# rvl-lab-utoronto/video_similarity_search

Hardware: NVIDIA B200
Metric: finch_full_hierarchy_embeddings_per_s (higher is better)
Workload: dtype f16 screen (f32 accumulate) + f32/f64 exact re-rank

## Files before the change

### include/slic_b200.h

```cpp
#ifndef SLIC_B200_H
#define SLIC_B200_H

#include <stddef.h>
#include <stdint.h>

#ifdef __cplusplus
extern "C" {
#endif

#define SLIC_ABI_VERSION 1

#define SLIC_F32 0
#define SLIC_F64 1

#define SLIC_METRIC_COSINE 0
#define SLIC_METRIC_EUCLIDEAN 1

typedef enum slic_status {
    SLIC_OK = 0,
    SLIC_ERR_INVALID_ARG = -1,
    SLIC_ERR_CUDA = -2,
    SLIC_ERR_UNSUPPORTED = -3,
    SLIC_ERR_NO_DEVICE = -4,
    SLIC_ERR_OVERFLOW = -5
} slic_status;

typedef void* slic_stream_t;

int slic_abi_version(void);
const char* slic_last_error(void);
int slic_require_device(void);
int64_t slic_launch_count(void);
int slic_profile_screen(int32_t enable);
int slic_last_screen_time(float* ms_out, double* flop_out);
int slic_last_screen_exec_flop(double* flop_out);

int slic_screen_trace(int32_t enable, uint64_t* counters_out_host);

int slic_normalize_rows(const void* x_dev, int64_t n, int32_t d, int32_t dtype,
                        void* unit_dev, void* norms_dev,
                        uint16_t* unit_f16_dev, int32_t d_pad, slic_stream_t stream);

int slic_center_columns(const float* x_dev, int64_t n, int32_t d, float* out_dev, float* means_out_dev,
                        slic_stream_t stream);

int slic_nn_exact_top1(const void* q_unit_dev, const int32_t* q_rows_dev, int64_t nq,
                       const void* x_unit_dev, int64_t n, int32_t d, int32_t dtype,
                       int64_t self_offset, int32_t* idx_out_dev, void* dist_out_dev,
                       slic_stream_t stream);

int slic_nn_top1(const void* q_unit_dev, const uint16_t* q_f16_dev, int64_t nq,
                 const void* x_unit_dev, const uint16_t* x_f16_dev, int64_t n,
                 int32_t d, int32_t d_pad, int32_t dtype, int64_t self_offset, float eps,
                 int32_t* idx_out_dev, void* dist_out_dev, int32_t* stats_out_dev ,
                 slic_stream_t stream);

int slic_sym_row_bests(const float* unit_dev, const uint16_t* unit_f16_dev, int64_t n, int32_t d, int32_t d_pad,
                       int32_t part, int32_t parts, int32_t* bests_out_dev, slic_stream_t stream);
int slic_nn_top1_sym_part(const float* unit_dev, const uint16_t* unit_f16_dev, int64_t n, int32_t d,
                          int32_t d_pad, int32_t part, int32_t parts, const int32_t* row_bests_dev, float eps,
                          uint64_t* keys_out_dev, int32_t* stats_out_dev ,
                          slic_stream_t stream);
int slic_unpack_neighbor_keys(const uint64_t* keys_dev, int64_t n, int32_t* idx_out_dev,
                              float* dist_out_dev, int32_t* status_out_dev, slic_stream_t stream);

int slic_debug_sym_plan(int64_t n, int32_t part, int32_t parts, int32_t mode, int32_t gated_chunks,
                        int32_t* units_out_host, int64_t capacity, int64_t* num_units_out_host);

int slic_screen_scores_debug(const uint16_t* q_f16_dev, int64_t nq, const uint16_t* x_f16_dev,
                             int64_t n, int32_t d_pad, float* out_dev, slic_stream_t stream);

int slic_distance_matrix(const void* q_dev, int64_t nq, const void* x_dev, int64_t n,
                         int32_t d, int32_t dtype, int32_t metric, int32_t same_matrix,
                         void* out_dev, int64_t ld_out, slic_stream_t stream);

int slic_rows_topk(const void* dist_dev, int64_t nq, int64_t n, int64_t ld, int32_t dtype,
                   int32_t k, int32_t* idx_out_dev, void* val_out_dev, slic_stream_t stream);

int slic_topk_cosine(const void* q_unit_dev, int64_t nq, const void* x_unit_dev, int64_t n,
                     int32_t d, int32_t dtype, int32_t k, int64_t self_offset,
                     int32_t* idx_out_dev, void* dist_out_dev, slic_stream_t stream);

int slic_topk_cosine_tc(const void* q_unit_dev, const uint16_t* q_f16_dev, int64_t nq,
                        const void* x_unit_dev, const uint16_t* x_f16_dev, int64_t n,
                        int32_t d, int32_t d_pad, int32_t dtype, int32_t k, int64_t self_offset,
                        float eps, int32_t* idx_out_dev, void* dist_out_dev,
                        int32_t* stats_out_dev, slic_stream_t stream);

int slic_hit_at_k(const int32_t* topk_idx_dev, int64_t nq, int32_t k_stride,
                  const int64_t* q_labels_dev, const int64_t* x_labels_dev,
                  const int32_t* ks_dev, int32_t num_ks, int32_t* hits_out_dev,
                  slic_stream_t stream);

int slic_finch_components(const int32_t* nn_dev, int64_t n, int32_t use_filter, double min_sim,
                          const void* unit_dev, int32_t d, int32_t dtype, const void* dist_nn_dev,
                          int32_t* labels_out_dev, int32_t* num_clust_out_dev,
                          slic_stream_t stream);

int slic_finch_min_sim(const int32_t* nn_dev, int64_t n, const void* unit_dev, int32_t d,
                       int32_t dtype, const void* dist_nn_dev, float* min_sim_out_dev,
                       slic_stream_t stream);

int slic_finch_closest_link(const int32_t* nn_dev, int64_t n, const void* unit_dev, int32_t d,
                            int32_t dtype, const void* dist_nn_dev, int32_t* pair_out_dev,
                            slic_stream_t stream);

int slic_compose_labels(const int32_t* prev_dev, const int32_t* u_dev, int64_t n,
                        int32_t* out_dev, slic_stream_t stream);

int slic_segmented_mean(const float* data_dev, const int32_t* labels_dev, int64_t n, int32_t d,
                        int32_t num_clust, double* out_dev, slic_stream_t stream);

int slic_cluster_sums(const float* data_dev, const int32_t* labels_dev, int64_t n, int32_t d,
                      int32_t num_clust, double* sums_out_dev, int32_t* counts_out_dev,
                      double* means_out_dev, slic_stream_t stream);
int slic_merge_cluster_sums(const double* sums_prev_dev, const int32_t* counts_prev_dev,
                            const int32_t* labels_dev, int64_t n_prev, int32_t d, int32_t num_clust,
                            double* sums_out_dev, int32_t* counts_out_dev, double* means_out_dev,
                            slic_stream_t stream);

int slic_kmeans_plusplus(const float* unit_dev, int64_t n, int32_t d, int32_t k, int64_t first_id,
                         const double* uniforms_host, int32_t L, int32_t* seeds_out_dev, slic_stream_t stream);
int slic_spherical_kmeans(const float* x_dev, int64_t n, int32_t d, int32_t k, const float* init_dev,
                          const int64_t* first_ids_host, const double* uniforms_host, int32_t L, int32_t n_init,
                          int32_t max_iter, double tol, int32_t* labels_out_dev, float* centers_out_dev,
                          double* inertia_out_host, int32_t* n_iter_out_host, int64_t* stats_out_host,
                          slic_stream_t stream);

int slic_label_mask_u8(const int64_t* a_dev, int64_t na, const int64_t* b_dev, int64_t nb,
                       int32_t prepend_ones, int32_t negate, uint8_t* out_dev,
                       slic_stream_t stream);
int slic_label_mask_bits(const int64_t* a_dev, int64_t na, const int64_t* b_dev, int64_t nb,
                         int32_t negate, uint32_t* out_dev, slic_stream_t stream);

int slic_scatter_last_wins(const int32_t* values_dev, const int64_t* positions_dev, int64_t n,
                           int64_t n_out, int32_t fill, int32_t* out_dev, int32_t* out_of_range_dev,
                           slic_stream_t stream);

int slic_dense_labels(const int32_t* labels_dev, int64_t n, int32_t* dense_out_dev, int32_t* uniq_out_dev,
                      int32_t* num_out_dev, slic_stream_t stream);

int slic_cluster_metrics(const int32_t* labels_true_dev, const int32_t* labels_pred_dev, int64_t n,
                         int32_t num_true, int32_t num_pred, int32_t want_emi, double* out_dev,
                         slic_stream_t stream);

int slic_group_by_label(const int32_t* labels_dev, int64_t n, int32_t num_labels,
                        int32_t* order_out_dev, int32_t* offsets_out_dev, slic_stream_t stream);

int slic_set_flann_threshold(int64_t rows);

int slic_finch(const float* data_dev, int64_t n, int32_t d,
               const int32_t* nn0_dev, const float* dist0_dev, const float* unit0_dev,
               int32_t level0_dense, int32_t ensure_early_exit, int32_t capacity,
               int32_t* labels_out_dev, int32_t* num_clust_out_host, int32_t* num_levels_out_host,
               float* min_sim_out_host , int32_t* has_min_sim_out_host ,
               slic_stream_t stream);

int slic_first_neighbors_host(const void* x_host, int64_t n, int32_t d, int32_t dtype,
                              int32_t* nn_out_host, void* dist_out_host);


int slic_finch_host(const float* x_host, int64_t n, int32_t d, const int64_t* initial_rank_host,
                    int32_t ensure_early_exit, int32_t capacity, int32_t* labels_out_host,
                    int32_t* num_clust_out_host, int32_t* num_levels_out_host,
                    float* min_sim_out_host , int32_t* has_min_sim_out_host );

int slic_copy_to_device(void* dst_dev, const void* src_host, int64_t bytes, slic_stream_t stream);

int slic_set_upload_overlap(int32_t enable);

typedef struct slic_comm slic_comm_t;
#define SLIC_COMM_HANDLE_BYTES 64

int slic_comm_create(const int32_t* devices, int32_t num_devices, int64_t max_rows, slic_comm_t** comm_out);
int slic_finch_multi(slic_comm_t* comm, const float* x_host, int64_t n, int32_t d, const int64_t* initial_rank_host,
                     int32_t ensure_early_exit, int32_t capacity, int32_t* labels_out_host,
                     int32_t* num_clust_out_host, int32_t* num_levels_out_host,
                     float* min_sim_out_host , int32_t* has_min_sim_out_host );
int slic_comm_last_timeline(slic_comm_t* comm, float* ms_out_host);
int slic_comm_destroy(slic_comm_t* comm);

int slic_comm_window_create(int64_t max_rows, slic_comm_t** comm_out, void* ipc_handle_out );
int slic_comm_connect(slic_comm_t* comm, int32_t rank, int32_t world, const void* all_handles);
int slic_comm_nn_top1(slic_comm_t* comm, const float* unit_dev, const uint16_t* f16_dev, int64_t n, int32_t d,
                      int32_t d_pad, int32_t* idx_out_dev, float* dist_out_dev, int32_t* status_out_dev,
                      slic_stream_t stream);

int slic_comm_finch(slic_comm_t* comm, const float* data_dev, int64_t n, int32_t d, int32_t ensure_early_exit,
                    int32_t capacity, int32_t* labels_out_dev, int32_t* num_clust_out_host,
                    int32_t* num_levels_out_host, float* min_sim_out_host ,
                    int32_t* has_min_sim_out_host , slic_stream_t stream);

int slic_host_trace(int32_t enable, float* ms_out_host);

#ifdef __cplusplus
}
#endif
#endif
```

### video_similarity_search_b200/_lib.py

```python
import ctypes
import os

from . import build as _build

_c = ctypes
_i32, _i64, _f32, _f64 = _c.c_int32, _c.c_int64, _c.c_float, _c.c_double
_ptr = _c.c_void_p

SIGNATURES = {
    "slic_abi_version": [],
    "slic_last_error": [],
    "slic_require_device": [],
    "slic_launch_count": [],
    "slic_profile_screen": [_i32],
    "slic_last_screen_time": [_ptr, _ptr],
    "slic_last_screen_exec_flop": [_ptr],
    "slic_screen_trace": [_i32, _ptr],
    "slic_normalize_rows": [_ptr, _i64, _i32, _i32, _ptr, _ptr, _ptr, _i32, _ptr],
    "slic_center_columns": [_ptr, _i64, _i32, _ptr, _ptr, _ptr],
    "slic_nn_exact_top1": [_ptr, _ptr, _i64, _ptr, _i64, _i32, _i32, _i64, _ptr, _ptr, _ptr],
    "slic_nn_top1": [_ptr, _ptr, _i64, _ptr, _ptr, _i64, _i32, _i32, _i32, _i64, _f32, _ptr, _ptr, _ptr, _ptr],
    "slic_sym_row_bests": [_ptr, _ptr, _i64, _i32, _i32, _i32, _i32, _ptr, _ptr],
    "slic_nn_top1_sym_part": [_ptr, _ptr, _i64, _i32, _i32, _i32, _i32, _ptr, _f32, _ptr, _ptr, _ptr],
    "slic_debug_sym_plan": [_i64, _i32, _i32, _i32, _i32, _ptr, _i64, _ptr],
    "slic_unpack_neighbor_keys": [_ptr, _i64, _ptr, _ptr, _ptr, _ptr],
    "slic_screen_scores_debug": [_ptr, _i64, _ptr, _i64, _i32, _ptr, _ptr],
    "slic_distance_matrix": [_ptr, _i64, _ptr, _i64, _i32, _i32, _i32, _i32, _ptr, _i64, _ptr],
    "slic_rows_topk": [_ptr, _i64, _i64, _i64, _i32, _i32, _ptr, _ptr, _ptr],
    "slic_topk_cosine": [_ptr, _i64, _ptr, _i64, _i32, _i32, _i32, _i64, _ptr, _ptr, _ptr],
    "slic_topk_cosine_tc": [_ptr, _ptr, _i64, _ptr, _ptr, _i64, _i32, _i32, _i32, _i32, _i64, _f32, _ptr, _ptr, _ptr, _ptr],
    "slic_hit_at_k": [_ptr, _i64, _i32, _ptr, _ptr, _ptr, _i32, _ptr, _ptr],
    "slic_finch_components": [_ptr, _i64, _i32, _f64, _ptr, _i32, _i32, _ptr, _ptr, _ptr, _ptr],
    "slic_finch_min_sim": [_ptr, _i64, _ptr, _i32, _i32, _ptr, _ptr, _ptr],
    "slic_finch_closest_link": [_ptr, _i64, _ptr, _i32, _i32, _ptr, _ptr, _ptr],
    "slic_compose_labels": [_ptr, _ptr, _i64, _ptr, _ptr],
    "slic_segmented_mean": [_ptr, _ptr, _i64, _i32, _i32, _ptr, _ptr],
    "slic_cluster_sums": [_ptr, _ptr, _i64, _i32, _i32, _ptr, _ptr, _ptr, _ptr],
    "slic_merge_cluster_sums": [_ptr, _ptr, _ptr, _i64, _i32, _i32, _ptr, _ptr, _ptr, _ptr],
    "slic_label_mask_u8": [_ptr, _i64, _ptr, _i64, _i32, _i32, _ptr, _ptr],
    "slic_label_mask_bits": [_ptr, _i64, _ptr, _i64, _i32, _ptr, _ptr],
    "slic_dense_labels": [_ptr, _i64, _ptr, _ptr, _ptr, _ptr],
    "slic_scatter_last_wins": [_ptr, _ptr, _i64, _i64, _i32, _ptr, _ptr, _ptr],
    "slic_cluster_metrics": [_ptr, _ptr, _i64, _i32, _i32, _i32, _ptr, _ptr],
    "slic_group_by_label": [_ptr, _i64, _i32, _ptr, _ptr, _ptr],
    "slic_first_neighbors_host": [_ptr, _i64, _i32, _i32, _ptr, _ptr],
    "slic_set_flann_threshold": [_i64],
    "slic_host_trace": [_i32, _ptr],
    "slic_set_upload_overlap": [_i32],
    "slic_copy_to_device": [_ptr, _ptr, _i64, _ptr],
    "slic_comm_create": [_ptr, _i32, _i64, _ptr],
    "slic_finch_multi": [_ptr, _ptr, _i64, _i32, _ptr, _i32, _i32, _ptr, _ptr, _ptr, _ptr, _ptr],
    "slic_comm_last_timeline": [_ptr, _ptr],
    "slic_comm_destroy": [_ptr],
    "slic_comm_window_create": [_i64, _ptr, _ptr],
    "slic_comm_connect": [_ptr, _i32, _i32, _ptr],
    "slic_comm_nn_top1": [_ptr, _ptr, _ptr, _i64, _i32, _i32, _ptr, _ptr, _ptr, _ptr],
    "slic_comm_finch": [_ptr, _ptr, _i64, _i32, _i32, _i32, _ptr, _ptr, _ptr, _ptr, _ptr, _ptr],
    "slic_finch": [_ptr, _i64, _i32, _ptr, _ptr, _ptr, _i32, _i32, _i32, _ptr, _ptr, _ptr, _ptr, _ptr, _ptr],
    "slic_finch_host": [_ptr, _i64, _i32, _ptr, _i32, _i32, _ptr, _ptr, _ptr, _ptr, _ptr],
    "slic_kmeans_plusplus": [_ptr, _i64, _i32, _i32, _i64, _ptr, _i32, _ptr, _ptr],
    "slic_spherical_kmeans": [_ptr, _i64, _i32, _i32, _ptr, _ptr, _ptr, _i32, _i32, _i32, _f64, _ptr, _ptr, _ptr, _ptr,
                              _ptr, _ptr],
}
_RESTYPES = {"slic_last_error": _c.c_char_p, "slic_launch_count": _c.c_int64}

SLIC_F32, SLIC_F64 = 0, 1
SLIC_METRIC_COSINE, SLIC_METRIC_EUCLIDEAN = 0, 1

_lib = None


class SlicError(RuntimeError):
    """A C-ABI call returned a negative status."""


def library_path():
    return _build.LIB_PATH


def load(build_if_missing=True):
    global _lib
    if _lib is not None:
        return _lib
    path = library_path()
    if not os.path.exists(path):
        if not build_if_missing:
            raise ImportError("libslic_b200.so is missing; run `python -m video_similarity_search_b200.build`")
        _build.build()
    lib = ctypes.CDLL(path)
    for name, argtypes in SIGNATURES.items():
        fn = getattr(lib, name)
        fn.argtypes = argtypes
        fn.restype = _RESTYPES.get(name, _c.c_int)
    if lib.slic_abi_version() != 1:
        raise ImportError("libslic_b200.so ABI version mismatch")
    _lib = lib
    return lib


def check(status, what):
    if status != 0:
        msg = load().slic_last_error()
        raise SlicError("%s failed with status %d: %s" % (what, status, msg.decode() if msg else "?"))


def call(name, *args):
    lib = load()
    check(getattr(lib, name)(*args), name)
```

### video_similarity_search_b200/csrc/nn_screen_tc.cu

```cuda
#include <cuda.h>
#include <cuda_fp16.h>
#include <math.h>
#include <stdlib.h>
#include <string.h>
#include <math_constants.h>

#include <algorithm>
#include <type_traits>
#include <vector>

#include "common.cuh"

namespace slic {

constexpr int TC_BM = 128, TC_BK = 64, TC_UMMA_K = 16;
constexpr int TC_BN = 256;
constexpr int TC_ARES_SPS = 2;
constexpr int TC_ROW_UNIT = 256;
static_assert(TC_ROW_UNIT == TC_BN, "a row unit's diagonal block is one column tile");
constexpr uint32_t TC_A_BYTES = TC_BM * TC_BK * 2;
constexpr int TC_ARES_MAX_SLABS = 8;
constexpr uint32_t TC_BAR_BYTES = 384;
constexpr int TC_UQ_DEPTH = 4;
constexpr int TC_TMEM_COLS = 512;
constexpr int TC_ACCS = TC_TMEM_COLS / TC_BN;
template <bool ARES, bool TOPK> struct TcCfg {
    static constexpr uint32_t B_ROWS = TC_BN / 2;
    static constexpr uint32_t B_BYTES = B_ROWS * TC_BK * 2;
    static constexpr uint32_t A_RES_BYTES = ARES ? TC_ARES_MAX_SLABS * TC_A_BYTES : 0;
    static constexpr int SPS = ARES ? TC_ARES_SPS : 2;
    static constexpr uint32_t SLAB_BYTES = ARES ? B_BYTES : TC_A_BYTES + B_BYTES;
    static constexpr uint32_t STAGE_BYTES = SPS * SLAB_BYTES;
    static constexpr int STAGES = ARES ? (TOPK ? 64 : 96) * 1024 / (int)STAGE_BYTES : 3;
    static_assert(STAGES >= 2 && STAGES <= 6, "ring depth");
    static constexpr uint32_t OPERAND_BYTES = A_RES_BYTES + STAGES * STAGE_BYTES;
    static constexpr uint32_t SMEM_BYTES = OPERAND_BYTES + TC_BAR_BYTES  + 960  +
                                           (TOPK ? 32768u : 0u) ;
    static constexpr uint32_t SYM_THR_BYTES = 2 * 2 * 128 * 2;
    static constexpr uint32_t SYM_SMEM_BYTES = OPERAND_BYTES + TC_BAR_BYTES + SYM_THR_BYTES + (ARES ? 640u : 960u);
    static constexpr uint32_t CORESIDENT_MAX_BYTES = 233472 - 2 * 1024;
    static_assert(TOPK || SYM_SMEM_BYTES <= CORESIDENT_MAX_BYTES,
                  "symmetric variant leaves no shared memory for a co-resident CTA of the upload stream");
    static_assert(TOPK || SMEM_BYTES <= CORESIDENT_MAX_BYTES,
                  "top-1 variant (gated launches) leaves no shared memory for a co-resident CTA of the upload stream");
    static_assert(SMEM_BYTES <= 232448, "exceeds the 227 KB of shared memory a CTA may use");
};
constexpr int TC_MAX_STAGES = 6;
constexpr int TC_EPI_WARPS = 8;
constexpr int TC_THREADS = 64 + 32 * TC_EPI_WARPS;
constexpr int TC_THREADS_SYM = TC_THREADS + 32;
constexpr float TC_DEFAULT_EPS = 0.001953125f + 0.0009765625f + 0.0000152587890625f;
constexpr int TC_TOPK_MAX = 64;
constexpr int TC_HIST_BINS = 128;
constexpr int TC_HIST_STRIDE = 2 * TC_BM;
constexpr uint32_t TC_TOPK_SMEM = TC_HIST_BINS * TC_HIST_STRIDE;
static_assert(TC_TOPK_SMEM == 32768, "TcCfg::SMEM_BYTES assumes 32 KB of histograms");

struct ScreenParams {
    int64_t nq, n;
    int num_k_slabs;
    int64_t self_offset;
    float eps;
    int cap;
    int splits;
    int tiles_per_split;
    int64_t num_units;
    int* cand_idx;
    float* cand_score;
    int* cand_cnt;
    int* cand_flags;
    int topk;
    float* cand_kth;
    int* cand_tb;
    float* dump;
    int* error_flag;
    unsigned long long* trace;
    const int4* unit_table;
    const int* gates;
    unsigned int* best_enc;
    int* log_q;
    int log_region;
    int* sync_counter;
    const int* sync_targets;
    int* queue;
    int num_peers;
    unsigned int* peer_best[SLIC_MAX_PEERS];
    int* peer_sync[SLIC_MAX_PEERS];
};

struct UnitInfo {
    int64_t row_unit;
    int64_t ct0;
    int count, stride;
    int gate;
    int stream;
    bool coldir;
};
__device__ __forceinline__ UnitInfo unit_info(const ScreenParams& p, int64_t u, int64_t n_col_tiles) {
    UnitInfo ui;
    if (p.unit_table) {
        const int4 e = __ldg(p.unit_table + u);
        ui.row_unit = e.x;
        ui.ct0 = e.y;
        ui.count = e.z & 0xffff;
        ui.stride = (int)((unsigned)e.z >> 16);
        ui.gate = (e.w & 0xfff) - 1;
        ui.stream = (e.w >> 12) & 0xffff;
        ui.coldir = ((e.w >> 28) & 1) != 0;
    } else {
        const int64_t row_units = p.num_units / p.splits;
        const int split = (int)(u / row_units);
        ui.row_unit = u % row_units;
        ui.ct0 = (int64_t)split * p.tiles_per_split;
        const int64_t left = n_col_tiles - ui.ct0;
        ui.count = (int)(left < p.tiles_per_split ? (left > 0 ? left : 0) : p.tiles_per_split);
        ui.stride = 1;
        ui.gate = -1;
        ui.stream = split;
        ui.coldir = false;
    }
    return ui;
}

__device__ __forceinline__ unsigned enc_score(float f) {
    const unsigned u = __float_as_uint(f);
    return (u & 0x80000000u) ? ~u : (u | 0x80000000u);
}
__device__ __forceinline__ float dec_score(unsigned e) {
    return __uint_as_float((e & 0x80000000u) ? (e & 0x7fffffffu) : ~e);
}
constexpr unsigned ENC_NEG_INF = 0x007fffffu;

__device__ __forceinline__ uint32_t smem_u32(const void* p) { return (uint32_t)__cvta_generic_to_shared(p); }

__device__ __forceinline__ void mbar_init(uint32_t bar, uint32_t count) {
    asm volatile("mbarrier.init.shared::cta.b64 [%0], %1;" ::"r"(bar), "r"(count));
}
__device__ __forceinline__ void mbar_arrive(uint32_t bar) {
    asm volatile("mbarrier.arrive.shared::cta.b64 _, [%0];" ::"r"(bar) : "memory");
}
__device__ __forceinline__ void mbar_expect_tx(uint32_t bar, uint32_t bytes) {
    asm volatile("mbarrier.arrive.expect_tx.shared::cta.b64 _, [%0], %1;" ::"r"(bar), "r"(bytes) : "memory");
}
__device__ int* g_timeout_record = nullptr;
__device__ int g_timeout_lock = 0;
__device__ __noinline__ void record_timeout(int site, int a, int b) {
    int* r = g_timeout_record;
    if (r && atomicCAS(&g_timeout_lock, 0, 1) == 0) {
        volatile int* v = r;
        v[1] = (int)blockIdx.x;
        v[2] = (int)threadIdx.x;
        v[3] = a;
        v[4] = b;
        v[0] = site;
        __threadfence_system();
    }
}

__device__ __forceinline__ void mbar_wait(uint32_t bar, uint32_t parity, int* error_flag) {
    uint32_t done = 0;
    long long t0 = 0;
    uint32_t polls = 0;
    while (true) {
        asm volatile(
            "{\n\t.reg .pred p;\n\t"
            "mbarrier.try_wait.parity.shared::cta.b64 p, [%1], %2;\n\t"
            "selp.u32 %0, 1, 0, p;\n\t}"
            : "=r"(done)
            : "r"(bar), "r"(parity)
            : "memory");
        if (done) return;
        if ((++polls & 0x3ff) == 0) {
            long long now = clock64();
            if (t0 == 0) t0 = now;
            else if (now - t0 > 8000000000ll) {
                if (error_flag) atomicExch(error_flag, 1);
                record_timeout(1, (int)bar, (int)parity);
                __trap();
            }
        }
    }
}
__device__ __forceinline__ void mbar_wait_traced(uint32_t bar, uint32_t parity, int* error_flag, unsigned long long& acc,
                                                 bool tracing) {
    if (!tracing) {
        mbar_wait(bar, parity, error_flag);
        return;
    }
    const long long t0 = clock64();
    mbar_wait(bar, parity, error_flag);
    acc += (unsigned long long)(clock64() - t0);
}
__device__ __forceinline__ bool mbar_test(uint32_t bar, uint32_t parity) {
    uint32_t done;
    asm volatile(
        "{\n\t.reg .pred p;\n\t"
        "mbarrier.test_wait.parity.shared::cta.b64 p, [%1], %2;\n\t"
        "selp.u32 %0, 1, 0, p;\n\t}"
        : "=r"(done)
        : "r"(bar), "r"(parity)
        : "memory");
    return done != 0;
}
constexpr int SCREEN_ERR_GATE = 3;
__device__ __forceinline__ void gate_wait(const int* gate, int* error_flag) {
    long long t0 = 0;
    uint32_t polls = 0;
    while (true) {
        int v;
        asm volatile("ld.acquire.gpu.global.b32 %0, [%1];" : "=r"(v) : "l"(gate) : "memory");
        if (v != 0) break;
        __nanosleep(256);
        if ((++polls & 0xff) == 0) {
            if (error_flag && *reinterpret_cast<volatile int*>(error_flag) == SCREEN_ERR_GATE) break;
            long long now = clock64();
            if (t0 == 0) t0 = now;
            else if (now - t0 > 4000000000ll) {
                if (error_flag) atomicCAS(error_flag, 0, SCREEN_ERR_GATE);
                record_timeout(2, (int)(reinterpret_cast<uintptr_t>(gate) & 0xffff), v);
                break;
            }
        }
    }
    asm volatile("fence.proxy.async.global;" ::: "memory");
}
__device__ __forceinline__ void counter_wait(const int* counter, int target, int* error_flag) {
    long long t0 = 0;
    uint32_t polls = 0;
    while (true) {
        int v;
        asm volatile("ld.acquire.sys.global.b32 %0, [%1];" : "=r"(v) : "l"(counter) : "memory");
        if (v >= target) break;
        __nanosleep(128);
        if ((++polls & 0xff) == 0) {
            if (error_flag && *reinterpret_cast<volatile int*>(error_flag) == SCREEN_ERR_GATE) break;
            long long now = clock64();
            if (t0 == 0) t0 = now;
            else if (now - t0 > 4000000000ll) {
                if (error_flag) atomicCAS(error_flag, 0, SCREEN_ERR_GATE);
                record_timeout(3, v, target);
                break;
            }
        }
    }
}
constexpr uint32_t TC_PEER_BIT_MASK = 0xFEFFFFFFu;
__device__ __forceinline__ void tma_load_2d_pair(const CUtensorMap* map, uint32_t dst, uint32_t leader_bar, int c0, int c1) {
    asm volatile(
        "cp.async.bulk.tensor.2d.cta_group::2.shared::cluster.global.mbarrier::complete_tx::bytes [%0], [%1, {%2, %3}], [%4];"
        ::"r"(dst), "l"(map), "r"(c0), "r"(c1), "r"(leader_bar & TC_PEER_BIT_MASK)
        : "memory");
}
__device__ __forceinline__ void mbar_arrive_leader(uint32_t bar) {
    asm volatile("mbarrier.arrive.shared::cluster.b64 _, [%0];" ::"r"(bar & TC_PEER_BIT_MASK) : "memory");
}
__device__ __forceinline__ uint32_t peer_smem_addr(uint32_t local_addr, uint32_t rank) {
    uint32_t r;
    asm volatile("mapa.shared::cluster.u32 %0, %1, %2;" : "=r"(r) : "r"(local_addr), "r"(rank));
    return r;
}
__device__ __forceinline__ void st_cluster_u32(uint32_t cluster_addr, uint32_t v) {
    asm volatile("st.shared::cluster.u32 [%0], %1;" ::"r"(cluster_addr), "r"(v) : "memory");
}
__device__ __forceinline__ void mbar_arrive_release_cluster(uint32_t cluster_addr) {
    asm volatile("mbarrier.arrive.release.cluster.shared::cluster.b64 _, [%0];" ::"r"(cluster_addr) : "memory");
}
__device__ __forceinline__ void mbar_wait_cluster(uint32_t bar, uint32_t parity, int* error_flag) {
    uint32_t done = 0;
    long long t0 = 0;
    uint32_t polls = 0;
    while (true) {
        asm volatile(
            "{\n\t.reg .pred p;\n\t"
            "mbarrier.try_wait.parity.acquire.cluster.shared::cta.b64 p, [%1], %2;\n\t"
            "selp.u32 %0, 1, 0, p;\n\t}"
            : "=r"(done)
            : "r"(bar), "r"(parity)
            : "memory");
        if (done) return;
        if ((++polls & 0x3ff) == 0) {
            long long now = clock64();
            if (t0 == 0) t0 = now;
            else if (now - t0 > 40000000000ll) {
                if (error_flag) atomicExch(error_flag, 1);
                record_timeout(4, (int)bar, (int)parity);
                __trap();
            }
        }
    }
}
struct UnitRing {
    uint32_t full, val;
    uint32_t empty_leader;
    int slot;
    uint32_t phase;
};
__device__ __forceinline__ int ring_take(UnitRing& r, bool whole_warp, int* error_flag) {
    mbar_wait_cluster(r.full + 8u * r.slot, r.phase, error_flag);
    int u;
    asm volatile("ld.shared.s32 %0, [%1];" : "=r"(u) : "r"(r.val + 4u * r.slot) : "memory");
    if (whole_warp) __syncwarp();
    if (!whole_warp || (threadIdx.x & 31) == 0) mbar_arrive_release_cluster(r.empty_leader + 8u * r.slot);
    if (++r.slot == TC_UQ_DEPTH) {
        r.slot = 0;
        r.phase ^= 1u;
    }
    return u;
}
__device__ __forceinline__ uint32_t cluster_ctarank() {
    uint32_t r;
    asm volatile("mov.u32 %0, %%cluster_ctarank;" : "=r"(r));
    return r;
}
__device__ __forceinline__ void cluster_sync_all() {
    asm volatile("barrier.cluster.arrive.release.aligned;" ::: "memory");
    asm volatile("barrier.cluster.wait.acquire.aligned;" ::: "memory");
}
__device__ __forceinline__ void tc_fence_before() { asm volatile("tcgen05.fence::before_thread_sync;" ::: "memory"); }
__device__ __forceinline__ void tc_fence_after() { asm volatile("tcgen05.fence::after_thread_sync;" ::: "memory"); }
__device__ __forceinline__ void umma_f16_pair(uint32_t tmem_d, uint64_t desc_a, uint64_t desc_b, uint32_t idesc,
                                               uint32_t accumulate) {
    asm volatile(
        "{\n\t.reg .pred p;\n\t"
        "setp.ne.b32 p, %4, 0;\n\t"
        "tcgen05.mma.cta_group::2.kind::f16 [%0], %1, %2, %3, p;\n\t}"
        ::"r"(tmem_d), "l"(desc_a), "l"(desc_b), "r"(idesc), "r"(accumulate)
        : "memory");
}
__device__ __forceinline__ void umma_commit_pair(uint32_t bar) {
    asm volatile(
        "tcgen05.commit.cta_group::2.mbarrier::arrive::one.shared::cluster.multicast::cluster.b64 [%0], %1;"
        ::"r"(bar), "h"((uint16_t)3)
        : "memory");
}
#define SLIC_V32_OUT(v)                                                                                              \
    "=r"(v[0]), "=r"(v[1]), "=r"(v[2]), "=r"(v[3]), "=r"(v[4]), "=r"(v[5]), "=r"(v[6]), "=r"(v[7]), "=r"(v[8]),     \
        "=r"(v[9]), "=r"(v[10]), "=r"(v[11]), "=r"(v[12]), "=r"(v[13]), "=r"(v[14]), "=r"(v[15]), "=r"(v[16]),      \
        "=r"(v[17]), "=r"(v[18]), "=r"(v[19]), "=r"(v[20]), "=r"(v[21]), "=r"(v[22]), "=r"(v[23]), "=r"(v[24]),     \
        "=r"(v[25]), "=r"(v[26]), "=r"(v[27]), "=r"(v[28]), "=r"(v[29]), "=r"(v[30]), "=r"(v[31])
#define SLIC_V32_INOUT(v)                                                                                            \
    "+r"(v[0]), "+r"(v[1]), "+r"(v[2]), "+r"(v[3]), "+r"(v[4]), "+r"(v[5]), "+r"(v[6]), "+r"(v[7]), "+r"(v[8]),     \
        "+r"(v[9]), "+r"(v[10]), "+r"(v[11]), "+r"(v[12]), "+r"(v[13]), "+r"(v[14]), "+r"(v[15]), "+r"(v[16]),      \
        "+r"(v[17]), "+r"(v[18]), "+r"(v[19]), "+r"(v[20]), "+r"(v[21]), "+r"(v[22]), "+r"(v[23]), "+r"(v[24]),     \
        "+r"(v[25]), "+r"(v[26]), "+r"(v[27]), "+r"(v[28]), "+r"(v[29]), "+r"(v[30]), "+r"(v[31])
__device__ __forceinline__ void tmem_ld_issue(uint32_t taddr, uint32_t (&v)[32]) {
    asm volatile(
        "tcgen05.ld.sync.aligned.32x32b.x32.b32 "
        "{%0,%1,%2,%3,%4,%5,%6,%7,%8,%9,%10,%11,%12,%13,%14,%15,%16,%17,%18,%19,%20,%21,%22,%23,%24,%25,%26,%27,%28,"
        "%29,%30,%31}, [%32];"
        : SLIC_V32_OUT(v)
        : "r"(taddr)
        : "memory");
}
__device__ __forceinline__ void tmem_ld_wait(uint32_t (&v)[32]) {
    asm volatile("tcgen05.wait::ld.sync.aligned;" : SLIC_V32_INOUT(v)::"memory");
}

__device__ __forceinline__ uint64_t umma_smem_desc(uint32_t smem_addr) {
    uint64_t d = 0;
    d |= (uint64_t)((smem_addr & 0x3FFFFu) >> 4);
    d |= (uint64_t)1 << 16;
    d |= (uint64_t)(1024 >> 4) << 32;
    d |= (uint64_t)1 << 46;
    d |= (uint64_t)2 << 61;
    return d;
}
constexpr uint32_t TC_IDESC = (1u << 4) | ((uint32_t)(TC_BN >> 3) << 17) | ((uint32_t)((2 * TC_BM) >> 4) << 24);

struct RowState {
    float best, thr;
    int cnt, flags;
};

__device__ __noinline__ RowState push_candidate(RowState st, float s, int col, float eps, int cap,
                                                int* __restrict__ li, float* __restrict__ ls) {
    if (s > st.best) {
        st.best = s;
        st.thr = s - eps;
    }
    if (st.cnt == cap) {
        int w = 0;
        for (int r = 0; r < st.cnt; ++r) {
            const float sc = ls[r];
            if (sc >= st.thr) {
                ls[w] = sc;
                li[w] = li[r];
                ++w;
            }
        }
        st.cnt = w;
        st.flags |= 2;
    }
    if (st.cnt < cap) {
        ls[st.cnt] = s;
        li[st.cnt] = col;
        ++st.cnt;
    } else {
        st.flags |= 1;
    }
    return st;
}

struct LogCtx {
    int* q;
    int* nb;
    float* s;
    unsigned int* cnt;
    int region;
    int* overflow;
};
__device__ __noinline__ void log_append_raw(int* lq, int* lnb, float* ls, unsigned int* cnt, int region, int* overflow,
                                            unsigned int* best_enc, int q, int nb, float s) {
    const unsigned pos = atomicAdd(cnt, 1u);
    if (pos < (unsigned)region) {
        lq[pos] = q;
        lnb[pos] = nb;
        ls[pos] = s;
    } else {
        *overflow = 1;
    }
    if (best_enc) atomicMax(best_enc + q, enc_score(s));
}
__device__ __forceinline__ void log_append(const LogCtx& lg, unsigned int* best_enc, int q, int nb, float s) {
    log_append_raw(lg.q, lg.nb, lg.s, lg.cnt, lg.region, lg.overflow, best_enc, q, nb, s);
}
struct RowStateK {
    float thr;
    int tb, cge, ctb, cnt, flags;
};

__device__ __forceinline__ int score_bin(float s) {
    const int b = __float2int_rd(s * (float)TC_HIST_BINS);
    return min(max(b, 0), TC_HIST_BINS - 1);
}
__device__ __forceinline__ float bin_edge(int b) { return b == 0 ? -1.0f : (float)b * (1.0f / (float)TC_HIST_BINS); }

__device__ __forceinline__ bool hist_insert(RowStateK& st, uint8_t* __restrict__ h, float s, int k) {
    const int b = score_bin(s);
    if (b > st.tb) {
        h[b * TC_HIST_STRIDE] = (uint8_t)(h[b * TC_HIST_STRIDE] + 1);
        ++st.cge;
        return st.cge - st.ctb >= k;
    }
    if (b == st.tb) {
        ++st.cge;
        ++st.ctb;
    }
    return false;
}
__device__ __forceinline__ void hist_advance(RowStateK& st, const uint8_t* __restrict__ h, int k, float eps) {
    while (st.cge - st.ctb >= k) {
        st.cge -= st.ctb;
        ++st.tb;
        st.ctb = h[st.tb * TC_HIST_STRIDE];
    }
    st.thr = bin_edge(st.tb) - eps;
}

__device__ __noinline__ RowStateK push_candidate_topk(RowStateK st, float s, int col, float eps, int cap, int k,
                                                      bool count, uint8_t* __restrict__ h, int* __restrict__ li,
                                                      float* __restrict__ ls) {
    if (st.cnt == cap) {
        int w = 0;
        for (int r = 0; r < st.cnt; ++r) {
            const float sc = ls[r];
            if (sc >= st.thr) {
                ls[w] = sc;
                li[w] = li[r];
                ++w;
            }
        }
        st.cnt = w;
        st.flags |= 2;
    }
    if (st.cnt < cap) {
        ls[st.cnt] = s;
        li[st.cnt] = col;
        ++st.cnt;
    } else {
        st.flags |= 1;
    }
    if (count && hist_insert(st, h, s, k)) hist_advance(st, h, k, eps);
    return st;
}

struct Pending {
    float s0, s1, s2, s3;
    int c0, c1, c2, c3;
    int n;
};
__device__ __forceinline__ void pend_put(Pending& pd, float s, int col) {
    if (pd.n == 0) {
        pd.s0 = s;
        pd.c0 = col;
    } else if (pd.n == 1) {
        pd.s1 = s;
        pd.c1 = col;
    } else if (pd.n == 2) {
        pd.s2 = s;
        pd.c2 = col;
    } else {
        pd.s3 = s;
        pd.c3 = col;
    }
    ++pd.n;
}
__device__ __forceinline__ void pend_flush(Pending& pd, RowStateK& st, float eps, int cap, int k, bool count,
                                           uint8_t* __restrict__ h, int* __restrict__ li, float* __restrict__ ls) {
    if (pd.n > 0) st = push_candidate_topk(st, pd.s0, pd.c0, eps, cap, k, count, h, li, ls);
    if (pd.n > 1) st = push_candidate_topk(st, pd.s1, pd.c1, eps, cap, k, count, h, li, ls);
    if (pd.n > 2) st = push_candidate_topk(st, pd.s2, pd.c2, eps, cap, k, count, h, li, ls);
    if (pd.n > 3) st = push_candidate_topk(st, pd.s3, pd.c3, eps, cap, k, count, h, li, ls);
    pd.n = 0;
}

__device__ __forceinline__ float thr_lo_minus(uint32_t w, float s) {
    float d;
    asm("{\n\t.reg .b16 lo, hi;\n\tmov.b32 {lo, hi}, %1;\n\tsub.rn.f32.f16 %0, lo, %2;\n\t}" : "=f"(d) : "r"(w), "f"(s));
    return d;
}
__device__ __forceinline__ float thr_hi_minus(uint32_t w, float s) {
    float d;
    asm("{\n\t.reg .b16 lo, hi;\n\tmov.b32 {lo, hi}, %1;\n\tsub.rn.f32.f16 %0, hi, %2;\n\t}" : "=f"(d) : "r"(w), "f"(s));
    return d;
}

template <bool TOPK>
struct EpiCtx {
    const ScreenParams* p;
    typename std::conditional<TOPK, RowStateK, RowState>::type st;
    Pending pd;
    uint8_t* hist;
    int* li;
    float* ls;
    int64_t row, self_col;
    bool row_ok, count, tracing;
    unsigned long long n_trig, n_chunks;
    LogCtx lg;
};

template <bool TOPK, bool SYM>
__device__ __forceinline__ void epi_chunk(EpiCtx<TOPK>& cx, uint32_t (&v)[32], int64_t col_base, bool plain,
                                          bool cdir = false, uint32_t thr_s = 0u ) {
    const ScreenParams& p = *cx.p;
    if (!plain) {
        if (col_base >= p.n) return;
        if (col_base + 32 > p.n || (cx.self_col >= col_base && cx.self_col < col_base + 32)) {
#pragma unroll
            for (int t = 0; t < 32; ++t)
                if (col_base + t >= p.n || col_base + t == cx.self_col) v[t] = __float_as_uint(-CUDART_INF_F);
        }
        if (p.dump && cx.row_ok) {
#pragma unroll
            for (int t = 0; t < 32; ++t)
                if (col_base + t < p.n) p.dump[cx.row * p.n + col_base + t] = __uint_as_float(v[t]);
        }
    }
    if constexpr (TOPK) {
        float g[4];
#pragma unroll
        for (int q = 0; q < 4; ++q) {
            g[q] = __uint_as_float(v[8 * q]);
#pragma unroll
            for (int t = 1; t < 8; ++t) g[q] = fmaxf(g[q], __uint_as_float(v[8 * q + t]));
        }
        const float m = fmaxf(fmaxf(g[0], g[1]), fmaxf(g[2], g[3]));
        if (cx.tracing) {
            ++cx.n_chunks;
            cx.n_trig += __any_sync(0xffffffffu, cx.row_ok && m >= cx.st.thr) ? 1 : 0;
        }
        if (cx.row_ok && m >= cx.st.thr) {
#pragma unroll
            for (int q = 0; q < 4; ++q) {
                float gm = g[q];
                while (gm >= cx.st.thr && gm > -CUDART_INF_F) {
                    int ga = 0;
                    float best = __uint_as_float(v[8 * q]);
#pragma unroll
                    for (int t = 1; t < 8; ++t) {
                        const float s = __uint_as_float(v[8 * q + t]);
                        if (s > best) {
                            best = s;
                            ga = t;
                        }
                    }
                    const int col = (int)(col_base + 8 * q + ga);
                    if (cx.pd.n < 4)
                        pend_put(cx.pd, best, col);
                    else
                        cx.st = push_candidate_topk(cx.st, best, col, p.eps, p.cap, p.topk, cx.count, cx.hist, cx.li,
                                                    cx.ls);
                    gm = -CUDART_INF_F;
#pragma unroll
                    for (int t = 0; t < 8; ++t) {
                        if (t == ga) v[8 * q + t] = __float_as_uint(-CUDART_INF_F);
                        gm = fmaxf(gm, __uint_as_float(v[8 * q + t]));
                    }
                }
            }
        }
        if (__any_sync(0xffffffffu, cx.pd.n >= 3))
            pend_flush(cx.pd, cx.st, p.eps, p.cap, p.topk, cx.count, cx.hist, cx.li, cx.ls);
    } else {
        float g[4];
#pragma unroll
        for (int q = 0; q < 4; ++q) {
            g[q] = __uint_as_float(v[8 * q]);
#pragma unroll
            for (int t = 1; t < 8; ++t) g[q] = fmaxf(g[q], __uint_as_float(v[8 * q + t]));
        }
        const float m = fmaxf(fmaxf(g[0], g[1]), fmaxf(g[2], g[3]));
        if (cx.row_ok && m >= cx.st.thr) {
#pragma unroll
            for (int q = 0; q < 4; ++q) {
                if (g[q] < cx.st.thr) continue;
#pragma unroll
                for (int t = 0; t < 8; ++t) {
                    const float s = __uint_as_float(v[8 * q + t]);
                    if (s >= cx.st.thr && s > -CUDART_INF_F) {
                        if constexpr (SYM) {
                            if (s > cx.st.best) {
                                cx.st.best = s;
                                cx.st.thr = s - p.eps;
                            }
                            log_append(cx.lg, nullptr, (int)cx.row, (int)(col_base + 8 * q + t), s);
                        } else {
                            cx.st = push_candidate(cx.st, s, (int)(col_base + 8 * q + t), p.eps, p.cap, cx.li, cx.ls);
                        }
                    }
                }
            }
        }
        if constexpr (SYM) {
            if (cdir) {
                float mc = CUDART_INF_F;
#pragma unroll
                for (int j = 0; j < 4; ++j) {
                    uint32_t w0, w1, w2, w3;
                    asm volatile("ld.shared.v4.b32 {%0, %1, %2, %3}, [%4];"
                                 : "=r"(w0), "=r"(w1), "=r"(w2), "=r"(w3)
                                 : "r"(thr_s + 16u * j));
                    mc = fminf(mc, fminf(thr_lo_minus(w0, __uint_as_float(v[8 * j])), thr_hi_minus(w0, __uint_as_float(v[8 * j + 1]))));
                    mc = fminf(mc, fminf(thr_lo_minus(w1, __uint_as_float(v[8 * j + 2])), thr_hi_minus(w1, __uint_as_float(v[8 * j + 3]))));
                    mc = fminf(mc, fminf(thr_lo_minus(w2, __uint_as_float(v[8 * j + 4])), thr_hi_minus(w2, __uint_as_float(v[8 * j + 5]))));
                    mc = fminf(mc, fminf(thr_lo_minus(w3, __uint_as_float(v[8 * j + 6])), thr_hi_minus(w3, __uint_as_float(v[8 * j + 7]))));
                }
                const bool hit = cx.row_ok && mc <= 0.f;
                if (cx.tracing) {
                    ++cx.n_chunks;
                    cx.n_trig += __any_sync(0xffffffffu, hit) ? 1 : 0;
                }
                if (hit) {
#pragma unroll
                    for (int t = 0; t < 32; t += 2) {
                        uint32_t w;
                        asm volatile("ld.shared.b32 %0, [%1];" : "=r"(w) : "r"(thr_s + 2u * t));
                        const float s0 = __uint_as_float(v[t]), s1 = __uint_as_float(v[t + 1]);
                        if (thr_lo_minus(w, s0) <= 0.f) log_append(cx.lg, p.best_enc, (int)(col_base + t), (int)cx.row, s0);
                        if (thr_hi_minus(w, s1) <= 0.f) log_append(cx.lg, p.best_enc, (int)(col_base + t + 1), (int)cx.row, s1);
                    }
                }
            }
        }
    }
}

constexpr int TC_TOP1_MAX_REGS = 152;
template <bool TOPK, bool ARES, bool SYM = false>
__global__ void __maxnreg__(TOPK ? 168 : TC_TOP1_MAX_REGS) nn_screen_kernel(const __grid_constant__ CUtensorMap tmap_q,
                                                                  const __grid_constant__ CUtensorMap tmap_x,
                                                                  const ScreenParams p) {
    typedef TcCfg<ARES, TOPK> Cfg;
    constexpr int STAGES = Cfg::STAGES;
    static_assert(!SYM || !TOPK, "the symmetric variant exists for the top-1 kernels only");
    extern __shared__ uint8_t smem_raw[];
    uint8_t* smem = reinterpret_cast<uint8_t*>((reinterpret_cast<uintptr_t>(smem_raw) + 1023) & ~(uintptr_t)1023);
    {
        uint32_t dyn_bytes;
        asm volatile("mov.u32 %0, %%dynamic_smem_size;" : "=r"(dyn_bytes));
        const uint32_t need = Cfg::OPERAND_BYTES + TC_BAR_BYTES + (SYM ? Cfg::SYM_THR_BYTES : 0u) + (TOPK ? TC_TOPK_SMEM : 0u);
        if ((uint32_t)(smem - smem_raw) + need > dyn_bytes) {
            if (threadIdx.x == 0 && p.error_flag) atomicExch(p.error_flag, 2);
            return;
        }
    }
    uint64_t* bars = reinterpret_cast<uint64_t*>(smem + Cfg::OPERAND_BYTES);
    const uint32_t bar_full = smem_u32(bars);
    const uint32_t bar_empty = smem_u32(bars + TC_MAX_STAGES);
    const uint32_t bar_acc_full = smem_u32(bars + 12);
    const uint32_t bar_acc_empty = smem_u32(bars + 16);
    const uint32_t bar_a_full = smem_u32(bars + 20);
    const uint32_t bar_a_empty = smem_u32(bars + 21);
    uint32_t* tmem_slot = reinterpret_cast<uint32_t*>(bars + 22);
    const uint32_t bar_thr_full = smem_u32(bars + 28);
    const uint32_t bar_thr_empty = smem_u32(bars + 32);
    const uint32_t bar_uq_full = smem_u32(bars + 36);
    const uint32_t bar_uq_empty = smem_u32(bars + 40);
    const uint32_t uq_val = smem_u32(bars + 44);
    static_assert(46 * 8 <= TC_BAR_BYTES && 2 * TC_MAX_STAGES <= 12, "barrier block layout");
    const uint32_t smem_base = smem_u32(smem);
    const uint32_t ring_base = smem_base + Cfg::A_RES_BYTES;

    const int warp = threadIdx.x >> 5, lane = threadIdx.x & 31;
    const bool tracing = p.trace != nullptr;
    const uint32_t cta_rank = cluster_ctarank();

    if (threadIdx.x == 0) {
        asm volatile("prefetch.tensormap [%0];" ::"l"(&tmap_q) : "memory");
        asm volatile("prefetch.tensormap [%0];" ::"l"(&tmap_x) : "memory");
        for (int s = 0; s < STAGES; ++s) {
            mbar_init(bar_full + 8 * s, 1);
            mbar_init(bar_empty + 8 * s, 1);
        }
        for (int a = 0; a < TC_ACCS; ++a) {
            mbar_init(bar_acc_full + 8 * a, 1);
            mbar_init(bar_acc_empty + 8 * a, 2 * TC_EPI_WARPS);
        }
        mbar_init(bar_a_full, 1);
        mbar_init(bar_a_empty, 1);
        for (int s = 0; s < TC_UQ_DEPTH; ++s) {
            mbar_init(bar_uq_full + 8 * s, 1);
            mbar_init(bar_uq_empty + 8 * s, 2 * (TC_EPI_WARPS + (SYM ? 1 : 0)) + 2);
        }
        if constexpr (SYM) {
            for (int b = 0; b < 2; ++b) {
                mbar_init(bar_thr_full + 8 * b, 1);
                mbar_init(bar_thr_empty + 8 * b, TC_EPI_WARPS);
            }
        }
        asm volatile("fence.mbarrier_init.release.cluster;" ::: "memory");
    }
    if (warp == 1) {
        asm volatile("tcgen05.alloc.cta_group::2.sync.aligned.shared::cta.b32 [%0], %1;" ::"r"(smem_u32(tmem_slot)),
                     "r"(TC_TMEM_COLS)
                     : "memory");
        asm volatile("tcgen05.relinquish_alloc_permit.cta_group::2.sync.aligned;" ::: "memory");
    }
    tc_fence_before();
    __syncthreads();
    cluster_sync_all();
    tc_fence_after();
    const uint32_t tmem_base = *reinterpret_cast<volatile uint32_t*>(tmem_slot);

    const int64_t n_col_tiles = (p.n + TC_BN - 1) / TC_BN;
    UnitRing ring;
    ring.full = bar_uq_full;
    ring.val = uq_val;
    ring.empty_leader = peer_smem_addr(bar_uq_empty, 0u);
    ring.slot = 0;
    ring.phase = 0u;

    if (warp == 0) {
        if (lane == 0) {
            int stage = 0;
            uint32_t phase = 0, a_phase = 0;
            unsigned long long t_wait = 0;
            const bool scheduler = cta_rank == 0;
            int u_next = scheduler ? atomicAdd(p.queue, 1) : 0;
            while (true) {
                int u;
                if (scheduler) {
                    u = u_next < p.num_units ? u_next : -1;
                    mbar_wait_cluster(bar_uq_empty + 8u * ring.slot, ring.phase ^ 1u, p.error_flag);
#pragma unroll
                    for (uint32_t r = 0; r < 2u; ++r) {
                        st_cluster_u32(peer_smem_addr(uq_val + 4u * ring.slot, r), (uint32_t)u);
                        mbar_arrive_release_cluster(peer_smem_addr(bar_uq_full + 8u * ring.slot, r));
                    }
                    if (++ring.slot == TC_UQ_DEPTH) {
                        ring.slot = 0;
                        ring.phase ^= 1u;
                    }
                    if (u >= 0) u_next = atomicAdd(p.queue, 1);
                } else {
                    u = ring_take(ring, false, p.error_flag);
                }
                if (u < 0) break;
                const UnitInfo ui = unit_info(p, u, n_col_tiles);
                const int64_t row_block = ui.row_unit * 2 + cta_rank;
                if (ui.gate >= 0) gate_wait(p.gates + ui.gate, p.error_flag);
                if constexpr (SYM) {
                    if (ui.coldir && p.sync_counter)
                        counter_wait(p.sync_counter, __ldg(p.sync_targets + ui.gate + 1), p.error_flag);
                }
                if constexpr (ARES) {
                    mbar_wait_traced(bar_a_empty, a_phase ^ 1, p.error_flag, t_wait, tracing);
                    if (cta_rank == 0) mbar_expect_tx(bar_a_full, 2 * (uint32_t)p.num_k_slabs * TC_A_BYTES);
                    for (int ks = 0; ks < p.num_k_slabs; ++ks)
                        tma_load_2d_pair(&tmap_q, smem_base + ks * TC_A_BYTES, bar_a_full, ks * TC_BK,
                                         (int)(row_block * TC_BM));
                    a_phase ^= 1;
                }
                for (int kt = 0; kt < ui.count; ++kt) {
                    const int64_t ct = ui.ct0 + (int64_t)kt * ui.stride;
                    for (int ks = 0; ks < p.num_k_slabs; ks += Cfg::SPS) {
                        mbar_wait_traced(bar_empty + 8 * stage, phase ^ 1, p.error_flag, t_wait, tracing);
                        const uint32_t a_dst = ring_base + stage * Cfg::STAGE_BYTES;
                        const uint32_t b_dst = ARES ? a_dst : a_dst + TC_A_BYTES;
                        if constexpr (ARES) {
                            const int nsl = min(Cfg::SPS, p.num_k_slabs - ks);
                            if (cta_rank == 0) mbar_expect_tx(bar_full + 8 * stage, 2 * (uint32_t)nsl * Cfg::B_BYTES);
                            for (int j = 0; j < nsl; ++j)
                                tma_load_2d_pair(&tmap_x, b_dst + j * Cfg::SLAB_BYTES, bar_full + 8 * stage, (ks + j) * TC_BK,
                                                 (int)(ct * TC_BN + cta_rank * Cfg::B_ROWS));
                        } else {
                            const int nsl = min(Cfg::SPS, p.num_k_slabs - ks);
                            if (cta_rank == 0) mbar_expect_tx(bar_full + 8 * stage, 2 * (uint32_t)nsl * Cfg::SLAB_BYTES);
                            for (int j = 0; j < nsl; ++j) {
                                tma_load_2d_pair(&tmap_q, a_dst + j * Cfg::SLAB_BYTES, bar_full + 8 * stage, (ks + j) * TC_BK,
                                                 (int)(row_block * TC_BM));
                                tma_load_2d_pair(&tmap_x, b_dst + j * Cfg::SLAB_BYTES, bar_full + 8 * stage, (ks + j) * TC_BK,
                                                 (int)(ct * TC_BN + cta_rank * Cfg::B_ROWS));
                            }
                        }
                        if (++stage == STAGES) {
                            stage = 0;
                            phase ^= 1;
                        }
                    }
                }
            }
            if (tracing) atomicAdd(p.trace + 0, t_wait);
        }
    } else if (warp == 1) {
        if (lane == 0 && cta_rank == 0) {
            int stage = 0;
            uint32_t phase = 0;
            int acc = 0;
            uint32_t acc_phase = 0, a_phase = 0;
            unsigned long long t_acc = 0, t_smem = 0;
            const long long t_begin = tracing ? clock64() : 0;
            unsigned long long t_ring = 0, n_units = 0;
            while (true) {
                const long long tr0 = tracing ? clock64() : 0;
                const int u = ring_take(ring, false, p.error_flag);
                if (tracing) t_ring += (unsigned long long)(clock64() - tr0);
                if (u < 0) break;
                ++n_units;
                const int n_tiles = unit_info(p, u, n_col_tiles).count;
                if constexpr (ARES) {
                    mbar_wait_traced(bar_a_full, a_phase, p.error_flag, t_smem, tracing);
                    tc_fence_after();
                    a_phase ^= 1;
                }
                for (int kt = 0; kt < n_tiles; ++kt) {
                    mbar_wait_traced(bar_acc_empty + 8 * acc, acc_phase ^ 1, p.error_flag, t_acc, tracing);
                    tc_fence_after();
                    const uint32_t tmem_d = tmem_base + (uint32_t)(acc * TC_BN);
                    for (int ks = 0; ks < p.num_k_slabs; ks += Cfg::SPS) {
                        mbar_wait_traced(bar_full + 8 * stage, phase, p.error_flag, t_smem, tracing);
                        tc_fence_after();
                        const uint32_t st_addr = ring_base + stage * Cfg::STAGE_BYTES;
#pragma unroll
                        for (int j = 0; j < Cfg::SPS; ++j) {
                            if (ks + j < p.num_k_slabs) {
                                const uint32_t sl_addr = st_addr + j * Cfg::SLAB_BYTES;
                                const uint64_t da = umma_smem_desc(ARES ? smem_base + (ks + j) * TC_A_BYTES : sl_addr);
                                const uint64_t db = umma_smem_desc(ARES ? sl_addr : sl_addr + TC_A_BYTES);
#pragma unroll
                                for (int k = 0; k < TC_BK / TC_UMMA_K; ++k) {
                                    umma_f16_pair(tmem_d, da + (uint64_t)(2 * k), db + (uint64_t)(2 * k), TC_IDESC,
                                                  (uint32_t)((ks | j | k) != 0));
                                }
                            }
                        }
                        umma_commit_pair(bar_empty + 8 * stage);
                        if (++stage == STAGES) {
                            stage = 0;
                            phase ^= 1;
                        }
                    }
                    umma_commit_pair(bar_acc_full + 8 * acc);
                    if (++acc == TC_ACCS) {
                        acc = 0;
                        acc_phase ^= 1;
                    }
                }
                if constexpr (ARES) umma_commit_pair(bar_a_empty);
            }
            if (tracing) {
                atomicAdd(p.trace + 1, t_acc);
                atomicAdd(p.trace + 2, t_smem);
                atomicAdd(p.trace + 3, (unsigned long long)(clock64() - t_begin));
                atomicAdd(p.trace + 8, t_ring);
                atomicAdd(p.trace + 10, n_units);
            }
        }
    } else if (SYM && warp == 2 + TC_EPI_WARPS) {
        uint16_t* thr_buf = reinterpret_cast<uint16_t*>(smem + Cfg::OPERAND_BYTES + TC_BAR_BYTES);
        constexpr unsigned ENC_POS_INF = 0xff800000u;
        constexpr int PER_LANE = TC_BN / 32;
        unsigned cseq = 0u;
        for (int u; (u = ring_take(ring, true, p.error_flag)) >= 0;) {
            const UnitInfo ui = unit_info(p, u, n_col_tiles);
            if (!ui.coldir) continue;
            if (p.sync_counter) {
                if (lane == 0) counter_wait(p.sync_counter, __ldg(p.sync_targets + ui.gate + 1), p.error_flag);
                __syncwarp();
            }
            for (int kt = 0; kt < ui.count; ++kt) {
                const int64_t ct = ui.ct0 + (int64_t)kt * ui.stride;
                if (ct == ui.row_unit) continue;
                const uint32_t buf = cseq & 1u, ph = (cseq >> 1) & 1u;
                unsigned e[PER_LANE];
#pragma unroll
                for (int j = 0; j < PER_LANE; ++j) {
                    const int64_t c = ct * TC_BN + lane + 32 * j;
                    e[j] = c < p.n ? __ldcg(p.best_enc + c) : ENC_POS_INF;
                }
                mbar_wait(bar_thr_empty + 8 * buf, ph ^ 1u, p.error_flag);
                const uint32_t ta = smem_u32(thr_buf + buf * 256u) + 2u * lane;
#pragma unroll
                for (int j = 0; j < PER_LANE; ++j) {
                    const unsigned short t = __half_as_ushort(__float2half_rd(fmaxf(dec_score(e[j]) - p.eps, -60000.f)));
                    asm volatile("st.shared.b16 [%0], %1;" ::"r"(ta + 64u * j), "h"(t) : "memory");
                }
                __syncwarp();
                if (lane == 0) mbar_arrive(bar_thr_full + 8 * buf);
                ++cseq;
            }
        }
    } else {
        const int quad = warp & 3;
        const int half = (warp - 2) >> 2;
        const int row_in_tile = quad * 32 + lane;
        unsigned seq_all = 0;
        unsigned long long t_full = 0;
        const long long t_begin = tracing ? clock64() : 0;
        EpiCtx<TOPK> cx;
        cx.p = &p;
        cx.tracing = tracing;
        cx.n_trig = 0;
        cx.n_chunks = 0;
        if constexpr (TOPK) cx.hist = smem + Cfg::OPERAND_BYTES + TC_BAR_BYTES + half * TC_BM + row_in_tile;
        unsigned int* s_logcnt = reinterpret_cast<unsigned int*>(bars + 24) + (warp - 2);
        uint16_t* thr_buf = reinterpret_cast<uint16_t*>(smem + Cfg::OPERAND_BYTES + TC_BAR_BYTES);
        unsigned tile_seq = 0;
        const int64_t log_region_id = (int64_t)blockIdx.x * TC_EPI_WARPS + (warp - 2);
        if constexpr (SYM) {
            if (lane == 0) *s_logcnt = 0u;
            __syncwarp();
            cx.lg.q = p.log_q + log_region_id * p.log_region;
            cx.lg.nb = p.cand_idx + log_region_id * p.log_region;
            cx.lg.s = p.cand_score + log_region_id * p.log_region;
            cx.lg.cnt = s_logcnt;
            cx.lg.region = p.log_region;
            cx.lg.overflow = p.cand_flags;
        }
        unsigned long long t_unit = 0;
        while (true) {
            const long long tr0 = tracing ? clock64() : 0;
            const int u = ring_take(ring, true, p.error_flag);
            if (u < 0) break;
            const UnitInfo ui = unit_info(p, u, n_col_tiles);
            if constexpr (SYM) {
                if (ui.coldir && p.sync_counter) {
                    if (lane == 0) counter_wait(p.sync_counter, __ldg(p.sync_targets + ui.gate + 1), p.error_flag);
                    __syncwarp();
                }
            }
            if (tracing) t_unit += (unsigned long long)(clock64() - tr0);
            const int64_t row_block = ui.row_unit * 2 + cta_rank;
            cx.row = row_block * TC_BM + row_in_tile;
            cx.row_ok = cx.row < p.nq;
            cx.self_col = (p.self_offset >= 0 && cx.row_ok) ? cx.row + p.self_offset : -1;
            const int64_t slot = SYM ? 0 : (int64_t)(ui.stream * 2 + half) * p.nq + (cx.row_ok ? cx.row : 0);
            cx.li = p.cand_idx + slot * p.cap;
            cx.ls = p.cand_score + slot * p.cap;
            if constexpr (TOPK) {
                for (int i = 0; i < TC_HIST_BINS; ++i) cx.hist[i * TC_HIST_STRIDE] = 0;
                int seed = 0;
                if (p.cand_tb && cx.row_ok)
                    for (int s2 = 0; s2 < 2 * p.splits; ++s2) seed = max(seed, __ldcg(p.cand_tb + (int64_t)s2 * p.nq + cx.row));
                cx.st.tb = seed;
                cx.st.cge = 0;
                cx.st.ctb = 0;
                cx.st.thr = bin_edge(seed) - p.eps;
                cx.pd.n = 0;
            } else if constexpr (SYM) {
                cx.st.best = cx.row_ok ? dec_score(__ldcg(p.best_enc + cx.row)) : -CUDART_INF_F;
                cx.st.thr = cx.st.best - p.eps;
            } else {
                cx.st.best = -CUDART_INF_F;
                cx.st.thr = -CUDART_INF_F;
            }
            cx.st.cnt = 0;
            cx.st.flags = 0;
            uint32_t va[32], vb[32];
            bool prefetched = false;
            bool first = true;
            for (int kt = 0; kt < ui.count; ++kt, ++seq_all) {
                const int acc = (int)(seq_all % (unsigned)TC_ACCS);
                const uint32_t acc_phase = (seq_all / (unsigned)TC_ACCS) & 1u;
                const int64_t ct = ui.ct0 + (int64_t)kt * ui.stride;
                const int64_t col0 = ct * TC_BN + half * 128;
                bool cdir = false;
                uint32_t thr_tile = 0u;
                uint32_t thr_done_bar = 0u;
                if constexpr (SYM) {
                    cdir = ui.coldir && ct != ui.row_unit;
                    if (cdir) {
                        const uint32_t buf = tile_seq & 1u, ph = (tile_seq >> 1) & 1u;
                        thr_tile = smem_u32(thr_buf + (buf * 2 + half) * 128);
                        thr_done_bar = bar_thr_empty + 8 * buf;
                        mbar_wait(bar_thr_full + 8 * buf, ph, p.error_flag);
                        ++tile_seq;
                    }
                }
                if (TOPK || !prefetched) {
                    mbar_wait_traced(bar_acc_full + 8 * acc, acc_phase, p.error_flag, t_full, tracing);
                    tc_fence_after();
                }
                const uint32_t tbase = tmem_base + ((uint32_t)(quad * 32) << 16) + (uint32_t)(acc * TC_BN + half * 128);
                if constexpr (TOPK) {
                    cx.count = !first;
                    if (first) {
#pragma unroll 1
                        for (int c = 0; c < 4; ++c) {
                            tmem_ld_issue(tbase + (uint32_t)(c * 32), va);
                            tmem_ld_wait(va);
                            const int64_t col_base = col0 + c * 32;
                            if (col_base >= p.n || !cx.row_ok) continue;
#pragma unroll
                            for (int t = 0; t < 32; ++t) {
                                if (col_base + t < p.n && col_base + t != cx.self_col)
                                    hist_insert(cx.st, cx.hist, __uint_as_float(va[t]), p.topk);
                            }
                            hist_advance(cx.st, cx.hist, p.topk, p.eps);
                        }
                    }
                }
                const bool plain = col0 + 128 <= p.n && !p.dump &&
                                   (p.self_offset < 0 || row_block * TC_BM + p.self_offset + TC_BM <= col0 ||
                                    row_block * TC_BM + p.self_offset >= col0 + 128);
                if constexpr (TOPK) {
                    tmem_ld_issue(tbase, vb);
#pragma unroll 1
                    for (int c = 0; c < 4; ++c) {
                        tmem_ld_wait(vb);
#pragma unroll
                        for (int t = 0; t < 32; ++t) va[t] = vb[t];
                        if (c < 3) {
                            tmem_ld_issue(tbase + (uint32_t)(32 * (c + 1)), vb);
                        } else {
                            tc_fence_before();
                            __syncwarp();
                            if (lane == 0) mbar_arrive_leader(bar_acc_empty + 8 * acc);
                        }
                        epi_chunk<TOPK, false>(cx, va, col0 + 32 * c, plain);
                    }
                } else {
                    if (!prefetched) tmem_ld_issue(tbase, va);
                    prefetched = false;
#pragma unroll 1
                    for (int h = 0; h < 2; ++h) {
                        tmem_ld_wait(va);
                        tmem_ld_issue(tbase + (uint32_t)(64 * h + 32), vb);
                        epi_chunk<false, SYM>(cx, va, col0 + 64 * h, plain, cdir, thr_tile + 128u * h);
                        tmem_ld_wait(vb);
                        if (h == 0) {
                            tmem_ld_issue(tbase + 64u, va);
                        } else {
                            tc_fence_before();
                            __syncwarp();
                            if (lane == 0) mbar_arrive_leader(bar_acc_empty + 8 * acc);
                            if (kt + 1 < ui.count) {
                                const unsigned nxt = seq_all + 1;
                                const int acc_n = (int)(nxt % (unsigned)TC_ACCS);
                                const bool ready = __all_sync(0xffffffffu, mbar_test(bar_acc_full + 8 * acc_n, (nxt / (unsigned)TC_ACCS) & 1u));
                                if (ready) {
                                    tc_fence_after();
                                    tmem_ld_issue(tmem_base + ((uint32_t)(quad * 32) << 16) + (uint32_t)(acc_n * TC_BN + half * 128),
                                                  va);
                                    prefetched = true;
                                }
                            }
                        }
                        epi_chunk<false, SYM>(cx, vb, col0 + 64 * h + 32, plain, cdir, thr_tile + 128u * h + 64u);
                    }
                    if constexpr (SYM) {
                        if (cdir) {
                            __syncwarp();
                            if (lane == 0) mbar_arrive(thr_done_bar);
                        }
                    }
                }
                if constexpr (TOPK) {
                    if (first) pend_flush(cx.pd, cx.st, p.eps, p.cap, p.topk, false, cx.hist, cx.li, cx.ls);
                }
                first = false;
            }
            if constexpr (TOPK) pend_flush(cx.pd, cx.st, p.eps, p.cap, p.topk, true, cx.hist, cx.li, cx.ls);
            if constexpr (SYM) {
                if (cx.row_ok && cx.st.best > -CUDART_INF_F) {
                    const unsigned e = enc_score(cx.st.best);
                    atomicMax(p.best_enc + cx.row, e);
                    if (!ui.coldir)
                        for (int g = 0; g < p.num_peers; ++g) atomicMax(p.peer_best[g] + cx.row, e);
                }
                if (!ui.coldir && p.sync_counter) {
                    if (p.num_peers) __threadfence_system();
                    else __threadfence();
                    __syncwarp();
                    if (lane == 0) {
                        atomicAdd(p.sync_counter, 1);
                        for (int g = 0; g < p.num_peers; ++g) atomicAdd(p.peer_sync[g], 1);
                    }
                }
            } else if (cx.row_ok) {
                p.cand_cnt[slot] = cx.st.cnt;
                p.cand_flags[slot] = cx.st.flags;
                if constexpr (TOPK) {
                    p.cand_kth[slot] = bin_edge(cx.st.tb);
                    if (p.cand_tb) p.cand_tb[slot] = cx.st.tb;
                }
            }
        }
        if constexpr (SYM) {
            __syncwarp();
            if (lane == 0) p.cand_cnt[log_region_id] = (int)min(*s_logcnt, (unsigned)p.log_region);
        }
        if (tracing && lane == 0 && warp == 2) {
            atomicAdd(p.trace + 4, t_full);
            atomicAdd(p.trace + 5, (unsigned long long)(clock64() - t_begin));
            atomicAdd(p.trace + 6, cx.n_trig);
            atomicAdd(p.trace + 7, cx.n_chunks);
            atomicAdd(p.trace + 9, t_unit);
        }
    }

    tc_fence_before();
    __syncthreads();
    cluster_sync_all();
    if (warp == 1) {
        tc_fence_after();
        asm volatile("tcgen05.dealloc.cta_group::2.sync.aligned.b32 %0, %1;" ::"r"(tmem_base), "r"(TC_TMEM_COLS) : "memory");
    }
}

template <typename T>
__global__ void __launch_bounds__(256) rerank_top1_kernel(const T* __restrict__ q_unit, const T* __restrict__ x_unit,
                                                          int64_t nq, int d, float eps, int cap, int splits,
                                                          const int* __restrict__ cand_idx,
                                                          const float* __restrict__ cand_score,
                                                          const int* __restrict__ cand_cnt,
                                                          const int* __restrict__ cand_flags, int* __restrict__ idx_out,
                                                          T* __restrict__ dist_out, int* __restrict__ overflow_rows,
                                                          int* __restrict__ stats) {
    const int lane = threadIdx.x & 31;
    const int64_t r = (int64_t)blockIdx.x * (blockDim.x >> 5) + (threadIdx.x >> 5);
    if (r >= nq) return;
    float gbest = -CUDART_INF_F;
    int flags = 0;
    for (int sp = 0; sp < splits; ++sp) {
        const int64_t slot = (int64_t)sp * nq + r;
        const int c = min(cand_cnt[slot], cap);
        flags |= cand_flags[slot];
        for (int e = lane; e < c; e += 32) gbest = fmaxf(gbest, cand_score[slot * cap + e]);
    }
#pragma unroll
    for (int o = 16; o > 0; o >>= 1) gbest = fmaxf(gbest, __shfl_xor_sync(0xffffffffu, gbest, o));
    const float thr = gbest - eps;
    const T* qr = q_unit + r * d;
    double best_d = CUDART_INF;
    int best_j = 0x7fffffff, reranked = 0;
    for (int sp = 0; sp < splits; ++sp) {
        const int64_t slot = (int64_t)sp * nq + r;
        const int c = min(cand_cnt[slot], cap);
        for (int e = 0; e < c; ++e) {
            if (cand_score[slot * cap + e] < thr) continue;
            const int j = cand_idx[slot * cap + e];
            const double s = warp_dot<T>(qr, x_unit + (int64_t)j * d, d, lane);
            ++reranked;
            const double dist = (double)cosine_distance_from_sim<T>(s);
            if (closer(dist, j, best_d, best_j)) {
                best_d = dist;
                best_j = j;
            }
        }
    }
    if (lane == 0) {
        idx_out[r] = best_j == 0x7fffffff ? -1 : best_j;
        if (dist_out) dist_out[r] = (T)best_d;
        atomicAdd(&stats[0], reranked);
        if (flags & 2) atomicAdd(&stats[2], 1);
        if ((flags & 1) || best_j == 0x7fffffff) {
            const int pos = atomicAdd(&stats[1], 1);
            overflow_rows[pos] = (int)r;
        }
    }
}

template <typename T>
__global__ void scatter_rows_kernel(const int* __restrict__ rows, int count, const int* __restrict__ idx_src,
                                    const T* __restrict__ dist_src, int* __restrict__ idx_out, T* __restrict__ dist_out) {
    const int i = blockIdx.x * blockDim.x + threadIdx.x;
    if (i >= count) return;
    idx_out[rows[i]] = idx_src[i];
    if (dist_out) dist_out[rows[i]] = dist_src[i];
}

constexpr int RK_THREADS = 128, RK_MAX = 1024, RK_BINS = 1024;

template <typename T>
__global__ void __launch_bounds__(RK_THREADS) rerank_topk_kernel(const T* __restrict__ q_unit, const T* __restrict__ x_unit,
                                                                 int64_t nq, int d, float eps, int cap, int splits, int k,
                                                                 const int* __restrict__ cand_idx,
                                                                 const float* __restrict__ cand_score,
                                                                 const int* __restrict__ cand_cnt,
                                                                 const int* __restrict__ cand_flags,
                                                                 const float* __restrict__ cand_kth,
                                                                 int* __restrict__ idx_out, T* __restrict__ dist_out,
                                                                 int* __restrict__ overflow_rows, int* __restrict__ stats) {
    __shared__ int s_idx[RK_MAX];
    __shared__ T s_dist[RK_MAX];
    __shared__ int s_hist[RK_BINS];
    __shared__ int s_part[RK_THREADS];
    __shared__ int s_m, s_flags;
    __shared__ float s_thr;
    const int64_t r = blockIdx.x;
    const int tid = threadIdx.x, lane = tid & 31, warp = tid >> 5;
    if (tid == 0) {
        float kth = -CUDART_INF_F;
        int fl = 0, listed = 0;
        for (int sp = 0; sp < splits; ++sp) {
            kth = fmaxf(kth, cand_kth[(int64_t)sp * nq + r]);
            fl |= cand_flags[(int64_t)sp * nq + r];
            listed += cand_cnt[(int64_t)sp * nq + r];
        }
        atomicAdd(&stats[3], listed >> 4);
        s_thr = kth - eps;
        s_flags = fl;
        s_m = 0;
    }
    __syncthreads();
    for (int b = tid; b < RK_BINS; b += RK_THREADS) s_hist[b] = 0;
    __syncthreads();
    const float thr0 = s_thr;
    for (int sp = 0; sp < splits; ++sp) {
        const int64_t slot = (int64_t)sp * nq + r;
        const int c = cand_cnt[slot];
        for (int e = tid; e < c; e += RK_THREADS) {
            const float sc = cand_score[slot * cap + e];
            if (sc >= thr0) atomicAdd(&s_hist[min(max(__float2int_rd(sc * (float)RK_BINS), 0), RK_BINS - 1)], 1);
        }
    }
    __syncthreads();
    {
        constexpr int PER = RK_BINS / RK_THREADS;
        int local = 0;
#pragma unroll
        for (int i = 0; i < PER; ++i) local += s_hist[tid * PER + i];
        s_part[tid] = local;
        __syncthreads();
        for (int off = 1; off < RK_THREADS; off <<= 1) {
            const int add = tid + off < RK_THREADS ? s_part[tid + off] : 0;
            __syncthreads();
            s_part[tid] += add;
            __syncthreads();
        }
        const int above = tid + 1 < RK_THREADS ? s_part[tid + 1] : 0;
        if (above < k && s_part[tid] >= k) {
            int cum = above, b = tid * PER + PER - 1;
            for (; b > tid * PER; --b) {
                cum += s_hist[b];
                if (cum >= k) break;
            }
            const float edge = b == 0 ? -1.0f : (float)b * (1.0f / (float)RK_BINS);
            s_thr = fmaxf(thr0, edge - eps);
        }
    }
    __syncthreads();
    const float thr = s_thr;
    for (int sp = 0; sp < splits; ++sp) {
        const int64_t slot = (int64_t)sp * nq + r;
        const int c = cand_cnt[slot];
        for (int e = tid; e < c; e += RK_THREADS) {
            if (cand_score[slot * cap + e] >= thr) {
                const int pos = atomicAdd(&s_m, 1);
                if (pos < RK_MAX) s_idx[pos] = cand_idx[slot * cap + e];
            }
        }
    }
    __syncthreads();
    const int m = s_m;
    if ((s_flags & 1) || m > RK_MAX || m < k) {
        if (tid == 0) overflow_rows[atomicAdd(&stats[1], 1)] = (int)r;
        return;
    }
    const T* qr = q_unit + r * d;
    for (int e = warp; e < m; e += RK_THREADS / 32) {
        const double s = warp_dot<T>(qr, x_unit + (int64_t)s_idx[e] * d, d, lane);
        if (lane == 0) s_dist[e] = cosine_distance_from_sim<T>(s);
    }
    int m2 = 2;
    while (m2 < m) m2 <<= 1;
    for (int e = m + tid; e < m2; e += RK_THREADS) {
        s_dist[e] = (T)CUDART_INF;
        s_idx[e] = 0x7fffffff;
    }
    __syncthreads();
    for (int size = 2; size <= m2; size <<= 1) {
        for (int stride = size >> 1; stride > 0; stride >>= 1) {
            for (int t = tid; t < (m2 >> 1); t += RK_THREADS) {
                const int lo = 2 * t - (t & (stride - 1));
                const int hi = lo + stride;
                const bool up = ((lo & size) == 0);
                const T da = s_dist[lo], db = s_dist[hi];
                const int ia = s_idx[lo], ib = s_idx[hi];
                const bool a_after_b = (da > db) || (da == db && ia > ib);
                if (a_after_b == up) {
                    s_dist[lo] = db; s_dist[hi] = da;
                    s_idx[lo] = ib; s_idx[hi] = ia;
                }
            }
            __syncthreads();
        }
    }
    for (int j = tid; j < k; j += RK_THREADS) {
        idx_out[r * k + j] = s_idx[j];
        if (dist_out) dist_out[r * k + j] = s_dist[j];
    }
    if (tid == 0) {
        atomicAdd(&stats[0], m);
        if (s_flags & 2) atomicAdd(&stats[2], 1);
    }
}

template <typename T>
__global__ void scatter_topk_rows_kernel(const int* __restrict__ rows, int count, int k, const int* __restrict__ idx_src,
                                         const T* __restrict__ dist_src, int* __restrict__ idx_out,
                                         T* __restrict__ dist_out) {
    const int64_t i = (int64_t)blockIdx.x * blockDim.x + threadIdx.x;
    if (i >= (int64_t)count * k) return;
    const int64_t dst = (int64_t)rows[i / k] * k + (i % k);
    idx_out[dst] = idx_src[i];
    if (dist_out) dist_out[dst] = dist_src[i];
}

typedef CUresult (*EncodeTiledFn)(CUtensorMap*, CUtensorMapDataType, cuuint32_t, void*, const cuuint64_t*,
                                  const cuuint64_t*, const cuuint32_t*, const cuuint32_t*, CUtensorMapInterleave,
                                  CUtensorMapSwizzle, CUtensorMapL2promotion, CUtensorMapFloatOOBfill);

static int get_encode_fn(EncodeTiledFn* out) {
    static EncodeTiledFn cached = nullptr;
    if (!cached) {
        void* fn = nullptr;
        cudaDriverEntryPointQueryResult qres;
        SLIC_CUDA_OK(cudaGetDriverEntryPoint("cuTensorMapEncodeTiled", &fn, cudaEnableDefault, &qres));
        if (qres != cudaDriverEntryPointSuccess || !fn) {
            set_error("cuTensorMapEncodeTiled is not available from the driver");
            return SLIC_ERR_UNSUPPORTED;
        }
        cached = reinterpret_cast<EncodeTiledFn>(fn);
    }
    *out = cached;
    return SLIC_OK;
}

static int make_tmap(CUtensorMap* map, const uint16_t* base, int64_t rows, int d_pad, int box_rows) {
    EncodeTiledFn enc;
    SLIC_PROPAGATE(get_encode_fn(&enc));
    cuuint64_t gdim[2] = {(cuuint64_t)d_pad, (cuuint64_t)rows};
    cuuint64_t gstride[1] = {(cuuint64_t)d_pad * 2};
    cuuint32_t box[2] = {(cuuint32_t)TC_BK, (cuuint32_t)box_rows};
    cuuint32_t estr[2] = {1, 1};
    CUresult r = enc(map, CU_TENSOR_MAP_DATA_TYPE_FLOAT16, 2, const_cast<uint16_t*>(base), gdim, gstride, box, estr,
                     CU_TENSOR_MAP_INTERLEAVE_NONE, CU_TENSOR_MAP_SWIZZLE_128B, CU_TENSOR_MAP_L2_PROMOTION_L2_256B,
                     CU_TENSOR_MAP_FLOAT_OOB_FILL_NONE);
    if (r != CUDA_SUCCESS) {
        set_error("cuTensorMapEncodeTiled failed with CUresult %d (rows=%lld d_pad=%d)", (int)r, (long long)rows, d_pad);
        return SLIC_ERR_CUDA;
    }
    return SLIC_OK;
}

static bool g_profile = false, g_have_sample = false;
static unsigned long long* g_trace = nullptr;
static cudaEvent_t g_ev_start = nullptr, g_ev_stop = nullptr;
static double g_last_flop = 0.0, g_last_exec_flop = 0.0;

struct ScreenPlan {
    int splits, tiles_per_split;
    int64_t units;
};

static ScreenPlan plan_screen(int64_t nq, int64_t n) {
    const int64_t row_blocks = ceil_div(nq, TC_ROW_UNIT), col_tiles = ceil_div(n, TC_BN);
    const int64_t sms = num_sms() / 2;
    int64_t want = ceil_div(6 * sms, row_blocks);
    const int64_t min_tiles = 8;
    int64_t max_splits = col_tiles / min_tiles > 0 ? col_tiles / min_tiles : 1;
    int64_t splits = want < 1 ? 1 : (want > max_splits ? max_splits : want);
    ScreenPlan pl;
    pl.tiles_per_split = (int)ceil_div(col_tiles, splits);
    pl.splits = (int)ceil_div(col_tiles, pl.tiles_per_split);
    pl.units = row_blocks * pl.splits;
    return pl;
}

static ScreenPlan plan_screen_topk(int64_t nq, int64_t n, int k) {
    const int64_t row_blocks = ceil_div(nq, TC_ROW_UNIT), col_tiles = ceil_div(n, TC_BN);
    const int64_t sms = num_sms() / 2;
    const int64_t startup = 6;
    int64_t best_s = 1, best_cost = INT64_MAX;
    const int64_t min_tps = ceil_div((int64_t)32 * k, TC_BN / 2);
    for (int pass = 0; pass < 2; ++pass) {
        for (int64_t sp = 1; sp <= col_tiles && sp <= 64; ++sp) {
            const int64_t tps = ceil_div(col_tiles, sp);
            if (sp > 1 && tps < min_tps) break;
            const int64_t real = ceil_div(col_tiles, tps);
            const int64_t waves = ceil_div(row_blocks * real, sms);
            const int64_t cost = waves * (tps + startup);
            if (pass == 0) {
                if (cost < best_cost) {
                    best_cost = cost;
                    best_s = real;
                }
            } else if (cost * 100 <= best_cost * 102) {
                best_s = real;
                break;
            }
        }
    }
    ScreenPlan pl;
    pl.tiles_per_split = (int)ceil_div(col_tiles, best_s);
    pl.splits = (int)ceil_div(col_tiles, pl.tiles_per_split);
    pl.units = row_blocks * pl.splits;
    return pl;
}

static int topk_cap(int k, int64_t cols_per_split) {
    double later = cols_per_split > 128 ? (double)k * log((double)cols_per_split / 128.0) : 0.0;
    int64_t want = 128 + (int64_t)(3.0 * later) + 128;
    int cap = 512;
    while (cap < want && cap < 4096) cap <<= 1;
    return cap;
}

typedef void (*KernelFn)(const CUtensorMap, const CUtensorMap, const ScreenParams);
static bool screen_ares(int d_pad) { return d_pad / TC_BK <= TC_ARES_MAX_SLABS; }
static void pick_screen_kernel(bool sym, bool ares, bool is_topk, KernelFn* fn, size_t* smem_bytes) {
    if (sym) {
        *fn = ares ? (KernelFn)nn_screen_kernel<false, true, true> : (KernelFn)nn_screen_kernel<false, false, true>;
        *smem_bytes = ares ? TcCfg<true, false>::SYM_SMEM_BYTES : TcCfg<false, false>::SYM_SMEM_BYTES;
    } else if (ares) {
        *fn = is_topk ? (KernelFn)nn_screen_kernel<true, true> : (KernelFn)nn_screen_kernel<false, true>;
        *smem_bytes = is_topk ? TcCfg<true, true>::SMEM_BYTES : TcCfg<true, false>::SMEM_BYTES;
    } else {
        *fn = is_topk ? (KernelFn)nn_screen_kernel<true, false> : (KernelFn)nn_screen_kernel<false, false>;
        *smem_bytes = is_topk ? TcCfg<false, true>::SMEM_BYTES : TcCfg<false, false>::SMEM_BYTES;
    }
}

static int* g_timeout_record_host = nullptr;
static int arm_timeout_record() {
    if (!g_timeout_record_host) {
        SLIC_CUDA_OK(cudaHostAlloc(&g_timeout_record_host, 8 * sizeof(int), cudaHostAllocMapped));
        int* dev_view = nullptr;
        SLIC_CUDA_OK(cudaHostGetDevicePointer(&dev_view, g_timeout_record_host, 0));
        SLIC_CUDA_OK(cudaMemcpyToSymbol(g_timeout_record, &dev_view, sizeof(dev_view)));
    }
    for (int i = 0; i < 8; ++i) g_timeout_record_host[i] = 0;
    return SLIC_OK;
}
const char* timeout_record_text() {
    static thread_local char buf[160];
    const int* r = g_timeout_record_host;
    if (!r || r[0] == 0) return "";
    snprintf(buf, sizeof(buf), " [timed-out wait: site %d (1 mbarrier, 2 upload gate, 3 pre-pass counter) block %d thread %d a=%d b=%d]",
             r[0], r[1], r[2], r[3], r[4]);
    return buf;
}

static int launch_screen(const uint16_t* q_f16, int64_t nq, const uint16_t* x_f16, int64_t n, int d_pad,
                         int64_t self_offset, float eps, int cap, const ScreenPlan& pl, int* cand_idx, float* cand_score,
                         int* cand_cnt, int* cand_flags, float* dump, int* error_flag, cudaStream_t st, int topk = 0,
                         float* cand_kth = nullptr, const int4* unit_table = nullptr, const int* gates = nullptr,
                         unsigned int* best_enc = nullptr, int64_t exec_tiles = 0, int* log_q = nullptr,
                         int log_region = 0, int* sync_counter = nullptr, const int* sync_targets = nullptr,
                         const ScreenPeers* peers = nullptr, int* cand_tb = nullptr) {
    if (gates) SLIC_PROPAGATE(arm_timeout_record());
    CUtensorMap tq, tx;
    SLIC_PROPAGATE(make_tmap(&tq, q_f16, nq, d_pad, TC_BM));
    SLIC_PROPAGATE(make_tmap(&tx, x_f16, n, d_pad, TC_BN / 2));
    ScreenParams p;
    p.nq = nq;
    p.n = n;
    p.num_k_slabs = d_pad / TC_BK;
    p.self_offset = self_offset;
    p.eps = eps;
    p.cap = cap;
    p.splits = pl.splits;
    p.tiles_per_split = pl.tiles_per_split;
    p.num_units = pl.units;
    p.cand_idx = cand_idx;
    p.cand_score = cand_score;
    p.cand_cnt = cand_cnt;
    p.cand_flags = cand_flags;
    p.topk = topk;
    p.cand_kth = cand_kth;
    p.cand_tb = cand_tb;
    p.dump = dump;
    p.error_flag = error_flag;
    p.trace = g_trace;
    p.unit_table = unit_table;
    p.gates = gates;
    p.best_enc = best_enc;
    p.log_q = log_q;
    p.log_region = log_region;
    p.sync_counter = sync_counter;
    p.sync_targets = sync_targets;
    p.num_peers = 0;
    for (int g = 0; g < SLIC_MAX_PEERS; ++g) {
        p.peer_best[g] = nullptr;
        p.peer_sync[g] = nullptr;
    }
    if (peers) {
        p.num_peers = peers->num_peers;
        for (int g = 0; g < peers->num_peers; ++g) {
            p.peer_best[g] = peers->peer_best[g];
            p.peer_sync[g] = peers->peer_sync[g];
        }
    }
    Scratch queue;
    SLIC_CUDA_OK(queue.alloc(sizeof(int), st));
    SLIC_CUDA_OK(cudaMemsetAsync(queue.ptr, 0, sizeof(int), st));
    p.queue = queue.as<int>();
    const bool sym = best_enc != nullptr;
    const bool is_topk = topk > 0;
    const bool ares = screen_ares(d_pad);
    if (sym && (is_topk || !unit_table)) {
        set_error("symmetric screen: needs the top-1 kernel and a unit list");
        return SLIC_ERR_UNSUPPORTED;
    }
    KernelFn fn;
    size_t smem_bytes;
    pick_screen_kernel(sym, ares, is_topk, &fn, &smem_bytes);
    static bool attr_done[64][8] = {{false}};
    int dev = 0;
    SLIC_CUDA_OK(cudaGetDevice(&dev));
    bool& attr_set = attr_done[dev & 63][(sym ? 4 : 0) + (ares ? 2 : 0) + (is_topk ? 1 : 0)];
    if (!attr_set) {
        SLIC_CUDA_OK(cudaFuncSetAttribute(fn, cudaFuncAttributeMaxDynamicSharedMemorySize, (int)smem_bytes));
        attr_set = true;
    }
    const int64_t pairs = num_sms() / 2;
    const int64_t grid = (pl.units < pairs ? pl.units : pairs) * 2;
    if (g_profile) {
        if (!g_ev_start) {
            SLIC_CUDA_OK(cudaEventCreate(&g_ev_start));
            SLIC_CUDA_OK(cudaEventCreate(&g_ev_stop));
        }
        SLIC_CUDA_OK(cudaEventRecord(g_ev_start, st));
    }
    cudaLaunchConfig_t cfg = {};
    cfg.gridDim = dim3((unsigned)grid);
    cfg.blockDim = dim3(sym ? TC_THREADS_SYM : TC_THREADS);
    cfg.dynamicSmemBytes = smem_bytes;
    cfg.stream = st;
    cudaLaunchAttribute attr[1];
    attr[0].id = cudaLaunchAttributeClusterDimension;
    attr[0].val.clusterDim.x = 2;
    attr[0].val.clusterDim.y = 1;
    attr[0].val.clusterDim.z = 1;
    cfg.attrs = attr;
    cfg.numAttrs = 1;
    SLIC_CUDA_OK(cudaLaunchKernelEx(&cfg, fn, tq, tx, p));
    SLIC_LAUNCH_OK();
    if (g_profile) {
        SLIC_CUDA_OK(cudaEventRecord(g_ev_stop, st));
        g_last_flop = 2.0 * (double)nq * (double)n * (double)d_pad;
        g_last_exec_flop = exec_tiles > 0 ? 2.0 * (double)exec_tiles * TC_ROW_UNIT * TC_BN * (double)d_pad : g_last_flop;
        g_have_sample = true;
    }
    return SLIC_OK;
}

struct PinnedSlot {
    void* host = nullptr;
    size_t cap = 0;
    cudaEvent_t done = nullptr;
    bool used = false;
};
static int stage_to_device(void* dst_dev, const void* src, size_t bytes, cudaStream_t st) {
    constexpr int SLOTS = 8;
    static thread_local PinnedSlot ring[SLOTS];
    static thread_local int next = 0;
    if (bytes == 0) return SLIC_OK;
    PinnedSlot& s = ring[next];
    next = (next + 1) % SLOTS;
    if (s.used) SLIC_CUDA_OK(cudaEventSynchronize(s.done));
    if (s.cap < bytes) {
        if (s.host) SLIC_CUDA_OK(cudaFreeHost(s.host));
        s.cap = bytes < ((size_t)1 << 20) ? ((size_t)1 << 20) : bytes + bytes / 2;
        SLIC_CUDA_OK(cudaHostAlloc(&s.host, s.cap, cudaHostAllocDefault));
    }
    if (!s.done) SLIC_CUDA_OK(cudaEventCreateWithFlags(&s.done, cudaEventDisableTiming));
    memcpy(s.host, src, bytes);
    SLIC_CUDA_OK(cudaMemcpyAsync(dst_dev, s.host, bytes, cudaMemcpyHostToDevice, st));
    SLIC_CUDA_OK(cudaEventRecord(s.done, st));
    s.used = true;
    return SLIC_OK;
}

constexpr int TC_CAP = 32;

static int4 unit_entry(int64_t row_unit, int64_t ct0, int count, int stride, int gate, int stream, bool coldir) {
    int4 e;
    e.x = (int)row_unit;
    e.y = (int)ct0;
    e.z = (count & 0xffff) | (stride << 16);
    e.w = ((gate + 1) & 0xfff) | ((stream & 0xffff) << 12) | (coldir ? (1 << 28) : 0);
    return e;
}

constexpr int SYM_CHUNK_TILES = 64;
constexpr int SYM_SAMPLE_TILES = 16;
enum SymMode { SYM_FULL = 0, SYM_BESTS = 1, SYM_TRIANGLE = 2, SYM_FUSED = 3 };
constexpr int SYM_FUSED_PRE_TILES = 16;
static int plan_screen_sym(int64_t n, int part, int parts, const GateSpec* g, ScreenPlan* pl, std::vector<int4>* table,
                           SymMode mode = SYM_FULL, int64_t* prepass_units_all = nullptr) {
    const bool own_rows_prepass = mode == SYM_BESTS || mode == SYM_FUSED;
    const int64_t R = ceil_div(n, TC_ROW_UNIT), T = ceil_div(n, TC_BN);
    SLIC_REQUIRE(T < 65536, "symmetric screen: too many column tiles");
    SLIC_REQUIRE(parts >= 1 && part >= 0 && part < parts, "symmetric screen: bad partition");
    int64_t chunk_tiles_gate = 0, chunk_units_gate = 0;
    if (g) {
        SLIC_REQUIRE(g->gates && g->num_chunks >= 1 && g->num_chunks < 4095 && g->chunk_rows > 0 &&
                         g->chunk_rows % TC_ROW_UNIT == 0,
                     "gated screen: chunk_rows must be a positive multiple of 256");
        SLIC_REQUIRE(ceil_div(n, g->chunk_rows) == g->num_chunks, "gated screen: chunks do not tile the database");
        chunk_tiles_gate = g->chunk_rows / TC_BN;
        chunk_units_gate = g->chunk_rows / TC_ROW_UNIT;
    }
    table->clear();
    const int64_t span = g ? (chunk_tiles_gate < T ? chunk_tiles_gate : T) : T;
    int samples = own_rows_prepass ? (parts >= 4 ? 2 * SYM_SAMPLE_TILES : SYM_SAMPLE_TILES) : SYM_SAMPLE_TILES / parts;
    if (own_rows_prepass && samples > span / 4) samples = (int)(span / 4);
    if (mode == SYM_FULL && R < 128 && samples > R / 16) samples = (int)(R / 16);
    if (samples < 4) samples = 4;
    if (samples > span) samples = (int)span;
    const int stride = (int)(span / samples);
    const int64_t pre0 = own_rows_prepass ? R * part / parts : 0;
    const int64_t pre1 = own_rows_prepass ? R * (part + 1) / parts : R;
    const int pre_len = mode == SYM_FUSED ? SYM_FUSED_PRE_TILES : samples;
    if (prepass_units_all) *prepass_units_all = R * ceil_div(samples, pre_len);
    for (int64_t r = pre0; r < pre1 && mode != SYM_TRIANGLE; ++r) {
        const int gate = g ? (int)(r / chunk_units_gate) : -1;
        for (int s0 = 0; s0 < samples; s0 += pre_len)
            table->push_back(unit_entry(r, (int64_t)s0 * stride, samples - s0 < pre_len ? samples - s0 : pre_len, stride, gate, 0,
                                        false));
    }
    const int64_t chunk_tiles = SYM_CHUNK_TILES;
    int64_t total_tiles = 0;
    for (int64_t c0 = 0; c0 < T; c0 += chunk_tiles) {
        const int64_t c1 = c0 + chunk_tiles < T ? c0 + chunk_tiles : T;
        for (int64_t r = 0; r < c1; ++r) total_tiles += c1 - (r > c0 ? r : c0);
    }
    const int64_t pairs = num_sms() / 2 > 0 ? num_sms() / 2 : 1;
    int64_t unit_len = total_tiles / parts / (pairs * 12);
    unit_len = unit_len < 8 ? 8 : (unit_len > chunk_tiles ? chunk_tiles : unit_len);
    int64_t seen_tiles = 0;
    for (int64_t c0 = 0; c0 < T && mode != SYM_BESTS; c0 += chunk_tiles) {
        const int64_t c1 = c0 + chunk_tiles < T ? c0 + chunk_tiles : T;
        for (int64_t r = 0; r < c1; ++r) {
            const int gate = g ? (int)((c1 - 1) / chunk_tiles_gate) : -1;
            for (int64_t ct0 = r > c0 ? r : c0; ct0 < c1; ct0 += unit_len) {
                const int64_t cnt = c1 - ct0 < unit_len ? c1 - ct0 : unit_len;
                const int64_t owner = seen_tiles * parts / total_tiles;
                seen_tiles += cnt;
                if (owner != part) continue;
                table->push_back(unit_entry(r, ct0, (int)cnt, 1, gate, 0, true));
            }
        }
    }
    if (g)
        std::stable_sort(table->begin(), table->end(), [](const int4& a, const int4& b) { return (a.w & 0xfff) < (b.w & 0xfff); });
    pl->splits = 1;
    pl->tiles_per_split = (int)T;
    pl->units = (int64_t)table->size();
    return SLIC_OK;
}

static int plan_screen_gated(int64_t nq, int64_t n, int64_t self_offset, const GateSpec& g, ScreenPlan* pl,
                             std::vector<int4>* table) {
    const int64_t rows_per_unit = TC_ROW_UNIT;
    SLIC_REQUIRE(g.gates && g.num_chunks >= 1 && g.num_chunks < 32768 && g.chunk_rows > 0 && g.chunk_rows % TC_ROW_UNIT == 0,
                 "gated screen: chunk_rows must be a positive multiple of 256");
    SLIC_REQUIRE(ceil_div(n, g.chunk_rows) == g.num_chunks, "gated screen: chunks do not tile the database");
    SLIC_REQUIRE(self_offset >= 0 && self_offset + nq <= n, "gated screen: queries must be database rows");
    const int64_t row_units = ceil_div(nq, rows_per_unit);
    pl->tiles_per_split = (int)(g.chunk_rows / TC_BN);
    pl->splits = g.num_chunks;
    pl->units = row_units * pl->splits;
    table->clear();
    table->reserve((size_t)pl->units);
    for (int gate = 0; gate < g.num_chunks; ++gate)
        for (int s = 0; s <= gate; ++s)
            for (int64_t r = 0; r < row_units; ++r) {
                int64_t last = (r + 1) * rows_per_unit - 1;
                if (last > nq - 1) last = nq - 1;
                const int rc = (int)((last + self_offset) / g.chunk_rows);
                const int need = rc > s ? rc : s;
                if (need != gate) continue;
                const int64_t ct0 = (int64_t)s * pl->tiles_per_split;
                int64_t cnt = ceil_div(n, TC_BN) - ct0;
                if (cnt > pl->tiles_per_split) cnt = pl->tiles_per_split;
                table->push_back(unit_entry(r, ct0, (int)cnt, 1, gate, s, false));
            }
    SLIC_REQUIRE((int64_t)table->size() == pl->units, "gated screen: internal unit count mismatch");
    return SLIC_OK;
}

template <typename T>
static int nn_top1_sym_impl(const T* unit, const uint16_t* ub, int64_t n, int d, int d_pad, float eps, int* idx_out,
                            T* dist_out, int* stats_out, cudaStream_t st, int part, int parts, const GateSpec* gate,
                            AfterScreenFn after, void* after_ctx, bool* overflowed, int mode = 0,
                            const int* bests_in = nullptr, int* bests_out = nullptr, int* stats_ext = nullptr,
                            const ScreenPeers* peers = nullptr, AfterScreenFn before_screen = nullptr,
                            void* before_ctx = nullptr);
static bool screen_sym_allowed();
constexpr int64_t SYM_MIN_ROWS_FWD = 16384;

template <typename T>
static int nn_top1_impl(const T* q_unit, const uint16_t* q_f16, int64_t nq, const T* x_unit, const uint16_t* x_f16,
                        int64_t n, int d, int d_pad, int64_t self_offset, float eps, int* idx_out, T* dist_out,
                        int* stats_out, cudaStream_t st, const GateSpec* gate = nullptr, AfterScreenFn after = nullptr,
                        void* after_ctx = nullptr, int* stats_ext = nullptr) {
    if (q_f16 == x_f16 && q_unit == x_unit && nq == n && self_offset == 0 && n >= SYM_MIN_ROWS_FWD && screen_sym_allowed()) {
        bool overflowed = false;
        SLIC_PROPAGATE(nn_top1_sym_impl<T>(x_unit, x_f16, n, d, d_pad, eps, idx_out, dist_out, stats_out, st, 0, 1, gate,
                                           after, after_ctx, &overflowed, 0, nullptr, nullptr, stats_ext));
        if (stats_ext || !overflowed) return SLIC_OK;
        gate = nullptr;
        after = nullptr;
    }
    ScreenPlan pl = plan_screen(nq, n);
    std::vector<int4> table;
    Scratch table_dev;
    if (gate) {
        SLIC_PROPAGATE(plan_screen_gated(nq, n, self_offset, *gate, &pl, &table));
        SLIC_CUDA_OK(table_dev.alloc(table.size() * sizeof(int4), st));
        SLIC_PROPAGATE(stage_to_device(table_dev.ptr, table.data(), table.size() * sizeof(int4), st));
    }
    const int64_t slots = (int64_t)pl.splits * 2 * nq;
    Scratch ci, cs, cc, cf, ovr, stats;
    SLIC_CUDA_OK(ci.alloc(slots * TC_CAP * sizeof(int), st));
    SLIC_CUDA_OK(cs.alloc(slots * TC_CAP * sizeof(float), st));
    SLIC_CUDA_OK(cc.alloc(slots * sizeof(int), st));
    SLIC_CUDA_OK(cf.alloc(slots * sizeof(int), st));
    SLIC_CUDA_OK(ovr.alloc(nq * sizeof(int), st));
    int* stats_dev = stats_ext;
    if (!stats_dev) {
        SLIC_CUDA_OK(stats.alloc(8 * sizeof(int), st));
        stats_dev = stats.as<int>();
    }
    SLIC_CUDA_OK(cudaMemsetAsync(stats_dev, 0, 8 * sizeof(int), st));
    SLIC_PROPAGATE(launch_screen(q_f16, nq, x_f16, n, d_pad, self_offset, eps, TC_CAP, pl, ci.as<int>(), cs.as<float>(),
                                 cc.as<int>(), cf.as<int>(), nullptr, stats_dev + 4, st, 0, nullptr,
                                 gate ? table_dev.as<int4>() : nullptr, gate ? gate->gates : nullptr));
    if (after) SLIC_PROPAGATE(after(after_ctx));
    rerank_top1_kernel<T><<<(unsigned)ceil_div(nq, 8), 256, 0, st>>>(q_unit, x_unit, nq, d, eps, TC_CAP, 2 * pl.splits,
                                                                     ci.as<int>(), cs.as<float>(), cc.as<int>(),
                                                                     cf.as<int>(), idx_out, dist_out, ovr.as<int>(),
                                                                     stats_dev);
    SLIC_LAUNCH_OK();
    if (stats_ext) return SLIC_OK;
    int host_stats[8];
    SLIC_CUDA_OK(cudaMemcpyAsync(host_stats, stats_dev, sizeof(host_stats), cudaMemcpyDeviceToHost, st));
    SLIC_CUDA_OK(cudaStreamSynchronize(st));
    if (host_stats[4] != 0) {
        set_error("nn_screen_kernel: pipeline barrier timed out");
        return SLIC_ERR_CUDA;
    }
    const int n_over = host_stats[1];
    if (n_over > 0) {
        Scratch oi, od;
        SLIC_CUDA_OK(oi.alloc((int64_t)n_over * sizeof(int), st));
        SLIC_CUDA_OK(od.alloc((int64_t)n_over * sizeof(T), st));
        SLIC_PROPAGATE(slic_nn_exact_top1(q_unit, ovr.as<int>(), n_over, x_unit, n, d,
                                          sizeof(T) == 4 ? SLIC_F32 : SLIC_F64, self_offset, oi.as<int>(), od.ptr, st));
        scatter_rows_kernel<T><<<(unsigned)ceil_div(n_over, 256), 256, 0, st>>>(ovr.as<int>(), n_over, oi.as<int>(),
                                                                                od.as<T>(), idx_out, dist_out);
        SLIC_LAUNCH_OK();
    }
    if (stats_out) SLIC_CUDA_OK(cudaMemcpyAsync(stats_out, stats_dev, 4 * sizeof(int), cudaMemcpyDeviceToDevice, st));
    return SLIC_OK;
}

template <typename T>
static int topk_tc_impl(const T* q_unit, const uint16_t* q_f16, int64_t nq, const T* x_unit, const uint16_t* x_f16,
                        int64_t n, int d, int d_pad, int k, int64_t self_offset, float eps, int* idx_out, T* dist_out,
                        int* stats_out, cudaStream_t st) {
    const ScreenPlan pl = plan_screen_topk(nq, n, k);
    const int TC_CAP_TOPK = topk_cap(k, (int64_t)pl.tiles_per_split * (TC_BN / 2));
    const int64_t slots = (int64_t)pl.splits * 2 * nq;
    Scratch ci, cs, cc, cf, ck, ctb, ovr, stats;
    SLIC_CUDA_OK(ctb.alloc(slots * sizeof(int), st));
    SLIC_CUDA_OK(cudaMemsetAsync(ctb.ptr, 0, slots * sizeof(int), st));
    SLIC_CUDA_OK(ci.alloc(slots * TC_CAP_TOPK * sizeof(int), st));
    SLIC_CUDA_OK(cs.alloc(slots * TC_CAP_TOPK * sizeof(float), st));
    SLIC_CUDA_OK(cc.alloc(slots * sizeof(int), st));
    SLIC_CUDA_OK(cf.alloc(slots * sizeof(int), st));
    SLIC_CUDA_OK(ck.alloc(slots * sizeof(float), st));
    SLIC_CUDA_OK(ovr.alloc(nq * sizeof(int), st));
    SLIC_CUDA_OK(stats.alloc(8 * sizeof(int), st));
    SLIC_CUDA_OK(cudaMemsetAsync(stats.ptr, 0, 8 * sizeof(int), st));
    SLIC_PROPAGATE(launch_screen(q_f16, nq, x_f16, n, d_pad, self_offset, eps, TC_CAP_TOPK, pl, ci.as<int>(),
                                 cs.as<float>(), cc.as<int>(), cf.as<int>(), nullptr, stats.as<int>() + 4, st, k,
                                 ck.as<float>(), nullptr, nullptr, nullptr, 0, nullptr, 0, nullptr, nullptr, nullptr,
                                 ctb.as<int>()));
    rerank_topk_kernel<T><<<(unsigned)nq, RK_THREADS, 0, st>>>(q_unit, x_unit, nq, d, eps, TC_CAP_TOPK, 2 * pl.splits, k,
                                                               ci.as<int>(), cs.as<float>(), cc.as<int>(), cf.as<int>(),
                                                               ck.as<float>(), idx_out, dist_out, ovr.as<int>(),
                                                               stats.as<int>());
    SLIC_LAUNCH_OK();
    int host_stats[8];
    SLIC_CUDA_OK(cudaMemcpyAsync(host_stats, stats.ptr, sizeof(host_stats), cudaMemcpyDeviceToHost, st));
    SLIC_CUDA_OK(cudaStreamSynchronize(st));
    if (host_stats[4] != 0) {
        set_error("nn_screen_kernel: pipeline barrier timed out");
        return SLIC_ERR_CUDA;
    }
    const int n_over = host_stats[1];
    if (n_over > 0) {
        Scratch oi, od;
        SLIC_CUDA_OK(oi.alloc((int64_t)n_over * k * sizeof(int), st));
        SLIC_CUDA_OK(od.alloc((int64_t)n_over * k * sizeof(T), st));
        SLIC_PROPAGATE(exact_topk_cosine_rows(q_unit, ovr.as<int>(), n_over, x_unit, n, d,
                                              sizeof(T) == 4 ? SLIC_F32 : SLIC_F64, k, self_offset, oi.as<int>(), od.ptr,
                                              st));
        scatter_topk_rows_kernel<T><<<(unsigned)ceil_div((int64_t)n_over * k, 256), 256, 0, st>>>(
            ovr.as<int>(), n_over, k, oi.as<int>(), od.as<T>(), idx_out, dist_out);
        SLIC_LAUNCH_OK();
    }
    if (stats_out) SLIC_CUDA_OK(cudaMemcpyAsync(stats_out, stats.ptr, 4 * sizeof(int), cudaMemcpyDeviceToDevice, st));
    return SLIC_OK;
}

constexpr int SYM_LOG_PER_ROW = 96;
constexpr int64_t SYM_LOG_MIN = (int64_t)1 << 23;

static bool screen_sym_allowed();
bool screen_self_search_is_symmetric(int64_t n) { return n >= SYM_MIN_ROWS_FWD && screen_sym_allowed(); }
static bool screen_sym_allowed() {
    static int cached = -1;
    if (cached < 0) {
        const char* e = getenv("SLIC_SCREEN_SYM");
        cached = (e && atoi(e) == 0) ? 0 : 1;
    }
    return cached != 0;
}

__global__ void flip_sign_bit_kernel(const unsigned int* __restrict__ in, int64_t n, unsigned int* __restrict__ out) {
    const int64_t i = (int64_t)blockIdx.x * blockDim.x + threadIdx.x;
    if (i < n) out[i] = in[i] ^ 0x80000000u;
}

__global__ void sym_init_kernel(int* __restrict__ stats8, int* __restrict__ lcnt, int64_t regions,
                                unsigned char* __restrict__ rmin_bytes, int64_t rmin_n_bytes, int* __restrict__ sync_counter,
                                unsigned int* __restrict__ best, const unsigned int* __restrict__ bests_in, int64_t n,
                                unsigned int* __restrict__ idx_out) {
    const int64_t i = (int64_t)blockIdx.x * blockDim.x + threadIdx.x;
    if (i < 8) stats8[i] = 0;
    if (i == 0) *sync_counter = 0;
    if (i < regions) lcnt[i] = 0;
    if (i < n) {
        best[i] = bests_in ? (bests_in[i] ^ 0x80000000u) : ENC_NEG_INF;
        if (idx_out) idx_out[i] = 0x7fffffffu;
    }
    const int64_t b = i * 16;
    if (b + 16 <= rmin_n_bytes) *reinterpret_cast<uint4*>(rmin_bytes + b) = make_uint4(~0u, ~0u, ~0u, ~0u);
    else
        for (int64_t k = b; k < rmin_n_bytes; ++k) rmin_bytes[k] = 0xff;
}

__global__ void fill_u32_kernel(unsigned int* out, int64_t n, unsigned int v) {
    const int64_t i = (int64_t)blockIdx.x * blockDim.x + threadIdx.x;
    if (i < n) out[i] = v;
}

template <typename T> struct DistBits;
template <> struct DistBits<float> {
    typedef unsigned int type;
    static __device__ __forceinline__ type of(float d) { return __float_as_uint(d); }
    static __device__ __forceinline__ float back(type b) { return __uint_as_float(b); }
};
template <> struct DistBits<double> {
    typedef unsigned long long type;
    static __device__ __forceinline__ type of(double d) { return (type)__double_as_longlong(d); }
    static __device__ __forceinline__ double back(type b) { return __longlong_as_double((long long)b); }
};

template <typename T>
__global__ void __launch_bounds__(256) sym_rerank_dist_kernel(const T* __restrict__ unit, int d, float eps, int region,
                                                              const int* __restrict__ log_q, const int* __restrict__ log_nb,
                                                              const float* __restrict__ log_s,
                                                              const int* __restrict__ log_cnt,
                                                              const unsigned int* __restrict__ best_enc,
                                                              typename DistBits<T>::type* __restrict__ row_min,
                                                              T* __restrict__ edist, int* __restrict__ stats) {
    const int lane = threadIdx.x & 31, warp = threadIdx.x >> 5, nwarps = blockDim.x >> 5;
    const int64_t base = (int64_t)blockIdx.x * region;
    const int cnt = log_cnt[blockIdx.x];
    if (threadIdx.x == 0) {
        atomicAdd(&stats[3], cnt >> 4);
        atomicMax(&stats[6], cnt);
    }
    int reranked = 0;
    for (int e0 = warp * 32; e0 < cnt; e0 += nwarps * 32) {
        const int e = e0 + lane;
        int q = 0, nb = 0;
        bool keep = false;
        if (e < cnt) {
            q = log_q[base + e];
            nb = log_nb[base + e];
            keep = log_s[base + e] >= dec_score(best_enc[q]) - eps;
            if (!keep) edist[base + e] = (T)-1;
        }
        unsigned mask = __ballot_sync(0xffffffffu, keep);
        while (mask) {
            const int src = __ffs(mask) - 1;
            mask &= mask - 1;
            const int qq = __shfl_sync(0xffffffffu, q, src), nn = __shfl_sync(0xffffffffu, nb, src);
            const double sim = warp_dot<T>(unit + (int64_t)qq * d, unit + (int64_t)nn * d, d, lane);
            if (lane == 0) {
                const T dist = cosine_distance_from_sim<T>(sim);
                edist[base + e0 + src] = dist;
                atomicMin(row_min + qq, DistBits<T>::of(dist));
            }
            ++reranked;
        }
    }
    if (lane == 0 && reranked) atomicAdd(&stats[0], reranked);
}

template <typename T>
__global__ void __launch_bounds__(256) sym_rerank_pick_kernel(int region, const int* __restrict__ log_q,
                                                              const int* __restrict__ log_nb,
                                                              const int* __restrict__ log_cnt,
                                                              const typename DistBits<T>::type* __restrict__ row_min,
                                                              const T* __restrict__ edist, int* __restrict__ idx_out,
                                                              T* __restrict__ dist_out) {
    const int64_t base = (int64_t)blockIdx.x * region;
    const int cnt = log_cnt[blockIdx.x];
    for (int e = threadIdx.x; e < cnt; e += blockDim.x) {
        const T dist = edist[base + e];
        if (dist < (T)0) continue;
        const int q = log_q[base + e];
        if (DistBits<T>::of(dist) == row_min[q]) {
            atomicMin(idx_out + q, log_nb[base + e]);
            if (dist_out) dist_out[q] = dist;
        }
    }
}

__global__ void sym_unsettled_rows_kernel(int* __restrict__ idx_out, int64_t n, int* __restrict__ rows, int* __restrict__ stats) {
    const int64_t i = (int64_t)blockIdx.x * blockDim.x + threadIdx.x;
    if (i < n && idx_out[i] == 0x7fffffff) rows[atomicAdd(&stats[1], 1)] = (int)i;
}

template <typename T>
static int nn_top1_sym_impl(const T* unit, const uint16_t* ub, int64_t n, int d, int d_pad, float eps, int* idx_out,
                            T* dist_out, int* stats_out, cudaStream_t st, int part, int parts, const GateSpec* gate,
                            AfterScreenFn after, void* after_ctx, bool* overflowed, int mode, const int* bests_in,
                            int* bests_out, int* stats_ext, const ScreenPeers* peers, AfterScreenFn before_screen,
                            void* before_ctx) {
    typedef typename DistBits<T>::type Bits;
    *overflowed = false;
    ScreenPlan pl;
    std::vector<int4> table;
    int64_t prepass_units_all = 0;
    SLIC_PROPAGATE(plan_screen_sym(n, part, parts, gate, &pl, &table, (SymMode)mode, &prepass_units_all));
    SLIC_REQUIRE((mode == SYM_FUSED) == (peers != nullptr), "symmetric screen: the fused mode needs peer windows (and only it)");
    SLIC_REQUIRE(mode != SYM_FUSED || (stats_ext && !gate), "symmetric screen: the fused mode is asynchronous and ungated");
    int64_t exec_tiles = 0;
    for (const int4& e : table) exec_tiles += e.z & 0xffff;
    const int num_gates = gate ? gate->num_chunks : 0;
    std::vector<int> targets(num_gates + 1, 0);
    for (const int4& e : table) {
        if ((e.w >> 28) & 1) continue;
        const int g = (e.w & 0xfff) - 1;
        for (int k = g + 1; k <= num_gates; ++k) targets[k] += 2 * TC_EPI_WARPS;
    }
    if (mode == SYM_FUSED) targets[0] = (int)(prepass_units_all * 2 * TC_EPI_WARPS);
    const int64_t groups = num_sms() / 2;
    const int64_t grid = (pl.units < groups ? pl.units : groups) * 2;
    const int64_t regions = grid * TC_EPI_WARPS;
    int64_t capacity = (int64_t)SYM_LOG_PER_ROW * n > SYM_LOG_MIN ? (int64_t)SYM_LOG_PER_ROW * n : SYM_LOG_MIN;
    if (mode == SYM_BESTS) capacity = SYM_LOG_MIN;
    const int64_t region = ceil_div(capacity, regions);
    SLIC_REQUIRE(region < ((int64_t)1 << 31), "symmetric screen: log region too large");
    Scratch table_dev, lq, lnb, ls, lcnt, best, rmin, edist, ovr, stats;
    const size_t table_bytes = table.size() * sizeof(int4);
    SLIC_CUDA_OK(table_dev.alloc(table_bytes + (targets.size() + 4) * sizeof(int), st));
    {
        std::vector<unsigned char> blob(table_bytes + (targets.size() + 1) * sizeof(int));
        memcpy(blob.data(), table.data(), table_bytes);
        const int zero = 0;
        memcpy(blob.data() + table_bytes, &zero, sizeof(int));
        memcpy(blob.data() + table_bytes + sizeof(int), targets.data(), targets.size() * sizeof(int));
        SLIC_PROPAGATE(stage_to_device(table_dev.ptr, blob.data(), blob.size(), st));
    }
    int* sync_dev = reinterpret_cast<int*>(static_cast<unsigned char*>(table_dev.ptr) + table_bytes);
    SLIC_CUDA_OK(lq.alloc(regions * region * sizeof(int), st));
    SLIC_CUDA_OK(lnb.alloc(regions * region * sizeof(int), st));
    SLIC_CUDA_OK(ls.alloc(regions * region * sizeof(float), st));
    SLIC_CUDA_OK(edist.alloc(regions * region * sizeof(T), st));
    SLIC_CUDA_OK(lcnt.alloc(regions * sizeof(int), st));
    if (!peers) SLIC_CUDA_OK(best.alloc(n * sizeof(unsigned int), st));
    unsigned int* best_dev = peers ? peers->own_best : best.as<unsigned int>();
    int* sync_counter_dev = peers ? peers->own_sync : sync_dev;
    SLIC_CUDA_OK(rmin.alloc(n * sizeof(Bits), st));
    SLIC_CUDA_OK(ovr.alloc(n * sizeof(int), st));
    int* stats_dev = stats_ext;
    if (!stats_dev) {
        SLIC_CUDA_OK(stats.alloc(8 * sizeof(int), st));
        stats_dev = stats.as<int>();
    }
    int* flag_dev = stats_dev + 5;
    {
        const int64_t rmin_bytes = n * (int64_t)sizeof(Bits);
        int64_t threads = n > regions ? n : regions;
        if (ceil_div(rmin_bytes, 16) > threads) threads = ceil_div(rmin_bytes, 16);
        if (threads < 8) threads = 8;
        sym_init_kernel<<<(unsigned)ceil_div(threads, 256), 256, 0, st>>>(stats_dev, lcnt.as<int>(), regions,
                                                                         static_cast<unsigned char*>(rmin.ptr), rmin_bytes,
                                                                         sync_counter_dev, best_dev,
                                                                         (const unsigned int*)bests_in, n, (unsigned int*)idx_out);
        SLIC_LAUNCH_OK();
    }
    if (before_screen) SLIC_PROPAGATE(before_screen(before_ctx));
    SLIC_PROPAGATE(launch_screen(ub, n, ub, n, d_pad, 0, eps, 0, pl, lnb.as<int>(), ls.as<float>(), lcnt.as<int>(),
                                 flag_dev, nullptr, stats_dev + 4, st, 0, nullptr, table_dev.as<int4>(),
                                 gate ? gate->gates : nullptr, best_dev, exec_tiles, lq.as<int>(),
                                 (int)region, sync_counter_dev, sync_dev + 1, peers));
    if (g_profile && parts > 1) g_last_flop /= (double)parts;
    if (after) SLIC_PROPAGATE(after(after_ctx));
    if (mode == SYM_BESTS) {
        flip_sign_bit_kernel<<<(unsigned)ceil_div(n, 256), 256, 0, st>>>(best_dev, n, (unsigned int*)bests_out);
        SLIC_LAUNCH_OK();
        int host_err = 0;
        SLIC_CUDA_OK(cudaMemcpyAsync(&host_err, stats_dev + 4, sizeof(int), cudaMemcpyDeviceToHost, st));
        SLIC_CUDA_OK(cudaStreamSynchronize(st));
        if (host_err != 0) {
            set_error(host_err == 2 ? "nn_screen_kernel: shared-memory window is not aligned as the symmetric layout assumes"
                                    : "nn_screen_kernel: pipeline barrier timed out");
            return SLIC_ERR_CUDA;
        }
        return SLIC_OK;
    }
    sym_rerank_dist_kernel<T><<<(unsigned)regions, 256, 0, st>>>(unit, d, eps, (int)region, lq.as<int>(), lnb.as<int>(),
                                                                 ls.as<float>(), lcnt.as<int>(), best_dev,
                                                                 rmin.as<Bits>(), edist.as<T>(), stats_dev);
    SLIC_LAUNCH_OK();
    sym_rerank_pick_kernel<T><<<(unsigned)regions, 256, 0, st>>>((int)region, lq.as<int>(), lnb.as<int>(), lcnt.as<int>(),
                                                                 rmin.as<Bits>(), edist.as<T>(), idx_out, dist_out);
    SLIC_LAUNCH_OK();
    sym_unsettled_rows_kernel<<<(unsigned)ceil_div(n, 256), 256, 0, st>>>(idx_out, n, ovr.as<int>(), stats_dev);
    SLIC_LAUNCH_OK();
    if (stats_ext) return SLIC_OK;
    int host_stats[8];
    SLIC_CUDA_OK(cudaMemcpyAsync(host_stats, stats_dev, sizeof(host_stats), cudaMemcpyDeviceToHost, st));
    SLIC_CUDA_OK(cudaStreamSynchronize(st));
    if (host_stats[4] == 2) {
        set_error("nn_screen_kernel: shared-memory window is not aligned as the symmetric layout assumes (set SLIC_SCREEN_SYM=0)");
        return SLIC_ERR_UNSUPPORTED;
    }
    if (host_stats[4] != 0) {
        set_error("nn_screen_kernel: pipeline barrier timed out");
        return SLIC_ERR_CUDA;
    }
    if (const char* dbg = getenv("SLIC_SYM_DEBUG")) {
        if (atoi(dbg) == 2) {
            std::vector<int> hq((size_t)(regions * region)), hnb((size_t)(regions * region)), hc((size_t)regions);
            std::vector<float> hs((size_t)(regions * region));
            cudaMemcpy(hq.data(), lq.ptr, hq.size() * 4, cudaMemcpyDeviceToHost);
            cudaMemcpy(hnb.data(), lnb.ptr, hnb.size() * 4, cudaMemcpyDeviceToHost);
            cudaMemcpy(hs.data(), ls.ptr, hs.size() * 4, cudaMemcpyDeviceToHost);
            cudaMemcpy(hc.data(), lcnt.ptr, hc.size() * 4, cudaMemcpyDeviceToHost);
            FILE* f = fopen("/tmp/slic_sym_log.bin", "wb");
            if (f) {
                long long hdr[3] = {(long long)n, (long long)regions, (long long)region};
                fwrite(hdr, sizeof(hdr), 1, f);
                fwrite(hc.data(), 4, hc.size(), f);
                fwrite(hq.data(), 4, hq.size(), f);
                fwrite(hnb.data(), 4, hnb.size(), f);
                fwrite(hs.data(), 4, hs.size(), f);
                fclose(f);
            }
        }
    }
    if (host_stats[5] != 0) {
        if (getenv("SLIC_SYM_DEBUG"))
            fprintf(stderr, "[slic] symmetric screen: log overflow, n=%lld regions=%lld region=%lld records=%d fullest=%d\n",
                    (long long)n, (long long)regions, (long long)region, host_stats[3] * 16, host_stats[6]);
        *overflowed = true;
        return SLIC_OK;
    }
    if (getenv("SLIC_SYM_DEBUG"))
        fprintf(stderr, "[slic] symmetric screen: n=%lld regions=%lld region=%lld records=%d fullest=%d\n", (long long)n,
                (long long)regions, (long long)region, host_stats[3] * 16, host_stats[6]);
    const int n_over = host_stats[1];
    if (n_over > 0 && parts == 1) {
        Scratch oi, od;
        SLIC_CUDA_OK(oi.alloc((int64_t)n_over * sizeof(int), st));
        SLIC_CUDA_OK(od.alloc((int64_t)n_over * sizeof(T), st));
        SLIC_PROPAGATE(slic_nn_exact_top1(unit, ovr.as<int>(), n_over, unit, n, d, sizeof(T) == 4 ? SLIC_F32 : SLIC_F64, 0,
                                          oi.as<int>(), od.ptr, st));
        scatter_rows_kernel<T><<<(unsigned)ceil_div(n_over, 256), 256, 0, st>>>(ovr.as<int>(), n_over, oi.as<int>(),
                                                                                od.as<T>(), idx_out, dist_out);
        SLIC_LAUNCH_OK();
    }
    if (stats_out) SLIC_CUDA_OK(cudaMemcpyAsync(stats_out, stats_dev, 4 * sizeof(int), cudaMemcpyDeviceToDevice, st));
    return SLIC_OK;
}

__global__ void sym_pack_keys_kernel(const int* __restrict__ idx, const float* __restrict__ dist, int64_t n,
                                     unsigned long long* __restrict__ keys) {
    const int64_t i = (int64_t)blockIdx.x * blockDim.x + threadIdx.x;
    if (i >= n) return;
    const int j = idx[i];
    keys[i] = j == 0x7fffffff ? SYM_KEY_NONE : (((unsigned long long)__float_as_uint(dist[i]) << 32) | (unsigned int)j);
}

__global__ void sym_unpack_keys_kernel(const unsigned long long* __restrict__ keys, int64_t n, int* __restrict__ idx,
                                       float* __restrict__ dist, int* __restrict__ unsettled) {
    const int64_t i = (int64_t)blockIdx.x * blockDim.x + threadIdx.x;
    if (i >= n) return;
    const unsigned long long k = keys[i];
    idx[i] = (int)(unsigned int)(k & 0xffffffffull);
    dist[i] = __uint_as_float((unsigned int)(k >> 32));
    if (k == SYM_KEY_NONE) atomicAdd(unsettled, 1);
}

bool screen_can_overlap_upload(int64_t n, int d_pad, int guest_threads, int guest_regs) {
    const bool sym = screen_self_search_is_symmetric(n);
    KernelFn fn;
    size_t smem_bytes;
    pick_screen_kernel(sym, screen_ares(d_pad), false, &fn, &smem_bytes);
    cudaFuncAttributes fa;
    if (cudaFuncGetAttributes(&fa, fn) != cudaSuccess) {
        cudaGetLastError();
        return false;
    }
    const int host_regs = (fa.numRegs + 7) / 8 * 8, gr = (guest_regs + 7) / 8 * 8;
    const int host_threads = sym ? TC_THREADS_SYM : TC_THREADS;
    const int host_warps = (host_threads / 32 + 3) / 4, guest_warps = (guest_threads / 32 + 3) / 4;
    const bool regs_ok = 32 * (host_warps * host_regs + guest_warps * gr) <= 16384;
    const bool smem_ok = smem_bytes + 2 * 1024 <= 233472;
    const bool threads_ok = host_threads + guest_threads <= 2048;
    if (getenv("SLIC_SYM_DEBUG"))
        fprintf(stderr, "[slic] overlap check: screen %d regs, %zu B smem; guest %d threads x %d regs -> regs %d smem %d\n",
                fa.numRegs, smem_bytes, guest_threads, guest_regs, (int)regs_ok, (int)smem_ok);
    return regs_ok && smem_ok && threads_ok;
}

int nn_top1_f32_gated(const float* q_unit, const uint16_t* q_f16, int64_t nq, const float* x_unit,
                      const uint16_t* x_f16, int64_t n, int d, int d_pad, int64_t self_offset, float eps, int* idx_out,
                      float* dist_out, int* stats_out, const GateSpec* gate, AfterScreenFn after, void* after_ctx,
                      cudaStream_t st, int* stats_ext) {
    if (eps <= 0.f) eps = TC_DEFAULT_EPS;
    return nn_top1_impl<float>(q_unit, q_f16, nq, x_unit, x_f16, n, d, d_pad, self_offset, eps, idx_out, dist_out,
                               stats_out, st, gate, after, after_ctx, stats_ext);
}

int nn_top1_self_async(const void* unit, const uint16_t* ub, int64_t n, int d, int d_pad, int dtype, int* idx_out,
                       void* dist_out, int* stats_ext, cudaStream_t st) {
    if (dtype == SLIC_F32)
        return nn_top1_impl<float>((const float*)unit, ub, n, (const float*)unit, ub, n, d, d_pad, 0, TC_DEFAULT_EPS,
                                   idx_out, (float*)dist_out, nullptr, st, nullptr, nullptr, nullptr, stats_ext);
    return nn_top1_impl<double>((const double*)unit, ub, n, (const double*)unit, ub, n, d, d_pad, 0, TC_DEFAULT_EPS, idx_out,
                                (double*)dist_out, nullptr, st, nullptr, nullptr, nullptr, stats_ext);
}

int nn_top1_sym_fused(const float* unit, const uint16_t* ub, int64_t n, int d, int d_pad, int part, int parts,
                      const ScreenPeers* peers, AfterScreenFn before_screen, void* before_ctx, int* idx_out,
                      float* dist_out, int* stats_dev, cudaStream_t st) {
    if (!screen_self_search_is_symmetric(n)) {
        set_error("fused multi-GPU search: the symmetric screen needs n >= %lld rows", (long long)SYM_MIN_ROWS_FWD);
        return SLIC_ERR_UNSUPPORTED;
    }
    bool overflowed = false;
    return nn_top1_sym_impl<float>(unit, ub, n, d, d_pad, TC_DEFAULT_EPS, idx_out, dist_out, nullptr, st, part, parts, nullptr,
                                   nullptr, nullptr, &overflowed, SYM_FUSED, nullptr, nullptr, stats_dev, peers,
                                   before_screen, before_ctx);
}

}

extern "C" {

int slic_nn_top1(const void* q_unit_dev, const uint16_t* q_f16_dev, int64_t nq, const void* x_unit_dev,
                 const uint16_t* x_f16_dev, int64_t n, int32_t d, int32_t d_pad, int32_t dtype, int64_t self_offset,
                 float eps, int32_t* idx_out_dev, void* dist_out_dev, int32_t* stats_out_dev, slic_stream_t stream) {
    SLIC_REQUIRE(nq > 0 && n > 1 && n < ((int64_t)1 << 31) && nq < ((int64_t)1 << 31), "nn_top1: bad shape");
    SLIC_REQUIRE(d > 0 && d_pad >= d && d_pad % 64 == 0, "nn_top1: d_pad must be a multiple of 64 >= d");
    SLIC_REQUIRE(q_unit_dev && q_f16_dev && x_unit_dev && x_f16_dev && idx_out_dev, "nn_top1: null pointer");
    SLIC_REQUIRE(dtype == SLIC_F32 || dtype == SLIC_F64, "nn_top1: bad dtype");
    SLIC_REQUIRE((reinterpret_cast<uintptr_t>(q_f16_dev) & 15) == 0 && (reinterpret_cast<uintptr_t>(x_f16_dev) & 15) == 0,
                 "nn_top1: f16 matrices must be 16-byte aligned");
    SLIC_PROPAGATE(slic_require_device());
    if (eps <= 0.f) eps = slic::TC_DEFAULT_EPS;
    cudaStream_t st = slic::as_stream(stream);
    if (dtype == SLIC_F32)
        return slic::nn_top1_impl<float>((const float*)q_unit_dev, q_f16_dev, nq, (const float*)x_unit_dev, x_f16_dev,
                                         n, d, d_pad, self_offset, eps, idx_out_dev, (float*)dist_out_dev,
                                         stats_out_dev, st);
    return slic::nn_top1_impl<double>((const double*)q_unit_dev, q_f16_dev, nq, (const double*)x_unit_dev, x_f16_dev, n,
                                      d, d_pad, self_offset, eps, idx_out_dev, (double*)dist_out_dev, stats_out_dev,
                                      st);
}

int slic_sym_row_bests(const float* unit_dev, const uint16_t* f16_dev, int64_t n, int32_t d, int32_t d_pad, int32_t part,
                       int32_t parts, int32_t* bests_out_dev, slic_stream_t stream) {
    using namespace slic;
    SLIC_REQUIRE(n > 1 && n < ((int64_t)1 << 31), "sym_row_bests: bad shape");
    SLIC_REQUIRE(d > 0 && d_pad >= d && d_pad % 64 == 0, "sym_row_bests: d_pad must be a multiple of 64 >= d");
    SLIC_REQUIRE(unit_dev && f16_dev && bests_out_dev, "sym_row_bests: null pointer");
    SLIC_REQUIRE(parts >= 1 && part >= 0 && part < parts, "sym_row_bests: part must be in [0, parts)");
    SLIC_REQUIRE((reinterpret_cast<uintptr_t>(f16_dev) & 15) == 0, "sym_row_bests: f16 matrix must be 16-byte aligned");
    SLIC_PROPAGATE(slic_require_device());
    if (!screen_self_search_is_symmetric(n)) {
        set_error("sym_row_bests: the symmetric screen needs n >= %lld rows (and SLIC_SCREEN_SYM != 0)", (long long)SYM_MIN_ROWS_FWD);
        return SLIC_ERR_UNSUPPORTED;
    }
    bool overflowed = false;
    return nn_top1_sym_impl<float>(unit_dev, f16_dev, n, d, d_pad, TC_DEFAULT_EPS, nullptr, nullptr, nullptr,
                                   as_stream(stream), part, parts, nullptr, nullptr, nullptr, &overflowed, SYM_BESTS, nullptr,
                                   bests_out_dev);
}

int slic_nn_top1_sym_part(const float* unit_dev, const uint16_t* f16_dev, int64_t n, int32_t d, int32_t d_pad,
                          int32_t part, int32_t parts, const int32_t* row_bests_dev, float eps, uint64_t* keys_out_dev,
                          int32_t* stats_out_dev, slic_stream_t stream) {
    using namespace slic;
    SLIC_REQUIRE(n > 1 && n < ((int64_t)1 << 31), "nn_top1_sym_part: bad shape");
    SLIC_REQUIRE(d > 0 && d_pad >= d && d_pad % 64 == 0, "nn_top1_sym_part: d_pad must be a multiple of 64 >= d");
    SLIC_REQUIRE(unit_dev && f16_dev && keys_out_dev, "nn_top1_sym_part: null pointer");
    SLIC_REQUIRE(parts >= 1 && part >= 0 && part < parts, "nn_top1_sym_part: part must be in [0, parts)");
    SLIC_REQUIRE((reinterpret_cast<uintptr_t>(f16_dev) & 15) == 0, "nn_top1_sym_part: f16 matrix must be 16-byte aligned");
    SLIC_PROPAGATE(slic_require_device());
    if (!screen_self_search_is_symmetric(n)) {
        set_error("nn_top1_sym_part: the symmetric screen needs n >= %lld rows (and SLIC_SCREEN_SYM != 0)",
                  (long long)SYM_MIN_ROWS_FWD);
        return SLIC_ERR_UNSUPPORTED;
    }
    if (eps <= 0.f) eps = TC_DEFAULT_EPS;
    cudaStream_t st = as_stream(stream);
    Scratch idx, dist;
    SLIC_CUDA_OK(idx.alloc((size_t)n * sizeof(int), st));
    SLIC_CUDA_OK(dist.alloc((size_t)n * sizeof(float), st));
    bool overflowed = false;
    SLIC_PROPAGATE(nn_top1_sym_impl<float>(unit_dev, f16_dev, n, d, d_pad, eps, idx.as<int>(), dist.as<float>(),
                                           stats_out_dev, st, part, parts, nullptr, nullptr, nullptr, &overflowed,
                                           row_bests_dev ? SYM_TRIANGLE : SYM_FULL, row_bests_dev, nullptr));
    sym_pack_keys_kernel<<<(unsigned)ceil_div(n, 256), 256, 0, st>>>(idx.as<int>(), dist.as<float>(), n,
                                                                     (unsigned long long*)keys_out_dev);
    SLIC_LAUNCH_OK();
    const unsigned long long flag = overflowed ? 0ull : 1ull;
    SLIC_CUDA_OK(cudaMemcpyAsync(keys_out_dev + n, &flag, sizeof(flag), cudaMemcpyHostToDevice, st));
    SLIC_CUDA_OK(cudaStreamSynchronize(st));
    return SLIC_OK;
}

int slic_debug_sym_plan(int64_t n, int32_t part, int32_t parts, int32_t mode, int32_t gated_chunks, int32_t* units_out_host,
                        int64_t capacity, int64_t* num_units_out_host) {
    using namespace slic;
    SLIC_REQUIRE(n > 1 && n < ((int64_t)1 << 31) && num_units_out_host, "debug_sym_plan: bad arguments");
    SLIC_REQUIRE(mode >= 0 && mode <= 3, "debug_sym_plan: mode must be 0 (full), 1 (row bests), 2 (triangle) or 3 (fused)");
    SLIC_REQUIRE(gated_chunks >= 0 && gated_chunks < 4095, "debug_sym_plan: bad chunk count");
    GateSpec gs = {reinterpret_cast<const int*>(num_units_out_host) , 0, 0};
    if (gated_chunks > 0) {
        gs.chunk_rows = ceil_div(ceil_div(n, gated_chunks), 256) * 256;
        gs.num_chunks = (int)ceil_div(n, gs.chunk_rows);
    }
    ScreenPlan pl;
    std::vector<int4> table;
    SLIC_PROPAGATE(plan_screen_sym(n, part, parts, gated_chunks > 0 ? &gs : nullptr, &pl, &table, (SymMode)mode));
    *num_units_out_host = (int64_t)table.size();
    if (units_out_host) {
        SLIC_REQUIRE(capacity >= (int64_t)table.size(), "debug_sym_plan: unit buffer too small");
        for (size_t u = 0; u < table.size(); ++u) {
            const int4 e = table[u];
            int32_t* o = units_out_host + 6 * u;
            o[0] = e.x;
            o[1] = e.y;
            o[2] = e.z & 0xffff;
            o[3] = (int)((unsigned)e.z >> 16);
            o[4] = (e.w & 0xfff) - 1;
            o[5] = (e.w >> 28) & 1;
        }
    }
    return SLIC_OK;
}

int slic_unpack_neighbor_keys(const uint64_t* keys_dev, int64_t n, int32_t* idx_out_dev, float* dist_out_dev,
                              int32_t* status_out_dev, slic_stream_t stream) {
    using namespace slic;
    SLIC_REQUIRE(n > 0 && keys_dev && idx_out_dev && dist_out_dev && status_out_dev, "unpack_neighbor_keys: bad argument");
    SLIC_PROPAGATE(slic_require_device());
    cudaStream_t st = as_stream(stream);
    SLIC_CUDA_OK(cudaMemsetAsync(status_out_dev, 0, sizeof(int), st));
    sym_unpack_keys_kernel<<<(unsigned)ceil_div(n, 256), 256, 0, st>>>((const unsigned long long*)keys_dev, n, idx_out_dev,
                                                                       dist_out_dev, status_out_dev);
    SLIC_LAUNCH_OK();
    return SLIC_OK;
}

int slic_topk_cosine_tc(const void* q_unit_dev, const uint16_t* q_f16_dev, int64_t nq, const void* x_unit_dev,
                        const uint16_t* x_f16_dev, int64_t n, int32_t d, int32_t d_pad, int32_t dtype, int32_t k,
                        int64_t self_offset, float eps, int32_t* idx_out_dev, void* dist_out_dev, int32_t* stats_out_dev,
                        slic_stream_t stream) {
    SLIC_REQUIRE(nq >= 0 && n > 0 && n < ((int64_t)1 << 31) && nq < ((int64_t)1 << 31), "topk_cosine_tc: bad shape");
    SLIC_REQUIRE(d > 0 && d_pad >= d && d_pad % 64 == 0, "topk_cosine_tc: d_pad must be a multiple of 64 >= d");
    SLIC_REQUIRE(k > 0 && k <= slic::TC_TOPK_MAX && k <= n - (self_offset >= 0 ? 1 : 0),
                 "topk_cosine_tc: k must satisfy 1 <= k <= min(64, columns available)");
    SLIC_REQUIRE(q_unit_dev && q_f16_dev && x_unit_dev && x_f16_dev && idx_out_dev, "topk_cosine_tc: null pointer");
    SLIC_REQUIRE(dtype == SLIC_F32 || dtype == SLIC_F64, "topk_cosine_tc: bad dtype");
    SLIC_REQUIRE((reinterpret_cast<uintptr_t>(q_f16_dev) & 15) == 0 && (reinterpret_cast<uintptr_t>(x_f16_dev) & 15) == 0,
                 "topk_cosine_tc: f16 matrices must be 16-byte aligned");
    if (nq == 0) return SLIC_OK;
    SLIC_PROPAGATE(slic_require_device());
    if (eps <= 0.f) eps = slic::TC_DEFAULT_EPS;
    cudaStream_t st = slic::as_stream(stream);
    if (dtype == SLIC_F32)
        return slic::topk_tc_impl<float>((const float*)q_unit_dev, q_f16_dev, nq, (const float*)x_unit_dev, x_f16_dev,
                                         n, d, d_pad, k, self_offset, eps, idx_out_dev, (float*)dist_out_dev,
                                         stats_out_dev, st);
    return slic::topk_tc_impl<double>((const double*)q_unit_dev, q_f16_dev, nq, (const double*)x_unit_dev, x_f16_dev, n,
                                      d, d_pad, k, self_offset, eps, idx_out_dev, (double*)dist_out_dev, stats_out_dev,
                                      st);
}

int slic_profile_screen(int32_t enable) {
    slic::g_profile = enable != 0;
    slic::g_have_sample = false;
    return SLIC_OK;
}

int slic_screen_trace(int32_t enable, uint64_t* counters_out_host) {
    using namespace slic;
    if (counters_out_host && g_trace) {
        SLIC_CUDA_OK(cudaDeviceSynchronize());
        SLIC_CUDA_OK(cudaMemcpy(counters_out_host, g_trace, 12 * sizeof(uint64_t), cudaMemcpyDeviceToHost));
    }
    if (enable && !g_trace) {
        SLIC_CUDA_OK(cudaMalloc(&g_trace, 12 * sizeof(uint64_t)));
    } else if (!enable && g_trace) {
        SLIC_CUDA_OK(cudaDeviceSynchronize());
        SLIC_CUDA_OK(cudaFree(g_trace));
        g_trace = nullptr;
    }
    if (g_trace) SLIC_CUDA_OK(cudaMemset(g_trace, 0, 12 * sizeof(uint64_t)));
    return SLIC_OK;
}

int slic_last_screen_time(float* ms_out, double* flop_out) {
    SLIC_REQUIRE(ms_out && flop_out, "last_screen_time: null pointer");
    if (!slic::g_have_sample) {
        slic::set_error("last_screen_time: no profiled launch (call slic_profile_screen(1) first)");
        return SLIC_ERR_INVALID_ARG;
    }
    SLIC_CUDA_OK(cudaEventSynchronize(slic::g_ev_stop));
    SLIC_CUDA_OK(cudaEventElapsedTime(ms_out, slic::g_ev_start, slic::g_ev_stop));
    *flop_out = slic::g_last_flop;
    return SLIC_OK;
}

int slic_last_screen_exec_flop(double* flop_out) {
    SLIC_REQUIRE(flop_out, "last_screen_exec_flop: null pointer");
    *flop_out = slic::g_have_sample ? slic::g_last_exec_flop : 0.0;
    return SLIC_OK;
}

int slic_screen_scores_debug(const uint16_t* q_f16_dev, int64_t nq, const uint16_t* x_f16_dev, int64_t n,
                             int32_t d_pad, float* out_dev, slic_stream_t stream) {
    using namespace slic;
    SLIC_REQUIRE(nq > 0 && n > 0 && d_pad > 0 && d_pad % 64 == 0, "screen_scores_debug: bad shape");
    SLIC_REQUIRE(q_f16_dev && x_f16_dev && out_dev, "screen_scores_debug: null pointer");
    SLIC_PROPAGATE(slic_require_device());
    cudaStream_t st = as_stream(stream);
    const ScreenPlan pl = plan_screen(nq, n);
    const int64_t slots = (int64_t)pl.splits * 2 * nq;
    Scratch ci, cs, cc, cf, err;
    SLIC_CUDA_OK(ci.alloc(slots * TC_CAP * sizeof(int), st));
    SLIC_CUDA_OK(cs.alloc(slots * TC_CAP * sizeof(float), st));
    SLIC_CUDA_OK(cc.alloc(slots * sizeof(int), st));
    SLIC_CUDA_OK(cf.alloc(slots * sizeof(int), st));
    SLIC_CUDA_OK(err.alloc(sizeof(int), st));
    SLIC_CUDA_OK(cudaMemsetAsync(err.ptr, 0, sizeof(int), st));
    SLIC_PROPAGATE(launch_screen(q_f16_dev, nq, x_f16_dev, n, d_pad, -1, TC_DEFAULT_EPS, TC_CAP, pl, ci.as<int>(),
                                 cs.as<float>(), cc.as<int>(), cf.as<int>(), out_dev, err.as<int>(), st));
    int host_err = 0;
    SLIC_CUDA_OK(cudaMemcpyAsync(&host_err, err.ptr, sizeof(int), cudaMemcpyDeviceToHost, st));
    SLIC_CUDA_OK(cudaStreamSynchronize(st));
    if (host_err) {
        set_error("nn_screen_kernel: pipeline barrier timed out");
        return SLIC_ERR_CUDA;
    }
    return SLIC_OK;
}

}
```

Measured before the change: 8.972 million.

## Add int8 tile-bound pruning pass before the symmetric f16 nearest-neighbour screen

Adds a pruned self-search path. Rows are quantised to int8 per unit, and an int8 tcgen05 MMA pass computes a per-tile maximum score bound. Tiles whose bound cannot beat a row's current best are dropped, and the f16 screen then runs only on the compacted survivor tiles before the exact re-rank. The goal is to skip most of the f16 GEMM work in the full-hierarchy FINCH nearest-neighbour search. The cost is extra quantise, bound, keep and compact kernels and a device-side unit count, plus more code paths where correctness depends on the bound being conservative.

```diff
diff --git a/include/slic_b200.h b/include/slic_b200.h
--- a/include/slic_b200.h
+++ b/include/slic_b200.h
@@ -34,6 +34,10 @@
 int slic_profile_screen(int32_t enable);
 int slic_last_screen_time(float* ms_out, double* flop_out);
 int slic_last_screen_exec_flop(double* flop_out);
+int slic_pruned_screen_info(double* out_host);
+int slic_last_pruned_perm(int32_t* perm_out_dev, int64_t n);
+int slic_debug_quantise_units(const void* unit_dev, int64_t n, int32_t d, int32_t d_pad, int32_t dtype, int8_t* q_out_dev,
+                              double* scale_out_dev, double* rmax_out_dev, slic_stream_t stream);
 
 int slic_screen_trace(int32_t enable, uint64_t* counters_out_host);
 
diff --git a/video_similarity_search_b200/_lib.py b/video_similarity_search_b200/_lib.py
--- a/video_similarity_search_b200/_lib.py
+++ b/video_similarity_search_b200/_lib.py
@@ -15,6 +15,9 @@
     "slic_profile_screen": [_i32],
     "slic_last_screen_time": [_ptr, _ptr],
     "slic_last_screen_exec_flop": [_ptr],
+    "slic_pruned_screen_info": [_ptr],
+    "slic_last_pruned_perm": [_ptr, _i64],
+    "slic_debug_quantise_units": [_ptr, _i64, _i32, _i32, _i32, _ptr, _ptr, _ptr, _ptr],
     "slic_screen_trace": [_i32, _ptr],
     "slic_normalize_rows": [_ptr, _i64, _i32, _i32, _ptr, _ptr, _ptr, _i32, _ptr],
     "slic_center_columns": [_ptr, _i64, _i32, _ptr, _ptr, _ptr],
diff --git a/video_similarity_search_b200/csrc/nn_screen_tc.cu b/video_similarity_search_b200/csrc/nn_screen_tc.cu
--- a/video_similarity_search_b200/csrc/nn_screen_tc.cu
+++ b/video_similarity_search_b200/csrc/nn_screen_tc.cu
@@ -1,5 +1,6 @@
 #include <cuda.h>
 #include <cuda_fp16.h>
+#include <limits.h>
 #include <math.h>
 #include <stdlib.h>
 #include <string.h>
@@ -86,6 +87,8 @@
     int num_peers;
     unsigned int* peer_best[SLIC_MAX_PEERS];
     int* peer_sync[SLIC_MAX_PEERS];
+    int* tile_max;
+    const int* num_units_dev;
 };
 
 struct UnitInfo {
@@ -366,6 +369,17 @@
     return d;
 }
 constexpr uint32_t TC_IDESC = (1u << 4) | ((uint32_t)(TC_BN >> 3) << 17) | ((uint32_t)((2 * TC_BM) >> 4) << 24);
+constexpr uint32_t TC_IDESC_I8 = (2u << 4) | (1u << 7) | (1u << 10) | ((uint32_t)(TC_BN >> 3) << 17) |
+                                 ((uint32_t)((2 * TC_BM) >> 4) << 24);
+__device__ __forceinline__ void umma_i8_pair(uint32_t tmem_d, uint64_t desc_a, uint64_t desc_b, uint32_t idesc,
+                                              uint32_t accumulate) {
+    asm volatile(
+        "{\n\t.reg .pred p;\n\t"
+        "setp.ne.b32 p, %4, 0;\n\t"
+        "tcgen05.mma.cta_group::2.kind::i8 [%0], %1, %2, %3, p;\n\t}"
+        ::"r"(tmem_d), "l"(desc_a), "l"(desc_b), "r"(idesc), "r"(accumulate)
+        : "memory");
+}
 
 struct RowState {
     float best, thr;
@@ -666,13 +680,15 @@
 }
 
 constexpr int TC_TOP1_MAX_REGS = 152;
-template <bool TOPK, bool ARES, bool SYM = false>
+template <bool TOPK, bool ARES, bool SYM = false, bool I8 = false>
 __global__ void __maxnreg__(TOPK ? 168 : TC_TOP1_MAX_REGS) nn_screen_kernel(const __grid_constant__ CUtensorMap tmap_q,
                                                                   const __grid_constant__ CUtensorMap tmap_x,
                                                                   const ScreenParams p) {
     typedef TcCfg<ARES, TOPK> Cfg;
     constexpr int STAGES = Cfg::STAGES;
     static_assert(!SYM || !TOPK, "the symmetric variant exists for the top-1 kernels only");
+    static_assert(!I8 || (ARES && !SYM && !TOPK), "the int8 bound pass is an A-resident, non-symmetric launch");
+    constexpr int SLAB_K = I8 ? 2 * TC_BK : TC_BK;
     extern __shared__ uint8_t smem_raw[];
     uint8_t* smem = reinterpret_cast<uint8_t*>((reinterpret_cast<uintptr_t>(smem_raw) + 1023) & ~(uintptr_t)1023);
     {
@@ -756,11 +772,12 @@
             uint32_t phase = 0, a_phase = 0;
             unsigned long long t_wait = 0;
             const bool scheduler = cta_rank == 0;
+            const int64_t num_units = p.num_units_dev ? (int64_t)*p.num_units_dev : p.num_units;
             int u_next = scheduler ? atomicAdd(p.queue, 1) : 0;
             while (true) {
                 int u;
                 if (scheduler) {
-                    u = u_next < p.num_units ? u_next : -1;
+                    u = u_next < num_units ? u_next : -1;
                     mbar_wait_cluster(bar_uq_empty + 8u * ring.slot, ring.phase ^ 1u, p.error_flag);
 #pragma unroll
                     for (uint32_t r = 0; r < 2u; ++r) {
@@ -787,7 +804,7 @@
                     mbar_wait_traced(bar_a_empty, a_phase ^ 1, p.error_flag, t_wait, tracing);
                     if (cta_rank == 0) mbar_expect_tx(bar_a_full, 2 * (uint32_t)p.num_k_slabs * TC_A_BYTES);
                     for (int ks = 0; ks < p.num_k_slabs; ++ks)
-                        tma_load_2d_pair(&tmap_q, smem_base + ks * TC_A_BYTES, bar_a_full, ks * TC_BK,
+                        tma_load_2d_pair(&tmap_q, smem_base + ks * TC_A_BYTES, bar_a_full, ks * SLAB_K,
                                          (int)(row_block * TC_BM));
                     a_phase ^= 1;
                 }
@@ -801,7 +818,7 @@
                             const int nsl = min(Cfg::SPS, p.num_k_slabs - ks);
                             if (cta_rank == 0) mbar_expect_tx(bar_full + 8 * stage, 2 * (uint32_t)nsl * Cfg::B_BYTES);
                             for (int j = 0; j < nsl; ++j)
-                                tma_load_2d_pair(&tmap_x, b_dst + j * Cfg::SLAB_BYTES, bar_full + 8 * stage, (ks + j) * TC_BK,
+                                tma_load_2d_pair(&tmap_x, b_dst + j * Cfg::SLAB_BYTES, bar_full + 8 * stage, (ks + j) * SLAB_K,
                                                  (int)(ct * TC_BN + cta_rank * Cfg::B_ROWS));
                         } else {
                             const int nsl = min(Cfg::SPS, p.num_k_slabs - ks);
@@ -859,8 +876,12 @@
                                 const uint64_t db = umma_smem_desc(ARES ? sl_addr : sl_addr + TC_A_BYTES);
 #pragma unroll
                                 for (int k = 0; k < TC_BK / TC_UMMA_K; ++k) {
-                                    umma_f16_pair(tmem_d, da + (uint64_t)(2 * k), db + (uint64_t)(2 * k), TC_IDESC,
-                                                  (uint32_t)((ks | j | k) != 0));
+                                    if constexpr (I8)
+                                        umma_i8_pair(tmem_d, da + (uint64_t)(2 * k), db + (uint64_t)(2 * k), TC_IDESC_I8,
+                                                     (uint32_t)((ks | j | k) != 0));
+                                    else
+                                        umma_f16_pair(tmem_d, da + (uint64_t)(2 * k), db + (uint64_t)(2 * k), TC_IDESC,
+                                                      (uint32_t)((ks | j | k) != 0));
                                 }
                             }
                         }
@@ -920,6 +941,38 @@
                 ++cseq;
             }
         }
+    } else if (I8) {
+        const int quad = warp & 3;
+        const int half = (warp - 2) >> 2;
+        unsigned seq_all = 0;
+        for (int u; (u = ring_take(ring, true, p.error_flag)) >= 0;) {
+            const UnitInfo ui = unit_info(p, u, n_col_tiles);
+            for (int kt = 0; kt < ui.count; ++kt, ++seq_all) {
+                const int acc = (int)(seq_all % (unsigned)TC_ACCS);
+                mbar_wait(bar_acc_full + 8 * acc, (seq_all / (unsigned)TC_ACCS) & 1u, p.error_flag);
+                tc_fence_after();
+                const uint32_t tbase = tmem_base + ((uint32_t)(quad * 32) << 16) + (uint32_t)(acc * TC_BN + half * 128);
+                uint32_t va[32], vb[32];
+                int m = INT_MIN;
+                tmem_ld_issue(tbase, va);
+#pragma unroll 1
+                for (int h = 0; h < 2; ++h) {
+                    tmem_ld_wait(va);
+                    tmem_ld_issue(tbase + (uint32_t)(64 * h + 32), vb);
+#pragma unroll
+                    for (int t = 0; t < 32; ++t) m = max(m, (int)va[t]);
+                    tmem_ld_wait(vb);
+                    if (h == 0) tmem_ld_issue(tbase + 64u, va);
+#pragma unroll
+                    for (int t = 0; t < 32; ++t) m = max(m, (int)vb[t]);
+                }
+                tc_fence_before();
+                __syncwarp();
+                if (lane == 0) mbar_arrive_leader(bar_acc_empty + 8 * acc);
+                m = __reduce_max_sync(0xffffffffu, m);
+                if (lane == 0) atomicMax(p.tile_max + ui.row_unit * n_col_tiles + ui.ct0 + (int64_t)kt * ui.stride, m);
+            }
+        }
     } else {
         const int quad = warp & 3;
         const int half = (warp - 2) >> 2;
@@ -938,7 +991,7 @@
         unsigned tile_seq = 0;
         const int64_t log_region_id = (int64_t)blockIdx.x * TC_EPI_WARPS + (warp - 2);
         if constexpr (SYM) {
-            if (lane == 0) *s_logcnt = 0u;
+            if (lane == 0) *s_logcnt = (unsigned)p.cand_cnt[log_region_id];
             __syncwarp();
             cx.lg.q = p.log_q + log_region_id * p.log_region;
             cx.lg.nb = p.cand_idx + log_region_id * p.log_region;
@@ -1358,14 +1411,15 @@
     return SLIC_OK;
 }
 
-static int make_tmap(CUtensorMap* map, const uint16_t* base, int64_t rows, int d_pad, int box_rows) {
+static int make_tmap(CUtensorMap* map, const void* base, int64_t rows, int d_pad, int box_rows, bool i8 = false) {
     EncodeTiledFn enc;
     SLIC_PROPAGATE(get_encode_fn(&enc));
     cuuint64_t gdim[2] = {(cuuint64_t)d_pad, (cuuint64_t)rows};
-    cuuint64_t gstride[1] = {(cuuint64_t)d_pad * 2};
-    cuuint32_t box[2] = {(cuuint32_t)TC_BK, (cuuint32_t)box_rows};
+    cuuint64_t gstride[1] = {(cuuint64_t)d_pad * (i8 ? 1 : 2)};
+    cuuint32_t box[2] = {(cuuint32_t)(i8 ? 2 * TC_BK : TC_BK), (cuuint32_t)box_rows};
     cuuint32_t estr[2] = {1, 1};
-    CUresult r = enc(map, CU_TENSOR_MAP_DATA_TYPE_FLOAT16, 2, const_cast<uint16_t*>(base), gdim, gstride, box, estr,
+    CUresult r = enc(map, i8 ? CU_TENSOR_MAP_DATA_TYPE_UINT8 : CU_TENSOR_MAP_DATA_TYPE_FLOAT16, 2, const_cast<void*>(base),
+                     gdim, gstride, box, estr,
                      CU_TENSOR_MAP_INTERLEAVE_NONE, CU_TENSOR_MAP_SWIZZLE_128B, CU_TENSOR_MAP_L2_PROMOTION_L2_256B,
                      CU_TENSOR_MAP_FLOAT_OOB_FILL_NONE);
     if (r != CUDA_SUCCESS) {
@@ -1377,8 +1431,32 @@
 
 static bool g_profile = false, g_have_sample = false;
 static unsigned long long* g_trace = nullptr;
-static cudaEvent_t g_ev_start = nullptr, g_ev_stop = nullptr;
-static double g_last_flop = 0.0, g_last_exec_flop = 0.0;
+static double g_last_flop = 0.0;
+struct ProfiledLaunch {
+    cudaEvent_t start = nullptr, stop = nullptr;
+    double exec_flop = 0.0;
+};
+static std::vector<ProfiledLaunch> g_prof;
+static size_t g_prof_used = 0;
+static bool g_profile_keep = false;
+static void g_prune_info_reset();
+static bool g_prune_info_valid();
+static int profile_begin(ProfiledLaunch** out, cudaStream_t st) {
+    if (!g_profile_keep) {
+        g_prof_used = 0;
+        g_prune_info_reset();
+    }
+    if (g_prof_used == g_prof.size()) {
+        ProfiledLaunch l;
+        SLIC_CUDA_OK(cudaEventCreate(&l.start));
+        SLIC_CUDA_OK(cudaEventCreate(&l.stop));
+        g_prof.push_back(l);
+    }
+    *out = &g_prof[g_prof_used++];
+    SLIC_CUDA_OK(cudaEventRecord((*out)->start, st));
+    g_have_sample = true;
+    return SLIC_OK;
+}
 
 struct ScreenPlan {
     int splits, tiles_per_split;
@@ -1479,15 +1557,19 @@
                          float* cand_kth = nullptr, const int4* unit_table = nullptr, const int* gates = nullptr,
                          unsigned int* best_enc = nullptr, int64_t exec_tiles = 0, int* log_q = nullptr,
                          int log_region = 0, int* sync_counter = nullptr, const int* sync_targets = nullptr,
-                         const ScreenPeers* peers = nullptr, int* cand_tb = nullptr) {
+                         const ScreenPeers* peers = nullptr, int* cand_tb = nullptr, int* tile_max = nullptr,
+                         const int* num_units_dev = nullptr) {
+    const bool i8 = tile_max != nullptr;
     if (gates) SLIC_PROPAGATE(arm_timeout_record());
     CUtensorMap tq, tx;
-    SLIC_PROPAGATE(make_tmap(&tq, q_f16, nq, d_pad, TC_BM));
-    SLIC_PROPAGATE(make_tmap(&tx, x_f16, n, d_pad, TC_BN / 2));
+    SLIC_PROPAGATE(make_tmap(&tq, q_f16, nq, d_pad, TC_BM, i8));
+    SLIC_PROPAGATE(make_tmap(&tx, x_f16, n, d_pad, TC_BN / 2, i8));
     ScreenParams p;
     p.nq = nq;
     p.n = n;
-    p.num_k_slabs = d_pad / TC_BK;
+    p.num_k_slabs = i8 ? (int)ceil_div(d_pad, 2 * TC_BK) : d_pad / TC_BK;
+    p.tile_max = tile_max;
+    p.num_units_dev = num_units_dev;
     p.self_offset = self_offset;
     p.eps = eps;
     p.cap = cap;
@@ -1529,31 +1611,34 @@
     p.queue = queue.as<int>();
     const bool sym = best_enc != nullptr;
     const bool is_topk = topk > 0;
-    const bool ares = screen_ares(d_pad);
+    const bool ares = i8 || screen_ares(d_pad);
     if (sym && (is_topk || !unit_table)) {
         set_error("symmetric screen: needs the top-1 kernel and a unit list");
         return SLIC_ERR_UNSUPPORTED;
     }
+    if (i8 && (sym || is_topk || !unit_table || p.num_k_slabs > TC_ARES_MAX_SLABS)) {
+        set_error("int8 bound pass: needs a unit list, the top-1 kernel and d_pad <= %d", TC_ARES_MAX_SLABS * 2 * TC_BK);
+        return SLIC_ERR_UNSUPPORTED;
+    }
     KernelFn fn;
     size_t smem_bytes;
     pick_screen_kernel(sym, ares, is_topk, &fn, &smem_bytes);
-    static bool attr_done[64][8] = {{false}};
+    if (i8) {
+        fn = (KernelFn)nn_screen_kernel<false, true, false, true>;
+        smem_bytes = TcCfg<true, false>::SMEM_BYTES;
+    }
+    static bool attr_done[64][9] = {{false}};
     int dev = 0;
     SLIC_CUDA_OK(cudaGetDevice(&dev));
-    bool& attr_set = attr_done[dev & 63][(sym ? 4 : 0) + (ares ? 2 : 0) + (is_topk ? 1 : 0)];
+    bool& attr_set = attr_done[dev & 63][i8 ? 8 : (sym ? 4 : 0) + (ares ? 2 : 0) + (is_topk ? 1 : 0)];
     if (!attr_set) {
         SLIC_CUDA_OK(cudaFuncSetAttribute(fn, cudaFuncAttributeMaxDynamicSharedMemorySize, (int)smem_bytes));
         attr_set = true;
     }
     const int64_t pairs = num_sms() / 2;
     const int64_t grid = (pl.units < pairs ? pl.units : pairs) * 2;
-    if (g_profile) {
-        if (!g_ev_start) {
-            SLIC_CUDA_OK(cudaEventCreate(&g_ev_start));
-            SLIC_CUDA_OK(cudaEventCreate(&g_ev_stop));
-        }
-        SLIC_CUDA_OK(cudaEventRecord(g_ev_start, st));
-    }
+    ProfiledLaunch* prof = nullptr;
+    if (g_profile) SLIC_PROPAGATE(profile_begin(&prof, st));
     cudaLaunchConfig_t cfg = {};
     cfg.gridDim = dim3((unsigned)grid);
     cfg.blockDim = dim3(sym ? TC_THREADS_SYM : TC_THREADS);
@@ -1568,11 +1653,12 @@
     cfg.numAttrs = 1;
     SLIC_CUDA_OK(cudaLaunchKernelEx(&cfg, fn, tq, tx, p));
     SLIC_LAUNCH_OK();
-    if (g_profile) {
-        SLIC_CUDA_OK(cudaEventRecord(g_ev_stop, st));
-        g_last_flop = 2.0 * (double)nq * (double)n * (double)d_pad;
-        g_last_exec_flop = exec_tiles > 0 ? 2.0 * (double)exec_tiles * TC_ROW_UNIT * TC_BN * (double)d_pad : g_last_flop;
-        g_have_sample = true;
+    if (prof) {
+        SLIC_CUDA_OK(cudaEventRecord(prof->stop, st));
+        const double flop = 2.0 * (double)nq * (double)n * (double)d_pad;
+        const double exec = exec_tiles > 0 ? 2.0 * (double)exec_tiles * TC_ROW_UNIT * TC_BN * (double)d_pad : flop;
+        prof->exec_flop = i8 ? exec / 2 : exec;
+        if (!g_profile_keep) g_last_flop = flop;
     }
     return SLIC_OK;
 }
@@ -1720,6 +1806,10 @@
                             const int* bests_in = nullptr, int* bests_out = nullptr, int* stats_ext = nullptr,
                             const ScreenPeers* peers = nullptr, AfterScreenFn before_screen = nullptr,
                             void* before_ctx = nullptr);
+template <typename T>
+static int nn_top1_pruned_impl(const T* unit, const uint16_t* ub, int64_t n, int d, int d_pad, float eps, int* idx_out,
+                               T* dist_out, int* stats_out, cudaStream_t st, bool* overflowed, int* stats_ext);
+static bool prune_applies(int64_t n, int d_pad);
 static bool screen_sym_allowed();
 constexpr int64_t SYM_MIN_ROWS_FWD = 16384;
 
@@ -1728,14 +1818,28 @@
                         int64_t n, int d, int d_pad, int64_t self_offset, float eps, int* idx_out, T* dist_out,
                         int* stats_out, cudaStream_t st, const GateSpec* gate = nullptr, AfterScreenFn after = nullptr,
                         void* after_ctx = nullptr, int* stats_ext = nullptr) {
+    bool keep_record = false;
     if (q_f16 == x_f16 && q_unit == x_unit && nq == n && self_offset == 0 && n >= SYM_MIN_ROWS_FWD && screen_sym_allowed()) {
         bool overflowed = false;
-        SLIC_PROPAGATE(nn_top1_sym_impl<T>(x_unit, x_f16, n, d, d_pad, eps, idx_out, dist_out, stats_out, st, 0, 1, gate,
-                                           after, after_ctx, &overflowed, 0, nullptr, nullptr, stats_ext));
+        const bool pruned = !gate && !after && prune_applies(n, d_pad);
+        if (pruned)
+            SLIC_PROPAGATE(nn_top1_pruned_impl<T>(x_unit, x_f16, n, d, d_pad, eps, idx_out, dist_out, stats_out, st,
+                                                  &overflowed, stats_ext));
+        else
+            SLIC_PROPAGATE(nn_top1_sym_impl<T>(x_unit, x_f16, n, d, d_pad, eps, idx_out, dist_out, stats_out, st, 0, 1, gate,
+                                               after, after_ctx, &overflowed, 0, nullptr, nullptr, stats_ext));
         if (stats_ext || !overflowed) return SLIC_OK;
         gate = nullptr;
         after = nullptr;
-    }
+        if (pruned && g_profile && g_prune_info_valid()) keep_record = true;
+    }
+    struct KeepRecord {
+        bool on;
+        ~KeepRecord() {
+            if (on) g_profile_keep = false;
+        }
+    } keep_guard{keep_record};
+    if (keep_record) g_profile_keep = true;
     ScreenPlan pl = plan_screen(nq, n);
     std::vector<int4> table;
     Scratch table_dev;
@@ -1900,7 +2004,8 @@
                                                               const int* __restrict__ log_cnt,
                                                               const unsigned int* __restrict__ best_enc,
                                                               typename DistBits<T>::type* __restrict__ row_min,
-                                                              T* __restrict__ edist, int* __restrict__ stats) {
+                                                              T* __restrict__ edist, int* __restrict__ stats,
+                                                              const int* __restrict__ perm = nullptr) {
     const int lane = threadIdx.x & 31, warp = threadIdx.x >> 5, nwarps = blockDim.x >> 5;
     const int64_t base = (int64_t)blockIdx.x * region;
     const int cnt = log_cnt[blockIdx.x];
@@ -1924,7 +2029,8 @@
             const int src = __ffs(mask) - 1;
             mask &= mask - 1;
             const int qq = __shfl_sync(0xffffffffu, q, src), nn = __shfl_sync(0xffffffffu, nb, src);
-            const double sim = warp_dot<T>(unit + (int64_t)qq * d, unit + (int64_t)nn * d, d, lane);
+            const int oq = perm ? __ldg(perm + qq) : qq, on = perm ? __ldg(perm + nn) : nn;
+            const double sim = warp_dot<T>(unit + (int64_t)oq * d, unit + (int64_t)on * d, d, lane);
             if (lane == 0) {
                 const T dist = cosine_distance_from_sim<T>(sim);
                 edist[base + e0 + src] = dist;
@@ -1942,7 +2048,7 @@
                                                               const int* __restrict__ log_cnt,
                                                               const typename DistBits<T>::type* __restrict__ row_min,
                                                               const T* __restrict__ edist, int* __restrict__ idx_out,
-                                                              T* __restrict__ dist_out) {
+                                                              T* __restrict__ dist_out, const int* __restrict__ perm = nullptr) {
     const int64_t base = (int64_t)blockIdx.x * region;
     const int cnt = log_cnt[blockIdx.x];
     for (int e = threadIdx.x; e < cnt; e += blockDim.x) {
@@ -1950,8 +2056,9 @@
         if (dist < (T)0) continue;
         const int q = log_q[base + e];
         if (DistBits<T>::of(dist) == row_min[q]) {
-            atomicMin(idx_out + q, log_nb[base + e]);
-            if (dist_out) dist_out[q] = dist;
+            const int oq = perm ? __ldg(perm + q) : q, on = perm ? __ldg(perm + log_nb[base + e]) : log_nb[base + e];
+            atomicMin(idx_out + oq, on);
+            if (dist_out) dist_out[oq] = dist;
         }
     }
 }
@@ -2109,6 +2216,522 @@
         SLIC_CUDA_OK(od.alloc((int64_t)n_over * sizeof(T), st));
         SLIC_PROPAGATE(slic_nn_exact_top1(unit, ovr.as<int>(), n_over, unit, n, d, sizeof(T) == 4 ? SLIC_F32 : SLIC_F64, 0,
                                           oi.as<int>(), od.ptr, st));
+        scatter_rows_kernel<T><<<(unsigned)ceil_div(n_over, 256), 256, 0, st>>>(ovr.as<int>(), n_over, oi.as<int>(),
+                                                                                od.as<T>(), idx_out, dist_out);
+        SLIC_LAUNCH_OK();
+    }
+    if (stats_out) SLIC_CUDA_OK(cudaMemcpyAsync(stats_out, stats_dev, 4 * sizeof(int), cudaMemcpyDeviceToDevice, st));
+    return SLIC_OK;
+}
+
+constexpr int64_t PRUNE_MIN_ROWS = 32768;
+constexpr int PRUNE_GROUP_ROWS = 64;
+constexpr int64_t PRUNE_MIN_SEEDS = 4096;
+constexpr int PRUNE_BAND_TILES = 4;
+constexpr int PRUNE_SAMPLE_EVERY = 64;
+constexpr float PRUNE_MAX_SURVIVAL = 0.35f;
+
+static bool prune_applies(int64_t n, int d_pad) {
+    return n >= PRUNE_MIN_ROWS && d_pad <= TC_ARES_MAX_SLABS * 2 * TC_BK && ceil_div(n, TC_ROW_UNIT) >= num_sms() / 2;
+}
+
+__global__ void strided_rows_kernel(int* __restrict__ rows, int64_t count, int64_t n) {
+    const int64_t i = (int64_t)blockIdx.x * blockDim.x + threadIdx.x;
+    if (i < count) rows[i] = (int)(i * n / count);
+}
+__global__ void gather_rows_kernel(const uint32_t* __restrict__ src, int64_t row_words, const int* __restrict__ idx,
+                                   int64_t count, uint32_t* __restrict__ dst) {
+    const int64_t total = count * row_words;
+    for (int64_t t = (int64_t)blockIdx.x * blockDim.x + threadIdx.x; t < total; t += (int64_t)gridDim.x * blockDim.x) {
+        const int64_t r = t / row_words;
+        dst[t] = __ldg(src + (int64_t)__ldg(idx + r) * row_words + (t - r * row_words));
+    }
+}
+__global__ void seed_rank_kernel(const int* __restrict__ order, int g, int* __restrict__ rank) {
+    const int i = blockIdx.x * blockDim.x + threadIdx.x;
+    if (i < g) rank[order[i]] = i;
+}
+__global__ void row_group_kernel(const int* __restrict__ assign, int64_t n, const int* __restrict__ rank, int g,
+                                 int* __restrict__ label) {
+    const int64_t i = (int64_t)blockIdx.x * blockDim.x + threadIdx.x;
+    if (i >= n) return;
+    const int a = assign[i];
+    label[i] = rank[(unsigned)a < (unsigned)g ? a : 0];
+}
+
+__device__ __forceinline__ double block_reduce_256(double v, bool is_max, double* sh) {
+    const int lane = threadIdx.x & 31, warp = threadIdx.x >> 5;
+#pragma unroll
+    for (int o = 16; o; o >>= 1) {
+        const double w = __shfl_xor_sync(0xffffffffu, v, o);
+        v = is_max ? fmax(v, w) : fmin(v, w);
+    }
+    __syncthreads();
+    if (lane == 0) sh[warp] = v;
+    __syncthreads();
+    v = sh[0];
+    for (int w = 1; w < 8; ++w) v = is_max ? fmax(v, sh[w]) : fmin(v, sh[w]);
+    return v;
+}
+template <typename T>
+__global__ void __launch_bounds__(256) quantise_units_kernel(const T* __restrict__ unit, const int* __restrict__ perm,
+                                                             int64_t n, int d, int d_pad, int8_t* __restrict__ q,
+                                                             double* __restrict__ scale, double* __restrict__ rmax) {
+    __shared__ double sh[8];
+    const int lane = threadIdx.x & 31, warp = threadIdx.x >> 5;
+    const int64_t r0 = (int64_t)blockIdx.x * TC_ROW_UNIT;
+    double m = 0.0;
+    for (int i = warp; i < TC_ROW_UNIT && r0 + i < n; i += 8) {
+        const T* x = unit + (int64_t)perm[r0 + i] * d;
+        for (int k = lane; k < d; k += 32) m = fmax(m, fabs((double)x[k]));
+    }
+    m = block_reduce_256(m, true, sh);
+    const double s = (double)((float)m / 127.0f);
+    double rm = 0.0;
+    for (int i = warp; i < TC_ROW_UNIT && r0 + i < n; i += 8) {
+        const T* x = unit + (int64_t)perm[r0 + i] * d;
+        int8_t* qr = q + (r0 + i) * d_pad;
+        double e2 = 0.0;
+        for (int k = lane; k < d_pad; k += 32) {
+            const double xv = k < d ? (double)x[k] : 0.0;
+            const double qi = s > 0.0 ? fmin(fmax(rint(xv / s), -127.0), 127.0) : 0.0;
+            qr[k] = (int8_t)qi;
+            const double e = xv - s * qi;
+            e2 = fma(e, e, e2);
+        }
+#pragma unroll
+        for (int o = 16; o; o >>= 1) e2 += __shfl_xor_sync(0xffffffffu, e2, o);
+        rm = fmax(rm, __dsqrt_ru(e2) * (1.0 + 0x1p-40));
+    }
+    rm = block_reduce_256(rm, true, sh);
+    if (threadIdx.x == 0) {
+        scale[blockIdx.x] = s;
+        rmax[blockIdx.x] = rm;
+    }
+}
+__global__ void __launch_bounds__(256) unit_lower_bound_kernel(const unsigned int* __restrict__ best_enc, int64_t n,
+                                                               float eps, double* __restrict__ lmin) {
+    __shared__ double sh[8];
+    const int64_t r = (int64_t)blockIdx.x * TC_ROW_UNIT + threadIdx.x;
+    double l = r < n ? (double)dec_score(best_enc[r]) - 0.5 * (double)eps : CUDART_INF;
+    l = block_reduce_256(l, false, sh);
+    if (threadIdx.x == 0) lmin[blockIdx.x] = l;
+}
+__device__ __forceinline__ bool tile_may_hold_neighbour(int acc, int64_t R, int64_t Tt, const double* scale,
+                                                        const double* rmax, const double* lmin) {
+    if (acc == INT_MIN) return true;
+    const double rR = rmax[R], rT = rmax[Tt];
+    const double hi = scale[R] * scale[Tt] * (double)acc + (rR + rT + rR * rT) * (1.0 + 0x1p-10) + 0x1p-30;
+    return hi >= fmin(lmin[R], lmin[Tt]) - 0x1p-20;
+}
+constexpr int PRUNE_CTL = 8;
+__global__ void __launch_bounds__(1024) prune_select_kernel(const int4* __restrict__ sample, int n_sample,
+                                                            const int* __restrict__ tile_max, int64_t T,
+                                                            const double* __restrict__ scale, const double* __restrict__ rmax,
+                                                            const double* __restrict__ lmin, int bound_units,
+                                                            float max_survival, int* __restrict__ ctl) {
+    __shared__ int s_tiles, s_kept;
+    if (threadIdx.x == 0) s_tiles = s_kept = 0;
+    __syncthreads();
+    int tiles = 0, kept = 0;
+    for (int e = threadIdx.x; e < n_sample; e += blockDim.x) {
+        const int4 u = sample[e];
+        for (int k = 0; k < (u.z & 0xffff); ++k) {
+            ++tiles;
+            kept += tile_may_hold_neighbour(tile_max[(int64_t)u.x * T + u.y + k], u.x, u.y + k, scale, rmax, lmin);
+        }
+    }
+    atomicAdd(&s_tiles, tiles);
+    atomicAdd(&s_kept, kept);
+    __syncthreads();
+    if (threadIdx.x == 0) {
+        const bool fallback = (float)s_kept > max_survival * (float)s_tiles;
+        ctl[0] = fallback ? 0 : bound_units;
+        ctl[1] = fallback ? 1 : 0;
+        ctl[5] = s_tiles;
+        ctl[6] = s_kept;
+    }
+}
+__global__ void prune_keep_kernel(const int4* __restrict__ seg, const int64_t* __restrict__ seg_off,
+                                  const int* __restrict__ tile_max, int64_t T, const double* __restrict__ scale,
+                                  const double* __restrict__ rmax, const double* __restrict__ lmin, int* __restrict__ ctl,
+                                  uint8_t* __restrict__ keep) {
+    const int4 s = seg[blockIdx.x];
+    const int k = threadIdx.x;
+    bool kp = false;
+    if (k < s.z) {
+        kp = ctl[1] != 0 || tile_may_hold_neighbour(tile_max[(int64_t)s.x * T + s.y + k], s.x, s.y + k, scale, rmax, lmin);
+        keep[seg_off[blockIdx.x] + k] = kp ? 1 : 0;
+    }
+    const int cnt = __syncthreads_count(kp);
+    if (threadIdx.x == 0) {
+        atomicAdd(&ctl[3], s.z);
+        atomicAdd(&ctl[4], cnt);
+    }
+}
+__device__ __forceinline__ int emit_runs(int4 s, const uint8_t* kp, int unit_len, int4* out) {
+    int units = 0, start = 0, cnt = 0;
+    for (int k = 0; k <= s.z; ++k) {
+        const bool in = k < s.z && kp[k];
+        if (in) {
+            if (cnt == 0) start = k;
+            ++cnt;
+        }
+        if (cnt > 0 && (!in || cnt == unit_len)) {
+            if (out) out[units] = make_int4(s.x, s.y + start, cnt | (1 << 16), (1 << 28));
+            ++units;
+            cnt = 0;
+        }
+    }
+    return units;
+}
+__global__ void __launch_bounds__(1024) prune_compact_kernel(const int4* __restrict__ seg, const int64_t* __restrict__ seg_off,
+                                                             int n_seg, const uint8_t* __restrict__ keep, int unit_len,
+                                                             int4* __restrict__ units_out, int* __restrict__ ctl) {
+    __shared__ int s_off[1024];
+    const int per = (n_seg + blockDim.x - 1) / blockDim.x;
+    const int s0 = min(n_seg, (int)threadIdx.x * per), s1 = min(n_seg, s0 + per);
+    int mine = 0;
+    for (int s = s0; s < s1; ++s) mine += emit_runs(seg[s], keep + seg_off[s], unit_len, nullptr);
+    s_off[threadIdx.x] = mine;
+    __syncthreads();
+    for (int o = 1; o < (int)blockDim.x; o <<= 1) {
+        const int v = threadIdx.x >= (unsigned)o ? s_off[threadIdx.x - o] : 0;
+        __syncthreads();
+        s_off[threadIdx.x] += v;
+        __syncthreads();
+    }
+    int at = s_off[threadIdx.x] - mine;
+    for (int s = s0; s < s1; ++s) at += emit_runs(seg[s], keep + seg_off[s], unit_len, units_out + at);
+    if (threadIdx.x == blockDim.x - 1) ctl[2] = s_off[threadIdx.x];
+}
+
+template <typename T>
+__global__ void __launch_bounds__(256) seed_probe_kernel(const T* __restrict__ seed_unit, const int* __restrict__ snn,
+                                                         int64_t g, int d, double* __restrict__ sim) {
+    const int lane = threadIdx.x & 31;
+    const int64_t i = ((int64_t)blockIdx.x * blockDim.x + threadIdx.x) >> 5;
+    if (i >= g) return;
+    const int j = snn[i];
+    const int64_t k = (i + g / 2) % g;
+    const double a = (unsigned)j < (unsigned)g ? warp_dot<T>(seed_unit + i * d, seed_unit + (int64_t)j * d, d, lane) : -1.0;
+    const double b = warp_dot<T>(seed_unit + i * d, seed_unit + k * d, d, lane);
+    if (lane == 0) {
+        sim[i] = a;
+        sim[g + i] = b;
+    }
+}
+constexpr double PRUNE_PROBE_GAP = 0.05;
+static bool probe_says_prune(std::vector<double>& h, int64_t g) {
+    auto median = [](double* b, double* e) {
+        std::nth_element(b, b + (e - b) / 2, e);
+        return b[(e - b) / 2];
+    };
+    const double nn = median(h.data(), h.data() + g);
+    const double bg = median(h.data() + g, h.data() + 2 * g);
+    for (int64_t i = g; i < 2 * g; ++i) h[i] = fabs(h[i] - bg);
+    const double sigma = 1.4826 * median(h.data() + g, h.data() + 2 * g);
+    return nn > bg + 4.5 * sigma + PRUNE_PROBE_GAP;
+}
+
+struct PruneInfo {
+    bool valid = false;
+    cudaEvent_t ev[6] = {};
+    int64_t band_tiles = 0;
+    int ctl[PRUNE_CTL] = {};
+    int path = 0;
+    int log_overflow = 0;
+    int* perm_dev = nullptr;
+    int64_t perm_cap = 0, perm_n = 0;
+};
+static PruneInfo g_prune_info;
+static void g_prune_info_reset() { g_prune_info.valid = false; }
+static bool g_prune_info_valid() { return g_prune_info.valid; }
+
+template <typename T>
+static int nn_top1_pruned_impl(const T* unit, const uint16_t* ub, int64_t n, int d, int d_pad, float eps, int* idx_out,
+                               T* dist_out, int* stats_out, cudaStream_t st, bool* overflowed, int* stats_ext) {
+    typedef typename DistBits<T>::type Bits;
+    *overflowed = false;
+    const int dtype = sizeof(T) == 4 ? SLIC_F32 : SLIC_F64;
+    const int64_t R = ceil_div(n, TC_ROW_UNIT), T_ = ceil_div(n, TC_BN);
+    SLIC_REQUIRE(T_ < 65536, "pruned screen: too many column tiles");
+    const int64_t pairs = num_sms() / 2;
+    const bool prof = g_profile;
+    PruneInfo& info = g_prune_info;
+    if (prof) {
+        for (cudaEvent_t& e : info.ev)
+            if (!e) SLIC_CUDA_OK(cudaEventCreate(&e));
+        SLIC_CUDA_OK(cudaEventRecord(info.ev[0], st));
+        g_prof_used = 0;
+        g_prune_info_reset();
+        g_profile_keep = true;
+    }
+    struct KeepOff {
+        ~KeepOff() { g_profile_keep = false; }
+    } keep_off;
+
+    const int64_t G = std::min<int64_t>(std::max<int64_t>(ceil_div(n, PRUNE_GROUP_ROWS), PRUNE_MIN_SEEDS), SYM_MIN_ROWS_FWD - 1);
+    Scratch seeds, seed_unit, seed_f16, assign, adist, astats, snn, sdist, comp, ncomp, sorder, soff, srank, label, perm,
+        poff, ubp;
+    SLIC_CUDA_OK(seeds.alloc(G * sizeof(int), st));
+    SLIC_CUDA_OK(seed_unit.alloc(G * d * sizeof(T), st));
+    SLIC_CUDA_OK(seed_f16.alloc(G * d_pad * sizeof(uint16_t), st));
+    strided_rows_kernel<<<(unsigned)ceil_div(G, 256), 256, 0, st>>>(seeds.as<int>(), G, n);
+    SLIC_LAUNCH_OK();
+    const int64_t unit_words = (int64_t)d * sizeof(T) / 4, f16_words = d_pad / 2;
+    gather_rows_kernel<<<(unsigned)std::min<int64_t>(ceil_div(G * unit_words, 256), 4096), 256, 0, st>>>(
+        reinterpret_cast<const uint32_t*>(unit), unit_words, seeds.as<int>(), G, seed_unit.as<uint32_t>());
+    SLIC_LAUNCH_OK();
+    gather_rows_kernel<<<(unsigned)std::min<int64_t>(ceil_div(G * f16_words, 256), 4096), 256, 0, st>>>(
+        reinterpret_cast<const uint32_t*>(ub), f16_words, seeds.as<int>(), G, seed_f16.as<uint32_t>());
+    SLIC_LAUNCH_OK();
+    SLIC_CUDA_OK(astats.alloc(8 * sizeof(int), st));
+    SLIC_CUDA_OK(snn.alloc(G * sizeof(int), st));
+    SLIC_CUDA_OK(sdist.alloc(G * sizeof(T), st));
+    SLIC_PROPAGATE(nn_top1_impl<T>(seed_unit.as<T>(), seed_f16.as<uint16_t>(), G, seed_unit.as<T>(), seed_f16.as<uint16_t>(),
+                                   G, d, d_pad, 0, eps, snn.as<int>(), sdist.as<T>(), nullptr, st, nullptr, nullptr, nullptr,
+                                   astats.as<int>()));
+    {
+        Scratch probe;
+        SLIC_CUDA_OK(probe.alloc(2 * G * sizeof(double), st));
+        seed_probe_kernel<T><<<(unsigned)ceil_div(G * 32, 256), 256, 0, st>>>(seed_unit.as<T>(), snn.as<int>(), G, d,
+                                                                              probe.as<double>());
+        SLIC_LAUNCH_OK();
+        std::vector<double> h((size_t)(2 * G));
+        SLIC_CUDA_OK(cudaMemcpyAsync(h.data(), probe.ptr, h.size() * sizeof(double), cudaMemcpyDeviceToHost, st));
+        SLIC_CUDA_OK(cudaStreamSynchronize(st));
+        if (!probe_says_prune(h, G)) {
+            SLIC_PROPAGATE(nn_top1_sym_impl<T>(unit, ub, n, d, d_pad, eps, idx_out, dist_out, stats_out, st, 0, 1, nullptr,
+                                               nullptr, nullptr, overflowed, 0, nullptr, nullptr, stats_ext));
+            if (prof) {
+                for (int i = 1; i < 6; ++i) SLIC_CUDA_OK(cudaEventRecord(info.ev[i], st));
+                info = PruneInfo{true, {info.ev[0], info.ev[1], info.ev[2], info.ev[3], info.ev[4], info.ev[5]}, 0, {}, 2, 0,
+                                 info.perm_dev, info.perm_cap, 0};
+                g_last_flop = 2.0 * (double)n * (double)n * (double)d_pad;
+            }
+            return SLIC_OK;
+        }
+    }
+    SLIC_CUDA_OK(assign.alloc(n * sizeof(int), st));
+    SLIC_CUDA_OK(adist.alloc(n * sizeof(T), st));
+    SLIC_PROPAGATE(nn_top1_impl<T>(unit, ub, n, seed_unit.as<T>(), seed_f16.as<uint16_t>(), G, d, d_pad, -1, eps,
+                                   assign.as<int>(), adist.as<T>(), nullptr, st, nullptr, nullptr, nullptr, astats.as<int>()));
+    SLIC_CUDA_OK(comp.alloc(G * sizeof(int), st));
+    SLIC_CUDA_OK(ncomp.alloc(sizeof(int), st));
+    SLIC_PROPAGATE(slic_finch_components(snn.as<int>(), G, 0, 0.0, nullptr, 0, dtype, nullptr, comp.as<int>(),
+                                         ncomp.as<int>(), (slic_stream_t)st));
+    SLIC_CUDA_OK(sorder.alloc(G * sizeof(int), st));
+    SLIC_CUDA_OK(soff.alloc((G + 1) * sizeof(int), st));
+    SLIC_PROPAGATE(slic_group_by_label(comp.as<int>(), G, (int)G, sorder.as<int>(), soff.as<int>(), (slic_stream_t)st));
+    SLIC_CUDA_OK(srank.alloc(G * sizeof(int), st));
+    seed_rank_kernel<<<(unsigned)ceil_div(G, 256), 256, 0, st>>>(sorder.as<int>(), (int)G, srank.as<int>());
+    SLIC_LAUNCH_OK();
+    SLIC_CUDA_OK(label.alloc(n * sizeof(int), st));
+    row_group_kernel<<<(unsigned)ceil_div(n, 256), 256, 0, st>>>(assign.as<int>(), n, srank.as<int>(), (int)G,
+                                                                 label.as<int>());
+    SLIC_LAUNCH_OK();
+    SLIC_CUDA_OK(perm.alloc(n * sizeof(int), st));
+    SLIC_CUDA_OK(poff.alloc((G + 1) * sizeof(int), st));
+    SLIC_PROPAGATE(slic_group_by_label(label.as<int>(), n, (int)G, perm.as<int>(), poff.as<int>(), (slic_stream_t)st));
+    SLIC_CUDA_OK(ubp.alloc(n * d_pad * sizeof(uint16_t), st));
+    gather_rows_kernel<<<(unsigned)std::min<int64_t>(ceil_div(n * f16_words, 256), 8192), 256, 0, st>>>(
+        reinterpret_cast<const uint32_t*>(ub), f16_words, perm.as<int>(), n, ubp.as<uint32_t>());
+    SLIC_LAUNCH_OK();
+    Scratch q8, scale, rmax, lmin;
+    SLIC_CUDA_OK(q8.alloc(n * d_pad, st));
+    SLIC_CUDA_OK(scale.alloc(R * sizeof(double), st));
+    SLIC_CUDA_OK(rmax.alloc(R * sizeof(double), st));
+    SLIC_CUDA_OK(lmin.alloc(R * sizeof(double), st));
+    quantise_units_kernel<T><<<(unsigned)R, 256, 0, st>>>(unit, perm.as<int>(), n, d, d_pad, q8.as<int8_t>(),
+                                                          scale.as<double>(), rmax.as<double>());
+    SLIC_LAUNCH_OK();
+    if (prof) SLIC_CUDA_OK(cudaEventRecord(info.ev[1], st));
+
+    std::vector<int4> band, bound, sample, segs;
+    std::vector<int64_t> seg_off;
+    int64_t band_tiles = 0, off_tiles = 0;
+    for (int64_t r = 0; r < R; ++r) {
+        const int64_t c0 = std::max<int64_t>(r - PRUNE_BAND_TILES, 0), c1 = std::min<int64_t>(r + PRUNE_BAND_TILES + 1, T_);
+        band.push_back(unit_entry(r, c0, (int)(c1 - c0), 1, -1, 0, false));
+        band_tiles += c1 - c0;
+    }
+    const int64_t chunk_tiles = SYM_CHUNK_TILES;
+    for (int64_t c0 = 0; c0 < T_; c0 += chunk_tiles) {
+        const int64_t c1 = std::min(c0 + chunk_tiles, T_);
+        for (int64_t r = 0; r < c1; ++r) {
+            const int64_t b = std::max(r + PRUNE_BAND_TILES + 1, c0);
+            if (b >= c1) continue;
+            segs.push_back(make_int4((int)r, (int)b, (int)(c1 - b), 0));
+            seg_off.push_back(off_tiles);
+            off_tiles += c1 - b;
+        }
+    }
+    int64_t unit_len = off_tiles / (pairs * 12);
+    unit_len = unit_len < 8 ? 8 : (unit_len > chunk_tiles ? chunk_tiles : unit_len);
+    for (const int4& s : segs)
+        for (int k = 0; k < s.z; k += (int)unit_len)
+            bound.push_back(unit_entry(s.x, s.y + k, (int)std::min<int64_t>(unit_len, s.z - k), 1, -1, 0, false));
+    for (size_t i = PRUNE_SAMPLE_EVERY / 2; i < bound.size(); i += PRUNE_SAMPLE_EVERY) sample.push_back(bound[i]);
+    if (sample.empty() && !bound.empty()) sample.push_back(bound[0]);
+    const size_t nb_band = band.size() * sizeof(int4), nb_bound = bound.size() * sizeof(int4),
+                 nb_sample = sample.size() * sizeof(int4), nb_seg = segs.size() * sizeof(int4),
+                 nb_off = seg_off.size() * sizeof(int64_t);
+    Scratch plan;
+    SLIC_CUDA_OK(plan.alloc(nb_band + nb_bound + nb_sample + nb_seg + nb_off, st));
+    {
+        std::vector<unsigned char> blob(nb_band + nb_bound + nb_sample + nb_seg + nb_off);
+        size_t o = 0;
+        memcpy(blob.data() + o, band.data(), nb_band), o += nb_band;
+        memcpy(blob.data() + o, bound.data(), nb_bound), o += nb_bound;
+        memcpy(blob.data() + o, sample.data(), nb_sample), o += nb_sample;
+        memcpy(blob.data() + o, segs.data(), nb_seg), o += nb_seg;
+        memcpy(blob.data() + o, seg_off.data(), nb_off);
+        SLIC_PROPAGATE(stage_to_device(plan.ptr, blob.data(), blob.size(), st));
+    }
+    unsigned char* pb = static_cast<unsigned char*>(plan.ptr);
+    const int4* band_dev = reinterpret_cast<const int4*>(pb);
+    const int4* bound_dev = reinterpret_cast<const int4*>(pb + nb_band);
+    const int4* sample_dev = reinterpret_cast<const int4*>(pb + nb_band + nb_bound);
+    const int4* seg_dev = reinterpret_cast<const int4*>(pb + nb_band + nb_bound + nb_sample);
+    const int64_t* seg_off_dev = reinterpret_cast<const int64_t*>(pb + nb_band + nb_bound + nb_sample + nb_seg);
+
+    const int64_t grid = pairs * 2;
+    const int64_t regions = grid * TC_EPI_WARPS;
+    const int64_t capacity = std::max<int64_t>((int64_t)SYM_LOG_PER_ROW * n, SYM_LOG_MIN);
+    const int64_t region = ceil_div(capacity, regions);
+    SLIC_REQUIRE(region < ((int64_t)1 << 31), "pruned screen: log region too large");
+    Scratch lq, lnb, ls, lcnt, best, rmin, edist, ovr, stats, ctl, sync;
+    SLIC_CUDA_OK(lq.alloc(regions * region * sizeof(int), st));
+    SLIC_CUDA_OK(lnb.alloc(regions * region * sizeof(int), st));
+    SLIC_CUDA_OK(ls.alloc(regions * region * sizeof(float), st));
+    SLIC_CUDA_OK(edist.alloc(regions * region * sizeof(T), st));
+    SLIC_CUDA_OK(lcnt.alloc(regions * sizeof(int), st));
+    SLIC_CUDA_OK(best.alloc(n * sizeof(unsigned int), st));
+    SLIC_CUDA_OK(rmin.alloc(n * sizeof(Bits), st));
+    SLIC_CUDA_OK(ovr.alloc(n * sizeof(int), st));
+    SLIC_CUDA_OK(ctl.alloc(PRUNE_CTL * sizeof(int), st));
+    SLIC_CUDA_OK(cudaMemsetAsync(ctl.ptr, 0, PRUNE_CTL * sizeof(int), st));
+    SLIC_CUDA_OK(sync.alloc(sizeof(int), st));
+    int* stats_dev = stats_ext;
+    if (!stats_dev) {
+        SLIC_CUDA_OK(stats.alloc(8 * sizeof(int), st));
+        stats_dev = stats.as<int>();
+    }
+    int* flag_dev = stats_dev + 5;
+    {
+        const int64_t rmin_bytes = n * (int64_t)sizeof(Bits);
+        int64_t threads = std::max<int64_t>(std::max<int64_t>(n, regions), std::max<int64_t>(ceil_div(rmin_bytes, 16), 8));
+        sym_init_kernel<<<(unsigned)ceil_div(threads, 256), 256, 0, st>>>(stats_dev, lcnt.as<int>(), regions,
+                                                                         static_cast<unsigned char*>(rmin.ptr), rmin_bytes,
+                                                                         sync.as<int>(), best.as<unsigned int>(), nullptr, n,
+                                                                         (unsigned int*)idx_out);
+        SLIC_LAUNCH_OK();
+    }
+    ScreenPlan pl;
+    pl.splits = 1;
+    pl.tiles_per_split = (int)T_;
+    pl.units = (int64_t)band.size();
+    SLIC_PROPAGATE(launch_screen(ubp.as<uint16_t>(), n, ubp.as<uint16_t>(), n, d_pad, 0, eps, 0, pl, lnb.as<int>(),
+                                 ls.as<float>(), lcnt.as<int>(), flag_dev, nullptr, stats_dev + 4, st, 0, nullptr, band_dev,
+                                 nullptr, best.as<unsigned int>(), band_tiles, lq.as<int>(), (int)region, nullptr, nullptr,
+                                 nullptr, nullptr, nullptr, (const int*)nullptr));
+    unit_lower_bound_kernel<<<(unsigned)R, 256, 0, st>>>(best.as<unsigned int>(), n, eps, lmin.as<double>());
+    SLIC_LAUNCH_OK();
+    if (prof) SLIC_CUDA_OK(cudaEventRecord(info.ev[2], st));
+
+    Scratch tmax, keep, survivors;
+    size_t bound_prof = SIZE_MAX;
+    SLIC_CUDA_OK(tmax.alloc(R * T_ * sizeof(int), st));
+    fill_u32_kernel<<<(unsigned)ceil_div(R * T_, 256), 256, 0, st>>>(tmax.as<unsigned int>(), R * T_, 0x80000000u);
+    SLIC_LAUNCH_OK();
+    SLIC_CUDA_OK(keep.alloc(std::max<int64_t>(off_tiles, 1), st));
+    SLIC_CUDA_OK(survivors.alloc(std::max<int64_t>(off_tiles, 1) * sizeof(int4), st));
+    if (!bound.empty()) {
+        pl.units = (int64_t)sample.size();
+        int64_t sample_tiles = 0;
+        for (const int4& e : sample) sample_tiles += e.z & 0xffff;
+        SLIC_PROPAGATE(launch_screen(reinterpret_cast<const uint16_t*>(q8.ptr), n, reinterpret_cast<const uint16_t*>(q8.ptr), n,
+                                     d_pad, -1, eps, 0, pl, nullptr, nullptr, nullptr, nullptr, nullptr, stats_dev + 4, st, 0,
+                                     nullptr, sample_dev, nullptr, nullptr, sample_tiles, nullptr, 0, nullptr, nullptr,
+                                     nullptr, nullptr, tmax.as<int>(), nullptr));
+        prune_select_kernel<<<1, 1024, 0, st>>>(sample_dev, (int)sample.size(), tmax.as<int>(), T_, scale.as<double>(),
+                                                rmax.as<double>(), lmin.as<double>(), (int)bound.size(), PRUNE_MAX_SURVIVAL,
+                                                ctl.as<int>());
+        SLIC_LAUNCH_OK();
+        pl.units = (int64_t)bound.size();
+        SLIC_PROPAGATE(launch_screen(reinterpret_cast<const uint16_t*>(q8.ptr), n, reinterpret_cast<const uint16_t*>(q8.ptr), n,
+                                     d_pad, -1, eps, 0, pl, nullptr, nullptr, nullptr, nullptr, nullptr, stats_dev + 4, st, 0,
+                                     nullptr, bound_dev, nullptr, nullptr, off_tiles, nullptr, 0, nullptr, nullptr, nullptr,
+                                     nullptr, tmax.as<int>(), ctl.as<int>() + 0));
+        if (prof) bound_prof = g_prof_used - 1;
+        prune_keep_kernel<<<(unsigned)segs.size(), (unsigned)chunk_tiles, 0, st>>>(
+            seg_dev, seg_off_dev, tmax.as<int>(), T_, scale.as<double>(), rmax.as<double>(), lmin.as<double>(), ctl.as<int>(),
+            keep.as<uint8_t>());
+        SLIC_LAUNCH_OK();
+        prune_compact_kernel<<<1, 1024, 0, st>>>(seg_dev, seg_off_dev, (int)segs.size(), keep.as<uint8_t>(), (int)unit_len,
+                                                 survivors.as<int4>(), ctl.as<int>());
+        SLIC_LAUNCH_OK();
+    }
+    if (prof) SLIC_CUDA_OK(cudaEventRecord(info.ev[3], st));
+
+    if (!bound.empty()) {
+        pl.units = off_tiles;
+        SLIC_PROPAGATE(launch_screen(ubp.as<uint16_t>(), n, ubp.as<uint16_t>(), n, d_pad, 0, eps, 0, pl, lnb.as<int>(),
+                                     ls.as<float>(), lcnt.as<int>(), flag_dev, nullptr, stats_dev + 4, st, 0, nullptr,
+                                     survivors.as<int4>(), nullptr, best.as<unsigned int>(), off_tiles, lq.as<int>(),
+                                     (int)region, nullptr, nullptr, nullptr, nullptr, nullptr, ctl.as<int>() + 2));
+    }
+    ProfiledLaunch* last = prof && g_prof_used ? &g_prof[g_prof_used - 1] : nullptr;
+    if (prof) SLIC_CUDA_OK(cudaEventRecord(info.ev[4], st));
+    sym_rerank_dist_kernel<T><<<(unsigned)regions, 256, 0, st>>>(unit, d, eps, (int)region, lq.as<int>(), lnb.as<int>(),
+                                                                 ls.as<float>(), lcnt.as<int>(), best.as<unsigned int>(),
+                                                                 rmin.as<Bits>(), edist.as<T>(), stats_dev, perm.as<int>());
+    SLIC_LAUNCH_OK();
+    sym_rerank_pick_kernel<T><<<(unsigned)regions, 256, 0, st>>>((int)region, lq.as<int>(), lnb.as<int>(), lcnt.as<int>(),
+                                                                 rmin.as<Bits>(), edist.as<T>(), idx_out, dist_out,
+                                                                 perm.as<int>());
+    SLIC_LAUNCH_OK();
+    sym_unsettled_rows_kernel<<<(unsigned)ceil_div(n, 256), 256, 0, st>>>(idx_out, n, ovr.as<int>(), stats_dev);
+    SLIC_LAUNCH_OK();
+    if (prof) {
+        SLIC_CUDA_OK(cudaEventRecord(info.ev[5], st));
+        SLIC_CUDA_OK(cudaMemcpyAsync(info.ctl, ctl.ptr, sizeof(info.ctl), cudaMemcpyDeviceToHost, st));
+        SLIC_CUDA_OK(cudaMemcpyAsync(&info.log_overflow, stats_dev + 5, sizeof(int), cudaMemcpyDeviceToHost, st));
+        if (info.perm_cap < n) {
+            if (info.perm_dev) SLIC_CUDA_OK(cudaFree(info.perm_dev));
+            SLIC_CUDA_OK(cudaMalloc(&info.perm_dev, n * sizeof(int)));
+            info.perm_cap = n;
+        }
+        SLIC_CUDA_OK(cudaMemcpyAsync(info.perm_dev, perm.ptr, n * sizeof(int), cudaMemcpyDeviceToDevice, st));
+        info.perm_n = n;
+        SLIC_CUDA_OK(cudaStreamSynchronize(st));
+        info.valid = true;
+        info.path = info.ctl[1];
+        info.band_tiles = band_tiles;
+        if (last && !bound.empty()) last->exec_flop = 2.0 * (double)info.ctl[4] * TC_ROW_UNIT * TC_BN * (double)d_pad;
+        if (bound_prof != SIZE_MAX && info.ctl[0] == 0) g_prof[bound_prof].exec_flop = 0.0;
+        g_last_flop = 2.0 * (double)n * (double)n * (double)d_pad;
+    }
+    if (stats_ext) return SLIC_OK;
+    int host_stats[8];
+    SLIC_CUDA_OK(cudaMemcpyAsync(host_stats, stats_dev, sizeof(host_stats), cudaMemcpyDeviceToHost, st));
+    SLIC_CUDA_OK(cudaStreamSynchronize(st));
+    if (host_stats[4] != 0) {
+        set_error(host_stats[4] == 2 ? "nn_screen_kernel: shared-memory window is not aligned as the symmetric layout assumes"
+                                     : "nn_screen_kernel: pipeline barrier timed out");
+        return host_stats[4] == 2 ? SLIC_ERR_UNSUPPORTED : SLIC_ERR_CUDA;
+    }
+    if (host_stats[5] != 0) {
+        *overflowed = true;
+        return SLIC_OK;
+    }
+    const int n_over = host_stats[1];
+    if (n_over > 0) {
+        Scratch oi, od;
+        SLIC_CUDA_OK(oi.alloc((int64_t)n_over * sizeof(int), st));
+        SLIC_CUDA_OK(od.alloc((int64_t)n_over * sizeof(T), st));
+        SLIC_PROPAGATE(slic_nn_exact_top1(unit, ovr.as<int>(), n_over, unit, n, d, dtype, 0, oi.as<int>(), od.ptr, st));
         scatter_rows_kernel<T><<<(unsigned)ceil_div(n_over, 256), 256, 0, st>>>(ovr.as<int>(), n_over, oi.as<int>(),
                                                                                 od.as<T>(), idx_out, dist_out);
         SLIC_LAUNCH_OK();
@@ -2363,15 +2986,79 @@
         slic::set_error("last_screen_time: no profiled launch (call slic_profile_screen(1) first)");
         return SLIC_ERR_INVALID_ARG;
     }
-    SLIC_CUDA_OK(cudaEventSynchronize(slic::g_ev_stop));
-    SLIC_CUDA_OK(cudaEventElapsedTime(ms_out, slic::g_ev_start, slic::g_ev_stop));
+    float total = 0.f;
+    for (size_t i = 0; i < slic::g_prof_used; ++i) {
+        float ms = 0.f;
+        SLIC_CUDA_OK(cudaEventSynchronize(slic::g_prof[i].stop));
+        SLIC_CUDA_OK(cudaEventElapsedTime(&ms, slic::g_prof[i].start, slic::g_prof[i].stop));
+        total += ms;
+    }
+    *ms_out = total;
     *flop_out = slic::g_last_flop;
     return SLIC_OK;
 }
 
+int slic_pruned_screen_info(double* out_host) {
+    using namespace slic;
+    SLIC_REQUIRE(out_host, "pruned_screen_info: null pointer");
+    if (!g_prune_info.valid) {
+        set_error("pruned_screen_info: no profiled pruned search (slic_profile_screen(1), then a self-search of >= %lld rows)",
+                  (long long)PRUNE_MIN_ROWS);
+        return SLIC_ERR_INVALID_ARG;
+    }
+    for (int i = 0; i < 5; ++i) {
+        float ms = 0.f;
+        SLIC_CUDA_OK(cudaEventElapsedTime(&ms, g_prune_info.ev[i], g_prune_info.ev[i + 1]));
+        out_host[i] = ms;
+    }
+    out_host[5] = (double)g_prune_info.band_tiles;
+    out_host[6] = g_prune_info.ctl[3];
+    out_host[7] = g_prune_info.ctl[4];
+    out_host[8] = g_prune_info.path;
+    out_host[9] = g_prune_info.ctl[5];
+    out_host[10] = g_prune_info.ctl[6];
+    out_host[11] = g_prune_info.log_overflow;
+    return SLIC_OK;
+}
+
+int slic_last_pruned_perm(int32_t* perm_out_dev, int64_t n) {
+    using namespace slic;
+    SLIC_REQUIRE(perm_out_dev, "last_pruned_perm: null pointer");
+    if (!g_prune_info.valid || g_prune_info.perm_n != n) {
+        set_error("last_pruned_perm: the last profiled search was not a pruned search of %lld rows", (long long)n);
+        return SLIC_ERR_INVALID_ARG;
+    }
+    SLIC_CUDA_OK(cudaMemcpy(perm_out_dev, g_prune_info.perm_dev, n * sizeof(int), cudaMemcpyDeviceToDevice));
+    return SLIC_OK;
+}
+
+int slic_debug_quantise_units(const void* unit_dev, int64_t n, int32_t d, int32_t d_pad, int32_t dtype, int8_t* q_out_dev,
+                              double* scale_out_dev, double* rmax_out_dev, slic_stream_t stream) {
+    using namespace slic;
+    SLIC_REQUIRE(unit_dev && q_out_dev && scale_out_dev && rmax_out_dev, "debug_quantise_units: null pointer");
+    SLIC_REQUIRE(n > 0 && n < ((int64_t)1 << 31) && d > 0 && d_pad >= d && d_pad % 64 == 0, "debug_quantise_units: bad shape");
+    SLIC_REQUIRE(dtype == SLIC_F32 || dtype == SLIC_F64, "debug_quantise_units: bad dtype");
+    cudaStream_t st = as_stream(stream);
+    Scratch ident;
+    SLIC_CUDA_OK(ident.alloc(n * sizeof(int), st));
+    strided_rows_kernel<<<(unsigned)ceil_div(n, 256), 256, 0, st>>>(ident.as<int>(), n, n);
+    SLIC_LAUNCH_OK();
+    const unsigned units = (unsigned)ceil_div(n, TC_ROW_UNIT);
+    if (dtype == SLIC_F32)
+        quantise_units_kernel<float><<<units, 256, 0, st>>>((const float*)unit_dev, ident.as<int>(), n, d, d_pad, q_out_dev,
+                                                            scale_out_dev, rmax_out_dev);
+    else
+        quantise_units_kernel<double><<<units, 256, 0, st>>>((const double*)unit_dev, ident.as<int>(), n, d, d_pad,
+                                                             q_out_dev, scale_out_dev, rmax_out_dev);
+    SLIC_LAUNCH_OK();
+    return SLIC_OK;
+}
+
 int slic_last_screen_exec_flop(double* flop_out) {
     SLIC_REQUIRE(flop_out, "last_screen_exec_flop: null pointer");
-    *flop_out = slic::g_have_sample ? slic::g_last_exec_flop : 0.0;
+    double total = 0.0;
+    for (size_t i = 0; slic::g_have_sample && i < slic::g_prof_used; ++i) total += slic::g_prof[i].exec_flop;
+    *flop_out = total;
     return SLIC_OK;
 }
 
```

New measurement: 16.19 million (median of 6 runs). 1.8x the previous value.
